# It4innovations/hyperqueue

Measured on AMD Instinct MI355X. Metric: tasks_assigned_per_sec, higher is better.
Workload: dtype u64

## Files before the change

hyperqueue_amd/_testhooks.py:

```python
from __future__ import annotations

import ctypes as C
import os

_LIB = None
LIB_PATH = os.environ.get("HQTICK_TEST_LIB") or os.path.join(os.path.dirname(os.path.abspath(__file__)), "libhqtick_test.so")


def load() -> C.CDLL:
    global _LIB
    if _LIB is None:
        if not os.path.exists(LIB_PATH):
            raise FileNotFoundError(f"{LIB_PATH} is missing: run `python -c 'import __graft_entry__ as g; g.build()'`")
        _LIB = C.CDLL(LIB_PATH)
    return _LIB
```

hyperqueue_amd/csrc/debug_capi.cpp:

```cpp
#include "../../include/hqtick_debug.h"

#include <algorithm>
#include <cstring>

#include "audit_core.h"
#include "clock_core.h"
#include "hb_order.h"
#include "milp.h"
#include "price_emul.h"

static thread_local int g_last_canonical = 0;
static thread_local long g_last_hull[2] = {0, 0};
extern "C" int hqtick_debug_milp_was_canonical(void) { return g_last_canonical; }
extern "C" void hqtick_debug_milp_last_hull(long *solves, long *nonpacking) {
    if (solves) *solves = g_last_hull[0];
    if (nonpacking) *nonpacking = g_last_hull[1];
}

extern "C" int hqtick_debug_milp_solve(int ncols, const double *obj, const uint8_t *col_kind, int nrows, const uint8_t *row_type,
                                       const double *rhs, const int *row_off, const int *row_col, const double *row_coef,
                                       double time_limit_s, int canonical, double *x_out, double *obj_out, int *is_optimal,
                                       long *nodes_out) {
    hqmilp::Model m;
    m.obj.assign(obj, obj + ncols);
    m.kind.assign(col_kind, col_kind + ncols);
    m.rtype.assign(row_type, row_type + nrows);
    m.rhs.assign(rhs, rhs + nrows);
    m.roff.assign(row_off, row_off + nrows + 1);
    int nnz = nrows ? row_off[nrows] : 0;
    m.rcol.assign(row_col, row_col + nnz);
    m.rcoef.assign(row_coef, row_coef + nnz);
    hqmilp::Result r = hqmilp::solve(m, time_limit_s, canonical != 0);
    g_last_canonical = r.canonical ? 1 : 0;
    g_last_hull[0] = r.hull_solves; g_last_hull[1] = r.hull_solves_nonpacking;
    if (nodes_out) *nodes_out = r.nodes;
    if (!r.feasible) return 0;
    for (int j = 0; j < ncols; j++) x_out[j] = r.x[j];
    *obj_out = r.objective;
    *is_optimal = r.optimal ? 1 : 0;
    return 1;
}

extern "C" void hqtick_debug_map_order_u32(const uint32_t *keys, uint32_t n, uint32_t *out_pos) {
    std::vector<uint32_t> order;
    hqhb::insertion_order_u32(keys, n, order);
    for (uint32_t i = 0; i < n; i++) out_pos[i] = order[i];
}

extern "C" int hqtick_debug_milp_solve_priced(int ncols, const double *obj, const uint8_t *col_kind, const int32_t *col_group, int nrows, const uint8_t *row_type,
                                              const uint8_t *row_implied, const double *rhs, const int *row_off, const int *row_col, const double *row_coef,
                                              double time_limit_s, int use_sweeps, uint32_t min_cols, double *x_out, double *obj_out, int *is_optimal, double *stats_out) {
    hqmilp::Model m;
    m.obj.assign(obj, obj + ncols);
    m.kind.assign(col_kind, col_kind + ncols);
    m.rtype.assign(row_type, row_type + nrows);
    m.rhs.assign(rhs, rhs + nrows);
    m.roff.assign(row_off, row_off + nrows + 1);
    int nnz = nrows ? row_off[nrows] : 0;
    m.rcol.assign(row_col, row_col + nnz);
    m.rcoef.assign(row_coef, row_coef + nnz);
    if (col_group) m.col_group.assign(col_group, col_group + ncols);
    if (row_implied) m.row_implied.assign(row_implied, row_implied + nrows);
    hqprice::EmulatedSweeper emu;
    if (min_cols) emu.min_cols = min_cols;
    hqmilp::Result r = hqmilp::solve(m, time_limit_s, true, hqmilp::REFERENCE_MIP_REL_GAP, use_sweeps ? &emu : nullptr);
    g_last_canonical = r.canonical ? 1 : 0;
    g_last_hull[0] = r.hull_solves; g_last_hull[1] = r.hull_solves_nonpacking;
    if (stats_out) { stats_out[0] = r.price_sweeps; stats_out[1] = r.price_rounds; stats_out[2] = r.price_total_us; stats_out[3] = r.canonical ? 1.0 : 0.0; }
    if (!r.feasible) return 0;
    for (int j = 0; j < ncols; j++) x_out[j] = r.x[j];
    *obj_out = r.objective;
    *is_optimal = r.optimal ? 1 : 0;
    return 1;
}

static thread_local hqmilp::Probe g_block_run_probe;
extern "C" void hqtick_debug_set_block_runs(int on) {
    hqmilp::g_probe = on < 0 ? nullptr : &g_block_run_probe; hqmilp::set_block_runs(on);
    if (on >= 0) { g_block_run_probe.model = g_block_run_probe.tables = g_block_run_probe.runs = g_block_run_probe.covered = 0; }
}
extern "C" void hqtick_debug_corrupt_block_runs(int on) { g_block_run_probe.corrupt_runs = on != 0; }
extern "C" void hqtick_debug_last_coupled_digest(uint64_t out[4]) {
    out[0] = g_block_run_probe.model; out[1] = g_block_run_probe.tables; out[2] = g_block_run_probe.runs; out[3] = g_block_run_probe.covered;
}
extern "C" void hqtick_debug_set_early_sweep(int on) { hqprice::set_early_sweep(on); }
extern "C" uint32_t hqtick_debug_early_sweeps(void) { return hqprice::early_sweeps(); }
extern "C" void hqtick_debug_capture_first_cut(int on) { hqprice::capture_first_cut(on != 0); }
extern "C" uint32_t hqtick_debug_first_cut(unsigned char *out, uint32_t cap) {
    const std::vector<unsigned char> &b = hqprice::first_cut_bytes();
    if (out && cap) memcpy(out, b.data(), std::min<size_t>(cap, b.size()));
    return (uint32_t)b.size();
}

extern "C" int hqtick_debug_clock_rows(uint32_t n, const int64_t *deadline_ns, int64_t now_ns, uint32_t nv, const uint64_t *min_time_ns, int sorted_form, int64_t *remaining_out) {
    if ((n && (!deadline_ns || !remaining_out)) || (nv && !min_time_ns)) return HQTICK_E_INVALID;
    if (!sorted_form) {
        for (uint32_t w = 0; w < n; w++) {
            if (deadline_ns[w] == hqclock::NO_LIMIT) { remaining_out[w] = hqclock::NO_LIMIT; continue; }
            const int64_t r = hqclock::sat_sub(deadline_ns[w], now_ns);
            uint64_t best = 0;
            for (uint32_t v0 = 0; r >= 0 && v0 < nv; v0 += hqclock::CHUNK) best = hqclock::fold_thresholds(best, r, min_time_ns + v0, std::min(hqclock::CHUNK, nv - v0));
            remaining_out[w] = r < 0 ? -1 : (int64_t)best;
        }
        return 0;
    }
    std::vector<uint64_t> thr(min_time_ns, min_time_ns + nv);
    std::sort(thr.begin(), thr.end()); thr.erase(std::unique(thr.begin(), thr.end()), thr.end());
    for (uint32_t w = 0; w < n; w++) remaining_out[w] = hqclock::canonical_sorted(deadline_ns[w], now_ns, thr.data(), (uint32_t)thr.size());
    return 0;
}
extern "C" int hqtick_debug_audit_host(const hqtick_debug_audit_tables *a, uint32_t parts, int order, hqtick_check_report *out) {
    if (!a || !out || (parts & ~(HQ_CHECK_ALL | HQ_CHECK_STRICT)) || order < 0 || order > 2 || (a->have & ~31u)) return HQTICK_E_INVALID;
    hqaudit::State S{};
    S.have = a->have; S.parts = parts;
    S.ready = hqaudit::Ready{a->ready_id, a->ready_rq, a->ready_n};
    S.graph = hqaudit::Graph{a->g_id, a->g_unfinished, a->g_gen, a->g_head, a->g_ht_key, a->g_ht_val, a->g_ht_mask, a->g_run_next, a->g_run_off, a->g_run_len, a->g_edge,
                             a->g_slots, a->g_runs, a->g_edges, a->g_tasks};
    S.ledger = hqaudit::Ledger{a->l_key, a->l_worker, a->l_rq, a->l_variant, a->l_mask, a->l_rq_off, a->l_ventry_off, a->l_ent_res, a->l_var_nodes, a->l_ent_kind, a->l_ent_amount,
                               a->l_Q, a->l_NV, a->l_wid, a->l_W, a->l_R, a->l_total, a->l_free, a->l_counts, a->l_stride, a->l_pf, a->l_pf_stride, a->l_mn_task, a->l_mn_root,
                               a->l_flags, a->l_n_live, a->l_mn_live, a->l_pf_live};
    S.retr = hqaudit::Retr{a->r_task, a->r_target, a->r_variant, a->r_flags, a->r_n};
    const hqaudit::Totals t{a->ready_live, a->g_tasks, a->g_free, a->g_slots};
    hqaudit::run_host(S, t, order, out);
    return (int)out->n_failed;
}
extern "C" int64_t hqtick_debug_clock_deadline(int64_t now_ns, int64_t remaining_ns) { return hqclock::deadline_of(now_ns, remaining_ns); }
extern "C" int64_t hqtick_debug_clock_remaining(int64_t deadline_ns, int64_t now_ns) { return hqclock::remaining_of(deadline_ns, now_ns); }
```

hyperqueue_amd/csrc/host_model.cpp:

```cpp
#include "host_model.h"

#include <algorithm>
#include <chrono>
#include <cmath>
#include <cstring>
#include <string>
#include <unordered_map>

#include "hb_order.h"

namespace hqhost {

namespace {

struct OrderEntry { uint64_t hash = 0; bool used = false; std::vector<uint32_t> ids, order; };
thread_local OrderEntry order_cache[32];
thread_local unsigned order_next = 0;
const std::vector<uint32_t> &cached_worker_order(const std::vector<uint32_t> &ids) {
    typedef OrderEntry Entry;
    Entry (&cache)[32] = order_cache;
    unsigned &next = order_next;
    uint64_t h = 0x9E3779B97F4A7C15ull ^ ids.size();
    for (uint32_t v : ids) { h ^= v; h *= 0xFF51AFD7ED558CCDull; h ^= h >> 29; }
    for (Entry &e : cache) if (e.used && e.hash == h && e.ids.size() == ids.size() && (ids.empty() || memcmp(e.ids.data(), ids.data(), ids.size() * 4) == 0)) return e.order;
// ... 1081 lines not shown
        if (blocker_ord[brq] < 0) {
            blocker_ord[brq] = (int32_t)n_blockers_seen++;
            left_state.resize((size_t)n_blockers_seen * n_sig_cap, 0); left_row.resize((size_t)n_blockers_seen * n_sig_cap * R); left_of.resize(left_state.size());
        }
        const size_t li = (size_t)blocker_ord[brq] * n_sig_cap + sg;
        if (left_state[li] == 0) {
            if (agg_off.empty()) build_agg();
            const uint32_t a0 = agg_off[w], na = agg_off[w + 1] - a0;
            const uint32_t *arq = na ? agg_rq.data() + a0 : nullptr, *acnt = na ? agg_cnt.data() + a0 : nullptr; const uint8_t *avar = na ? agg_variant.data() + a0 : nullptr;
            if (gaps.leftover_row(brq, ws.total + (size_t)w * R, R, arq, avar, na, acnt, &left_row[li * R])) left_state[li] = 3;
            else {
                Amounts tot; tot.a.assign(ws.total + (size_t)w * R, ws.total + (size_t)(w + 1) * R);
                left_state[li] = gaps.leftover(brq, tot, arq, avar, na, acnt, left_of[li]) ? 1 : 2;
            }
        }
        return left_state[li] == 3 ? gaps.fit_row(low_rq, &left_row[li * R], R) : (left_state[li] == 1 ? gaps.fit(low_rq, left_of[li]) : 0);
    };
    std::vector<uint32_t> gap_of_sig; uint32_t batch_no = UINT32_MAX;
    std::vector<std::vector<uint8_t>> cap_cache; std::vector<int8_t> all_cap_cache; size_t n_triples = 0, n_decided_once = 0;
    std::vector<uint32_t> bcols_off, bcols_end((size_t)ws.n, 0); std::vector<int> bcols; std::vector<uint64_t> bcols_ub; uint64_t bcols_ub_max = 0; uint32_t bcols_batch = UINT32_MAX;
    for (const TaskBatch &batch : batches) {
        batch_no++;
        auto cc = count_cols.find(batch.rq);
        if (cc == count_cols.end()) continue;
        const RequestView &brv = pb.rqs[batch.rq];
        if (!batch.limit_reached) {
            list_row(hqmilp::ROW_MAX, (double)batch.size, count_lhs_id(batch.rq), cc->second, -1, 0.0);
        }
        double bsize = (double)batch.size;
        std::vector<uint32_t> capped_by;
        struct PairMemo { bool done = false, whole = false, all_gap = false; uint32_t gap_all = 0; int lhs_id = -1; int64_t max_excess = INT64_MIN; std::vector<int> no_gap; std::vector<std::pair<uint32_t, uint32_t>> with_gap; };
        std::vector<PairMemo> pair_memo;
        for (const PriorityCut &cut : batch.cuts) {
            for (auto &bl : cut.blockers) {
                uint32_t brq = bl.first; bool bounded = bl.second != HQ_BLOCKER_UNBOUNDED;
                std::vector<int> no_gap_mn;
                const std::vector<int> *no_gap = &no_gap_mn;
                int no_gap_id = -1;
                std::vector<int> cols;
                int fl_cached = -2;
                if (pb.rq_multi_node(batch.rq)) {
                    for (uint32_t g = 0; g < pb.n_groups; g++) {
                        auto it = group_cols.find({batch.rq, g});
                        if (it != group_cols.end() && group_can_run_rq(g, brq)) no_gap_mn.push_back(it->second);
                    }
                } else {
                    if (pair_memo.size() < pb.rqs.size()) pair_memo.resize(pb.rqs.size());
                    PairMemo &pm = pair_memo[brq];
                    if (!pm.done) {
                        pm.done = true;
                        if (cap_cache.size() < pb.rqs.size()) cap_cache.resize(pb.rqs.size());
                        std::vector<uint8_t> &cap_brq = cap_cache[brq];
                        if (cap_brq.empty()) { cap_brq.assign(ws.n, 0); for (uint32_t w : solver_workers) cap_brq[w] = pb.capable_rqv(ws, w, brq) ? 1 : 0; }
                        if (bcols_batch != batch_no) {
                            bcols_batch = batch_no; bcols_off.assign((size_t)ws.n + 1, 0); bcols.clear(); bcols_ub.assign(ws.n, 0); bcols_ub_max = 0;
                            if (runs_on) bcols.reserve((size_t)m.ncols());
                            for (uint32_t w : solver_workers) {
                                bcols_off[w] = (uint32_t)bcols.size();
                                if (runs_on && stamp_first[w] != UINT32_MAX) {
                                    const uint32_t f = stamp_first[w]; const int d = blk_base[w] - blk_base[f];
                                    for (uint32_t i = bcols_off[f], e = bcols_end[f]; i < e; i++) { const int pc = bcols[i] + d; bcols.push_back(pc); }
                                    bcols_ub[w] = bcols_ub[f];
                                } else
                                for (uint8_t v = 0; v < brv.n_variants; v++) { const int pc = place_get(w, batch.rq, v); if (pc >= 0) { bcols.push_back(pc); bcols_ub[w] += col_ub[(size_t)pc]; } }
                                bcols_end[w] = (uint32_t)bcols.size(); bcols_ub_max = std::max(bcols_ub_max, bcols_ub[w]);
                            }
                        }
                        n_triples++;
                        if (!sigs_done) { for (uint32_t w : solver_workers) sig_of(w); sigs_done = true; }
                        gap_of_sig.assign(sig_rep.size(), UINT32_MAX);
                        bool all_capable = true;
                        if (runs_on) {
                            if (all_cap_cache.size() < pb.rqs.size()) all_cap_cache.resize(pb.rqs.size(), -1);
                            if (all_cap_cache[brq] < 0) { all_cap_cache[brq] = 1; for (uint32_t w : solver_workers) if (!cap_brq[w]) { all_cap_cache[brq] = 0; break; } }
                            all_capable = all_cap_cache[brq] != 0;
                        } else
                        if (sig_rep.size() == 1) for (uint32_t w : solver_workers) if (!cap_brq[w]) { all_capable = false; break; }
                        if (sig_rep.size() == 1 && all_capable && !solver_workers.empty()) {
                            const uint32_t w0 = solver_workers[0];
                            const uint32_t gap = gap_of(brq, batch.rq, gap_sig[w0], w0);
                            if (runs_on) {
                                if (gap > 0) { pm.all_gap = true; pm.gap_all = gap; pm.max_excess = (int64_t)bcols_ub_max - (int64_t)gap; } else pm.whole = true;
                            } else
                            if (gap > 0) { pm.with_gap.reserve(solver_workers.size()); for (uint32_t w : solver_workers) pm.with_gap.push_back({w, gap}); }
                            else pm.no_gap.assign(bcols.begin(), bcols.end());
                        } else {
                        pm.no_gap.reserve(bcols.size());
                        for (uint32_t w : solver_workers) {
                            if (!cap_brq[w]) continue;
                            uint32_t gap = gap_of_sig[gap_sig[w]];
                            if (gap == UINT32_MAX) gap = gap_of_sig[gap_sig[w]] = gap_of(brq, batch.rq, gap_sig[w], w);
                            if (gap > 0) pm.with_gap.push_back({w, gap});
                            else pm.no_gap.insert(pm.no_gap.end(), bcols.data() + bcols_off[w], bcols.data() + bcols_end[w]);
                        }
                        }
                        auto list_of = [&](const PairMemo &q) -> const std::vector<int> & { return q.whole ? bcols : q.no_gap; };
                        if (!list_of(pm).empty()) {
                            for (const PairMemo &o : pair_memo) if (&o != &pm && o.lhs_id >= 0 && ((o.whole && pm.whole) || list_of(o) == list_of(pm))) { pm.lhs_id = o.lhs_id; break; }
                            if (pm.lhs_id < 0) pm.lhs_id = next_lhs_id++;
                        }
                        if (runs_on) for (auto &wg : pm.with_gap) pm.max_excess = std::max(pm.max_excess, (int64_t)bcols_ub[wg.first] - (int64_t)wg.second);
                    }
                    no_gap = pm.whole ? &bcols : &pm.no_gap; no_gap_id = pm.lhs_id;
                    auto gap_rows = [&](const uint32_t w, const uint32_t gap) {
                        const int *wc = bcols.data() + bcols_off[w]; const size_t nwc = bcols_end[w] - bcols_off[w];
                        const uint64_t cols_ub = bcols_ub[w];
                        if (bounded && fl_cached == -2) fl_cached = short_flag(brq, bl.second);
                        const int fl = bounded ? fl_cached : -1;
                        if (cols_ub <= (uint64_t)cut.size + gap) return;
                        if (bounded && fl >= 0) { cols.assign(wc, wc + nwc); emit_plus(hqmilp::ROW_MAX, (double)cut.size + bsize + (double)gap, cols, fl, bsize); }
                        else if (!bounded) { m.begin_row(hqmilp::ROW_MAX, (double)cut.size + (double)gap); for (size_t k = 0; k < nwc; k++) m.term(wc[k], 1.0); m.end_row(); }
                    };
                    if (runs_on && (pm.all_gap || !pm.with_gap.empty()) && pm.max_excess <= (int64_t)cut.size) {
                        if (bounded) fl_cached = short_flag(brq, bl.second);
                        n_decided_once++;
                    } else if (pm.all_gap) for (uint32_t w : solver_workers) gap_rows(w, pm.gap_all);
                    else for (auto &wg : pm.with_gap) gap_rows(wg.first, wg.second);
                }
                if (no_gap->empty()) continue;
                int fl;
                if (bounded && (fl = short_flag(brq, bl.second)) >= 0) list_row(hqmilp::ROW_MAX, bsize + (double)cut.size, no_gap_id, *no_gap, fl, bsize);
                else if (!bounded && std::find(capped_by.begin(), capped_by.end(), brq) == capped_by.end()) {
                    capped_by.push_back(brq);
                    list_row(hqmilp::ROW_MAX, (double)cut.size, no_gap_id, *no_gap, -1, 0.0);
                }
            }
        }
    }

    if (!seq_start.empty()) {
        m.start.assign(m.ncols(), 0.0);
        for (const SeqStart &ss : seq_start) {
            const int pc = place_get(ss.w, batches[ss.batch].rq, ss.variant);
            if (pc < 0) { m.start.clear(); break; }
            m.start[pc] = ss.count;
        }
    }
    m.row_implied.resize(m.nrows(), 0);
    m.row_lhs.resize((size_t)m.nrows(), -1); m.row_lhs_len.resize((size_t)m.nrows(), 0); m.row_block.resize((size_t)m.nrows(), -1);
    m.col_ub = col_ub; m.col_ub.resize((size_t)m.ncols(), UINT32_MAX);
    if (hqmilp::g_probe) {
        using hqmilp::fnv1a_vec;
        uint64_t h = hqmilp::FNV_BASIS;
        h = fnv1a_vec(h, m.obj); h = fnv1a_vec(h, m.kind); h = fnv1a_vec(h, m.rtype); h = fnv1a_vec(h, m.rhs); h = fnv1a_vec(h, m.roff); h = fnv1a_vec(h, m.rcol); h = fnv1a_vec(h, m.rcoef);
        h = fnv1a_vec(h, m.start); h = fnv1a_vec(h, m.col_group); h = fnv1a_vec(h, m.row_implied); h = fnv1a_vec(h, m.row_lhs); h = fnv1a_vec(h, m.row_lhs_len);
        h = fnv1a_vec(h, m.list_off); h = fnv1a_vec(h, m.list_col); h = fnv1a_vec(h, m.row_block); h = fnv1a_vec(h, m.col_ub);
        hqmilp::g_probe->model = h; hqmilp::g_probe->runs = m.block_runs.size(); hqmilp::g_probe->tables = 0; hqmilp::g_probe->covered = 0;
    }
    const double t_model1 = clock_us();
    if (trace_model) {
        size_t run_blocks = 0; for (const auto &br : m.block_runs) run_blocks += (size_t)br.n_blocks;
        fprintf(stderr, "[model] cuts done at %.3f ms: %d columns, %d rows, %zu terms, %zu worker signatures, %zu (batch, cut, blocker) passes over the workers; %zu equal-block runs over %zu blocks, %zu (cut, blocker) passes decided once\n", (t_model1 - t_model0) / 1e3, m.ncols(), m.nrows(), m.rcol.size(), sig_rep.size(), n_triples, m.block_runs.size(), run_blocks, n_decided_once);
    }
    hqmilp::Result sol = hqmilp::solve(m, pb.time_limit_s, !pb.certificate_only, hqmilp::REFERENCE_MIP_REL_GAP, pb.pricer);
    if (trace_model) fprintf(stderr, "[model] solve done %.3f ms after the model\n", (clock_us() - t_model1) / 1e3);
    out.pre_us = t_model0 - t_enter; out.model_us = t_model1 - t_model0; out.milp_us = clock_us() - t_model1; out.price_sweeps = sol.price_sweeps; out.price_rounds = sol.price_rounds; out.price_us = sol.price_total_us;
    out.milp_nodes = sol.nodes; out.milp_cols = m.ncols(); out.milp_rows = m.nrows(); out.milp_components = sol.n_components;
    if (!sol.feasible) return out;
    out.is_optimal = sol.optimal;
    out.is_canonical = sol.canonical && sol.optimal;

    std::vector<uint64_t> key_hash; std::vector<std::pair<uint32_t, uint8_t>> key_list; std::vector<std::vector<std::pair<uint32_t, uint32_t>>> key_counts;
    std::vector<uint64_t> mn_hash; std::vector<uint32_t> mn_list; std::vector<std::vector<std::vector<uint32_t>>> mn_sets;
    std::vector<uint32_t> dec_ids, dec_widx, dec_cnt;
    for (const TaskBatch &batch : batches) {
        const RequestView &rv = pb.rqs[batch.rq];
        if (pb.rq_multi_node(batch.rq)) {
            size_t n_nodes = pb.variants[rv.first_variant].n_nodes;
            std::vector<std::vector<uint32_t>> sets;
            for (uint32_t w : solver_workers) {
                const int pc = place_get(w, batch.rq, 0);
                if (pc < 0 || (uint32_t)std::round(sol.x[pc]) == 0) continue;
                if (!sets.empty() && sets.back().size() < n_nodes) sets.back().push_back(w); else sets.push_back({w});
            }
            if (!sets.empty()) { mn_hash.push_back(hqhb::hash_rq_variant(batch.rq, 0)); mn_list.push_back(batch.rq); mn_sets.push_back(sets); }
        } else {
            for (uint8_t v = 0; v < rv.n_variants; v++) {
                const size_t nsw = solver_workers.size();
                dec_ids.resize(nsw + 1); dec_widx.resize(nsw + 1); dec_cnt.resize(nsw + 1);
                uint32_t *idp = dec_ids.data(), *wxp = dec_widx.data(), *cp = dec_cnt.data(); size_t nk = 0;
                const int *pcol = place_col.data() + rv.first_variant + v;
                const double *xs = sol.x.data();
                for (size_t i = 0; i < nsw; i++) {
                    const uint32_t w = solver_workers[i];
                    const int pc = pcol[(size_t)w * NVS];
                    const double xv = pc >= 0 ? xs[pc] : 0.0;
                    const uint32_t c = xv > 0.0 ? (uint32_t)(xv + 0.5) : 0u;
                    idp[nk] = ws.id[w]; wxp[nk] = w; cp[nk] = c; nk += c > 0 ? 1 : 0;
                }
                if (nk == 0) continue;
                dec_ids.resize(nk);
                const std::vector<uint32_t> &ids = dec_ids, &widx = dec_widx, &cnt = dec_cnt;
                const std::vector<uint32_t> &word = cached_worker_order(ids);
                std::vector<std::pair<uint32_t, uint32_t>> ordered; ordered.reserve(word.size());
                for (uint32_t k : word) ordered.push_back({widx[k], cnt[k]});
                key_hash.push_back(hqhb::hash_rq_variant(batch.rq, v)); key_list.push_back({batch.rq, v}); key_counts.push_back(std::move(ordered));
            }
        }
    }
    std::vector<uint32_t> ord;
    hqhb::insertion_order(key_hash.data(), (uint32_t)key_hash.size(), ord);
    for (uint32_t k : ord) { out.keys.push_back(key_list[k]); out.per_key.push_back(std::move(key_counts[k])); }
    hqhb::insertion_order(mn_hash.data(), (uint32_t)mn_hash.size(), ord);
    for (uint32_t k : ord) { out.mn_rq.push_back(mn_list[k]); out.mn_sets.push_back(std::move(mn_sets[k])); }
    if (trace_model) fprintf(stderr, "[model] decoded %.3f ms after the model, %.3f ms after the solver was entered\n", (clock_us() - t_model1) / 1e3, (clock_us() - t_enter) / 1e3);
    return out;
}

}
```

hyperqueue_amd/csrc/host_model.h:

```cpp
#pragma once
#include <cstdint>
#include <map>
#include <string>
#include <tuple>
#include <vector>

#include "../../include/hqtick.h"
#include "block_core.h"
#include "price.h"
#include "milp.h"

namespace hqhost {

struct VariantView {
    const uint32_t *res;
    const uint8_t *kind;
    const uint64_t *amount;
    uint32_t n_entries, n_nodes, weight;
    uint64_t min_time_ns;
    bool multi_node() const { return n_nodes > 0; }
};

struct RequestView {
    uint32_t first_variant, n_variants;
};

struct QueueLevels {
    std::vector<std::pair<uint64_t, uint32_t>> levels;
};

struct PriorityCut { uint32_t size; std::vector<std::pair<uint32_t, uint32_t>> blockers; };
struct TaskBatch {
    uint32_t rq = 0, size = 0, limit = 0;
    bool limit_reached = false, is_blocker = false;
    std::vector<PriorityCut> cuts;
};

struct WorkerGroups {
    std::vector<uint32_t> of, rep, count;
    std::vector<uint32_t> solver_workers;
    std::vector<double> pool;
    bool valid = false;
};

struct WorkerSet {
    WorkerGroups rows;
    uint32_t n = 0, R = 0;
    const uint32_t *id = nullptr;
    const uint64_t *total = nullptr, *free_ = nullptr;
    const int64_t *remaining_ns = nullptr;
    const float *min_util = nullptr;
    const uint8_t *flags = nullptr;
    const uint32_t *group = nullptr;
    const uint8_t *vflags = nullptr;
    const uint32_t *vtmc = nullptr;
    uint32_t n_variant_slots = 0;
    std::vector<std::vector<std::pair<uint32_t, uint8_t>>> blocked;
    uint32_t n_blocked_lists = 0;
    const uint32_t *assigned_off = nullptr, *assigned_rq = nullptr; const uint8_t *assigned_variant = nullptr;
    const uint32_t *agg_off = nullptr, *agg_rq = nullptr, *agg_cnt = nullptr; const uint8_t *agg_variant = nullptr;
    uint32_t n_assigned(uint32_t w) const { return assigned_off ? assigned_off[w + 1] - assigned_off[w] : agg_off ? agg_off[w + 1] - agg_off[w] : 0; }
    bool is_sn(uint32_t w) const { return flags ? (flags[w] & HQ_WORKER_SN) != 0 : true; }
    bool stopping(uint32_t w) const { return flags ? (flags[w] & HQ_WORKER_STOPPING) != 0 : false; }
    bool is_free(uint32_t w) const { return is_sn(w) && n_assigned(w) == 0 && !stopping(w); }
    uint8_t vf(uint32_t w, uint32_t slot) const { return vflags[(size_t)w * n_variant_slots + slot]; }
    uint32_t tmc(uint32_t w, uint32_t slot) const { return vtmc[(size_t)w * n_variant_slots + slot]; }
};

struct BlockSolver {
    virtual ~BlockSolver() {}
    virtual bool solve(const hqblock::ColTable &cols, const hqblock::ClassTable &classes, const hqblock::Output &out) = 0;
    virtual bool begin(const hqblock::ColTable &cols, const hqblock::ClassTable &classes, const hqblock::Output &out) { begun_ok = solve(cols, classes, out); return begun_ok; }
    virtual bool finish() { return begun_ok; }
    virtual bool overlaps() const { return false; }
    bool begun_ok = false;
};

void flush_tick_caches();

struct BlockMemo {
    struct Entry { uint64_t hash = 0; std::vector<unsigned char> key; std::vector<double> x; long nodes = 0; int n_components = 0; };
    static constexpr size_t CAP = 64;
    std::vector<Entry> entries;
    size_t next = 0;
    std::vector<unsigned char> scratch;
    uint64_t scratch_hash = 0;
    const Entry *find(const hqmilp::Model &m);
    void put(const hqmilp::Result &r);
};

struct Problem {
    BlockMemo *memo = nullptr;
    BlockSolver *blocks = nullptr;
    hqprice::Sweeper *pricer = nullptr;
    uint32_t block_min_classes = 1;
    uint32_t block_verify = 2;
    uint32_t tick_seq = 0;
    uint32_t R = 0, n_groups = 0;
    std::vector<RequestView> rqs;
    std::vector<VariantView> variants;
    WorkerSet real;
    const WorkerSet *custom = nullptr;
    double time_limit_s = 5.0;
    bool certificate_only = false;
    bool rq_multi_node(uint32_t rq) const { return variants[rqs[rq].first_variant].multi_node(); }
    bool capable_rqv(const WorkerSet &ws, uint32_t w, uint32_t rq) const {
        for (uint32_t v = 0; v < rqs[rq].n_variants; v++) {
            uint32_t slot = rqs[rq].first_variant + v;
            uint8_t f = ws.vf(w, slot);
            if ((f & 4) && (variants[slot].multi_node() || (f & 2))) return true;
        }
        return false;
    }
};

void group_equal_rows(WorkerSet &ws, bool all_solver);

std::vector<TaskBatch> create_task_batches(const Problem &pb, const std::vector<QueueLevels> &queues);

struct Counts {
    std::vector<std::pair<uint32_t, uint8_t>> keys;
    std::vector<std::vector<std::pair<uint32_t, uint32_t>>> per_key;
    std::vector<uint32_t> mn_rq;
    std::vector<std::vector<std::vector<uint32_t>>> mn_sets;
    struct WorkerList { std::vector<uint32_t> widx; };
    bool by_class = false;
    bool one_class = false;
    uint32_t n_cols = 0;
    std::vector<uint32_t> wclass, class_x, key_col, key_list;
    std::vector<WorkerList> lists;
    bool pairs_built = true;
    void pairs() {
        if (pairs_built) return;
        per_key.assign(keys.size(), {});
        for (size_t k = 0; k < keys.size(); k++) {
            const std::vector<uint32_t> &wi = lists[key_list[k]].widx;
            auto &out = per_key[k]; out.resize(wi.size());
            for (size_t i = 0; i < wi.size(); i++) out[i] = {wi[i], class_x[(size_t)wclass[wi[i]] * n_cols + key_col[k]]};
        }
        pairs_built = true;
    }
    size_t key_size(size_t k) const { return pairs_built ? per_key[k].size() : lists[key_list[k]].widx.size(); }
    bool is_optimal = true;
    bool is_canonical = true;
    bool empty() const {
        if (!pairs_built) { for (size_t k = 0; k < keys.size(); k++) if (key_size(k)) return false; }
        for (auto &k : per_key) if (!k.empty()) return false;
        for (auto &k : mn_sets) if (!k.empty()) return false;
        return true;
    }
    uint32_t checksum() const {
        uint32_t h = 2166136261u;
        auto mix = [&](uint32_t v) { for (int i = 0; i < 4; i++) { h ^= (v >> (8 * i)) & 0xFFu; h *= 16777619u; } };
        mix(is_optimal ? 1u : 0u);
        for (size_t k = 0; k < keys.size(); k++) {
            mix(keys[k].first); mix(keys[k].second);
            if (pairs_built) for (auto &wc : per_key[k]) { mix(wc.first); mix(wc.second); }
            else for (uint32_t w : lists[key_list[k]].widx) { mix(w); mix(class_x[(size_t)wclass[w] * n_cols + key_col[k]]); }
        }
        for (size_t k = 0; k < mn_rq.size(); k++) { mix(mn_rq[k]); for (auto &set : mn_sets[k]) { mix(0xFFFFFFFFu); for (uint32_t w : set) mix(w); } }
        return h;
    }
    int error = 0; std::string errmsg;
    long milp_nodes = 0; int milp_cols = 0, milp_rows = 0, milp_components = 0;
    int price_sweeps = 0, price_rounds = 0; double price_us = 0, milp_us = 0, model_us = 0, pre_us = 0;
    uint32_t blocks_device = 0, blocks_host = 0, block_steps_max = 0, n_classes = 0;
    uint32_t blocks_verified = 0, blocks_mismatch = 0, blocks_rejected = 0;
    uint32_t blocks_memo = 0;
    double t_classify_us = 0, t_blocks_us = 0, t_decode_us = 0;
};

Counts run_scheduling_solver(const Problem &pb, const std::vector<TaskBatch> &batches);

}
```

hyperqueue_amd/csrc/hqtick.cpp:

```cpp
#include "../../include/hqtick.h"
#ifdef HQTICK_TEST_HOOKS
#include "../../include/hqtick_debug.h"
#endif

#include <dlfcn.h>
#include <hip/hip_runtime.h>
#include <rccl/rccl.h>

#include <algorithm>
#include <chrono>
#include <cstdio>
#include <cstdlib>
#include <cstring>
#include <functional>
#include <map>
#include <string>
#include <vector>

#include "audit.h"
#include "block_solve.h"
#include "cluster.h"
#include "price_dev.h"
#include "ready.h"
#include "scan.h"
#ifdef HQTICK_TEST_HOOKS
#include "price_emul.h"
#endif
#include "devbuf.h"
#include "graph.h"
#include "ledger.h"
#include "map.h"
#include "hb_order.h"
#include "host_model.h"
#include "kernels.h"

using hqbuf::DevBuf;
using hqbuf::PinBuf;
using hqcluster::UpView;
using hqscan::Scan;
using hqscan::WorkerEval;

namespace {

double now_us() { return std::chrono::duration<double, std::micro>(std::chrono::steady_clock::now().time_since_epoch()).count(); }

}

namespace {
struct ViewHooks {
    hqscan::Scanner scan;
    bool valid = false; const void *ids = nullptr; uint64_t N = 0; uint32_t Q = 0, n_live = 0; bool rq_copy = false; std::vector<uint32_t> run_off, run_start, run_rank;
    DevBuf d_map, d_sel_task, d_sel_rank, d_rq, d_want;
    void release() { scan.release(); d_map.release(); d_sel_task.release(); d_sel_rank.release(); d_rq.release(); d_want.release(); }
};
}

struct hqtick_ctx {
    hqtick_config cfg;
    int device = 0;
    hipStream_t stream = nullptr;
    hipStream_t stream2 = nullptr;
    bool k2_on_hist = false;
    bool k2_own_stream = false;
    hipEvent_t ev[14] = {};
    std::string err = "";
    hqready::ReadySet ready;
    hqhost::BlockMemo block_memo;
    hqscan::Scanner scan;
    hqmap::Mapper map;
    bool timing = true, timing_k1 = false;
    PinBuf h_up, h_up2, h_q, h_blk;
    PinBuf h_blkprof; uint32_t n_blkprof = 0; bool block_profile = false;
    hqprice::DeviceSweeper *pricer = nullptr;
    uint32_t block_budget = 4096, block_min_classes = 12;
    DevBuf d_blk;
    hqcluster::WorkerSet ws;
    hqcluster::Retracting retr;
    uint32_t last_row_groups = 0;
    bool wait_on_kernel = true;
    hqhost::Problem pb;
    std::vector<uint32_t> b_rq, b_size, b_limit, b_cut_off, c_size, c_bl_off, bl_rq, bl_size; std::vector<uint8_t> b_lr, b_blk;
    std::vector<uint8_t> q_loaded;
    hqtick_kernel_stats stats{};
    uint32_t tpw_hint = 0;
    uint32_t shard_index = 0, shard_count = 1;
    void *sink = nullptr; size_t sink_bytes = 0;
    hqgraph::Graph graph;
    hqasg::Ledger asg;
    hqtick_ctx *qctx = nullptr;
    ViewHooks *view_hooks = nullptr;
    ncclComm_t comm = nullptr; uint32_t comm_rank = 0, comm_world = 0;
    hqtick_exchange_fn xfn = nullptr; void *xuser = nullptr;
    DevBuf d_xsend, d_xrecv; PinBuf h_xsend, h_xrecv;
    uint32_t shard_min_blocks = 1025, shard_min_classes = 1025; bool shard_solve = true;
    uint32_t block_verify = 2, tick_seq = 0;
    uint64_t x_calls = 0, x_bytes = 0; double x_us = 0;
    double tl[32] = {}; int ntl = 0;
    hqaudit::Auditor audit;
    bool check_resident = false; int audit_depth = 0;
};

namespace {

#define HQ_HIP(call)                                                                                          \
    do {                                                                                                      \
        hipError_t e_ = (call);                                                                               \
        if (e_ != hipSuccess) { ctx->err = std::string(#call) + ": " + hipGetErrorString(e_); return HQTICK_E_DEVICE; } \
    } while (0)

#define HQ_HIP_TIMED(call)                                                                                    \
    do {                                                                                                      \
        hipError_t e_ = (call);                                                                               \
        hqk::take_launch_timer();                                                                             \
        if (e_ != hipSuccess) { ctx->err = std::string(#call) + ": " + hipGetErrorString(e_); return HQTICK_E_DEVICE; } \
    } while (0)

#define HQ_HIP_LAST(call, launched)                                                                           \
    do {                                                                                                      \
        hipError_t e_ = (call);                                                                               \
        (launched) = hqk::take_launch_timer().stop == nullptr && ctx->wait_on_kernel;                        \
        if (e_ != hipSuccess) { ctx->err = std::string(#call) + ": " + hipGetErrorString(e_); return HQTICK_E_DEVICE; } \
    } while (0)

int fail(hqtick_ctx *ctx, int code, const std::string &msg) { ctx->err = msg; return code; }

double elapsed_us(hipEvent_t a, hipEvent_t b) {
    float ms = 0;
    if (hipEventElapsedTime(&ms, a, b) == hipSuccess) return (double)ms * 1000.0;
    (void)hipGetLastError();
    return -1.0;
}

int validate(hqtick_ctx *ctx, const hqtick_snapshot *s, bool need_tasks) {
    if (!s) return fail(ctx, HQTICK_E_INVALID, "null snapshot");
    if (s->n_workers && (!s->worker_id || !s->worker_total || !s->worker_free)) return fail(ctx, HQTICK_E_INVALID, "worker arrays missing");
    for (uint32_t w = 1; w < s->n_workers; w++) if (s->worker_id[w - 1] >= s->worker_id[w]) return fail(ctx, HQTICK_E_INVALID, "worker ids not ascending");
    if (s->n_requests && (!s->rq_variant_off || !s->variant_entry_off)) return fail(ctx, HQTICK_E_INVALID, "request arrays missing");
    for (uint32_t q = 0; q < s->n_requests; q++) {
        if (s->rq_variant_off[q + 1] <= s->rq_variant_off[q]) return fail(ctx, HQTICK_E_INVALID, "request without variants");
        if (s->rq_variant_off[q + 1] - s->rq_variant_off[q] > 32) return fail(ctx, HQTICK_E_INVALID, "more than 32 variants");
    }
    uint32_t nv = s->n_requests ? s->rq_variant_off[s->n_requests] : 0;
    for (uint32_t e = 0; e < (nv ? s->variant_entry_off[nv] : 0); e++) {
        if (s->entry_resource[e] >= s->n_resources) return fail(ctx, HQTICK_E_INVALID, "entry resource id out of range");
        if (s->entry_kind[e] == HQ_ENTRY_AMOUNT && s->entry_amount[e] == 0) return fail(ctx, HQTICK_E_INVALID, "zero amount request");
    }
    if (need_tasks && s->n_ready) {
        if (!s->task_id || !s->task_priority || !s->task_rq) return fail(ctx, HQTICK_E_INVALID, "ready-set columns missing");
        for (uint64_t i = 1; i < s->n_ready; i++) if (s->task_id[i - 1] >= s->task_id[i]) return fail(ctx, HQTICK_E_INVALID, "ready set not sorted by task id");
    }
    if (s->n_blocked && (!s->blocked_worker || !s->blocked_rq || !s->blocked_variant)) return fail(ctx, HQTICK_E_INVALID, "blocked arrays missing");
    for (uint32_t k = 0; k < s->n_blocked; k++) {
        if (s->blocked_worker[k] >= s->n_workers) return fail(ctx, HQTICK_E_INVALID, "blocked worker index");
        if (s->blocked_rq[k] >= s->n_requests) return fail(ctx, HQTICK_E_INVALID, "blocked request id out of range");
        if (s->blocked_variant[k] >= s->rq_variant_off[s->blocked_rq[k] + 1] - s->rq_variant_off[s->blocked_rq[k]]) return fail(ctx, HQTICK_E_INVALID, "blocked variant out of range");
    }
    if (s->worker_group) for (uint32_t w = 0; w < s->n_workers; w++) if (s->worker_group[w] >= (s->n_groups ? s->n_groups : 1)) return fail(ctx, HQTICK_E_INVALID, "worker_group >= n_groups");
    if (s->assigned_off) {
        for (uint32_t w = 0; w < s->n_workers; w++) if (s->assigned_off[w] > s->assigned_off[w + 1]) return fail(ctx, HQTICK_E_INVALID, "assigned_off not monotone");
        if (s->n_workers && s->assigned_off[s->n_workers] && (!s->assigned_rq || !s->assigned_variant)) return fail(ctx, HQTICK_E_INVALID, "assigned arrays missing");
    }
    if (s->prefilled_off) {
        for (uint32_t w = 0; w < s->n_workers; w++) if (s->prefilled_off[w] > s->prefilled_off[w + 1]) return fail(ctx, HQTICK_E_INVALID, "prefilled_off not monotone");
        if (s->n_workers && s->prefilled_off[s->n_workers] && !s->prefilled_rq) return fail(ctx, HQTICK_E_INVALID, "prefilled_rq missing");
    }
    if (s->prefill_off) {
        for (uint32_t q = 0; q < s->n_requests; q++) if (s->prefill_off[q] > s->prefill_off[q + 1]) return fail(ctx, HQTICK_E_INVALID, "prefill_off not monotone");
        const uint32_t np = s->n_requests ? s->prefill_off[s->n_requests] : 0;
        if (np && (!s->prefill_priority || !s->prefill_task || !s->prefill_worker)) return fail(ctx, HQTICK_E_INVALID, "prefill arrays missing");
        for (uint32_t i = 0; i < np; i++) if (s->prefill_worker[i] >= s->n_workers) return fail(ctx, HQTICK_E_INVALID, "prefill worker index");
    }
    if (s->n_retracting && (!s->retracting_task || !s->retracting_worker)) return fail(ctx, HQTICK_E_INVALID, "retracting arrays missing");
    for (uint32_t k = 0; k < s->n_retracting; k++) {
        if (s->retracting_worker[k] >= s->n_workers) return fail(ctx, HQTICK_E_INVALID, "retracting worker index");
        if (k && s->retracting_task[k - 1] >= s->retracting_task[k]) return fail(ctx, HQTICK_E_INVALID, "retracting tasks not ascending");
        if (s->retracting_redirect_worker && s->retracting_redirect_worker[k] != HQ_NO_WORKER && s->retracting_redirect_worker[k] >= s->n_workers) return fail(ctx, HQTICK_E_INVALID, "retracting redirect worker index");
    }
    return 0;
}

int upload_tables(hqtick_ctx *ctx, const hqtick_snapshot *s, uint32_t W, const uint64_t *total, const uint64_t *free_, const int64_t *rem, PinBuf &buf, UpView *uv) {
    const uint32_t R = s->n_resources;
    const hqcluster::TabLayout L = hqcluster::table_layout(s, W);
    if (hqk::worker_eval_lds(R, L.nv, L.ne) > 150 * 1024) return fail(ctx, HQTICK_E_CAPACITY, "request table + 32 worker rows exceed the 150 KiB the worker-evaluation kernel stages in LDS");
    if (!buf.ensure(L.bytes)) return fail(ctx, HQTICK_E_DEVICE, "allocating upload staging");
    unsigned char *h = buf.as<unsigned char>();
    hqcluster::pack_worker_rows(h, L, W, R, total, free_, rem);
    hqcluster::pack_request_tables(h, L, s);
    hqcluster::view_tables(buf.dev<unsigned char>(), L, uv);
    return 0;
}

int cluster_fail(hqtick_ctx *ctx, int rc) { if (rc < 0) ctx->err = ctx->ws.err; return rc; }

hqready::Env ready_env(hqtick_ctx *ctx) { return hqready::Env{ctx->device, ctx->stream, ctx->ev[11], ctx->wait_on_kernel}; }
int ready_fail(hqtick_ctx *ctx, int rc) { if (rc < 0) ctx->err = ctx->ready.err; return rc; }

int eval_workers_sync(hqtick_ctx *ctx, const hqtick_snapshot *s, uint32_t W, const uint64_t *total, const uint64_t *free_, const int64_t *rem, WorkerEval *out) {
    UpView uv; int rc;
    if ((rc = upload_tables(ctx, s, W, total, free_, rem, ctx->h_up2, &uv))) return rc;
    size_t n = (size_t)W * uv.rt.n_variants;
    if (!ctx->h_q.ensure(n * 5 + 64)) return fail(ctx, HQTICK_E_DEVICE, "hipHostMalloc query eval");
    out->tmc = ctx->h_q.as<uint32_t>(); out->flags = ctx->h_q.as<uint8_t>() + n * 4;
    if (n == 0) return 0;
    HQ_HIP(hqk::worker_eval(uv.total, uv.free_, uv.rem, W, s->n_resources, uv.rt, uv.n_entries, ctx->h_q.dev<uint8_t>() + n * 4, ctx->h_q.dev<uint32_t>(), ctx->stream));
    HQ_HIP(hipStreamSynchronize(ctx->stream));
    return 0;
}

void fill_problem(hqhost::Problem &pb, const hqtick_snapshot *s, const hqtick_config &cfg, const WorkerEval &ev) {
    pb.R = s->n_resources; pb.n_groups = s->n_groups ? s->n_groups : 1; pb.time_limit_s = cfg.mip_time_limit_s; pb.certificate_only = (cfg.flags & HQTICK_FLAG_CERTIFICATE_ONLY) != 0;
    uint32_t nv = s->n_requests ? s->rq_variant_off[s->n_requests] : 0;
    pb.rqs.resize(s->n_requests); pb.variants.resize(nv);
    for (uint32_t q = 0; q < s->n_requests; q++) pb.rqs[q] = {s->rq_variant_off[q], s->rq_variant_off[q + 1] - s->rq_variant_off[q]};
    for (uint32_t v = 0; v < nv; v++) {
        uint32_t e0 = s->variant_entry_off[v];
        pb.variants[v] = {s->entry_resource + e0, s->entry_kind + e0, s->entry_amount + e0, s->variant_entry_off[v + 1] - e0,
                          s->variant_n_nodes ? s->variant_n_nodes[v] : 0, s->variant_weight ? s->variant_weight[v] : 10000,
                          s->variant_min_time_ns ? s->variant_min_time_ns[v] : 0};
    }
    hqhost::WorkerSet &ws = pb.real;
    ws.n = s->n_workers; ws.R = s->n_resources; ws.id = s->worker_id; ws.total = s->worker_total; ws.free_ = s->worker_free;
    ws.remaining_ns = s->worker_remaining_ns; ws.min_util = s->worker_min_utilization; ws.flags = s->worker_flags; ws.group = s->worker_group;
    ws.vflags = ev.flags; ws.vtmc = ev.tmc; ws.n_variant_slots = nv;
    if (ws.blocked.size() != ws.n || ws.n_blocked_lists) { ws.blocked.assign(ws.n, {}); ws.n_blocked_lists = 0; }
    ws.assigned_off = s->assigned_off; ws.assigned_rq = s->assigned_rq; ws.assigned_variant = s->assigned_variant;
    ws.agg_off = nullptr; ws.agg_rq = nullptr; ws.agg_cnt = nullptr; ws.agg_variant = nullptr;
    for (uint32_t k = 0; k < s->n_blocked; k++) ws.blocked[s->blocked_worker[k]].push_back({s->blocked_rq[k], s->blocked_variant[k]});
    ws.n_blocked_lists = s->n_blocked;
    hqhost::group_equal_rows(ws, false);
}

// ... 57 lines not shown

struct DeviceBlocks : hqhost::BlockSolver {
    hqtick_ctx *ctx;
    explicit DeviceBlocks(hqtick_ctx *c) : ctx(c) {}
    bool solve(const hqblock::ColTable &ct, const hqblock::ClassTable &cl, const hqblock::Output &out) override { return begin(ct, cl, out) && finish(); }
    bool overlaps() const override { return true; }
    hqblock::Output p_out{}; size_t p_ox = 0, p_ost = 0, p_osteps = 0; uint32_t p_nd = 0, p_nc = 0; bool p_launched = false, p_pending = false;
    bool begin(const hqblock::ColTable &ct, const hqblock::ClassTable &cl, const hqblock::Output &out) override {
        p_pending = false;
        const uint32_t NC = ct.n_cols, R = ct.R, nd = cl.n_classes, ne = ct.ent_off[NC];
        auto al8 = [](size_t v) { return (v + 7) & ~(size_t)7; };
        const size_t o_off = 0, o_res = al8(o_off + (size_t)(NC + 1) * 4), o_w = al8(o_res + (size_t)ne * 4), o_kind = al8(o_w + (size_t)NC * 4), o_amt = al8(o_kind + ne),
                     o_pool = o_amt + (size_t)ne * 8, o_free = (o_pool + (size_t)R * 8 + 15) & ~(size_t)15, o_tot = o_free + (size_t)nd * R * 8, o_elig = o_tot + (size_t)nd * R * 8,
                     o_x = o_elig + (size_t)nd * 8, o_st = o_x + al8((size_t)nd * NC * 4), o_steps = o_st + al8((size_t)nd * 4), bytes = o_steps + al8((size_t)nd * 4) + 64;
        if (!ctx->h_blk.ensure(bytes)) return false;
        if (!ctx->d_blk.ensure(o_x + 64)) return false;
        unsigned char *h = ctx->h_blk.as<unsigned char>(), *d = ctx->d_blk.as<unsigned char>(), *dpin = ctx->h_blk.dev<unsigned char>();
        memcpy(h + o_off, ct.ent_off, (size_t)(NC + 1) * 4); memcpy(h + o_res, ct.ent_res, (size_t)ne * 4); memcpy(h + o_w, ct.weight, (size_t)NC * 4);
        memcpy(h + o_kind, ct.ent_kind, ne); memcpy(h + o_amt, ct.ent_amount, (size_t)ne * 8); memcpy(h + o_pool, ct.pool, (size_t)R * 8);
        memcpy(h + o_free, cl.free_, (size_t)nd * R * 8); memcpy(h + o_tot, cl.total, (size_t)nd * R * 8); memcpy(h + o_elig, cl.elig, (size_t)nd * 8);
        if (hqk::copy_pinned_to_hbm(dpin, d, o_x, ctx->stream) != hipSuccess) return false;
        hqblock::ColTable dct{NC, R, (const uint32_t *)(d + o_off), (const uint32_t *)(d + o_res), (const uint8_t *)(d + o_kind), (const uint64_t *)(d + o_amt), (const uint32_t *)(d + o_w), (const double *)(d + o_pool), d, (uint32_t)o_free};
        hqblock::ClassTable dcl{nd, (const uint64_t *)(d + o_free), (const uint64_t *)(d + o_tot), (const uint64_t *)(d + o_elig)};
        uint64_t *dprof = nullptr;
        if (ctx->block_profile) {
            if (!ctx->h_blkprof.ensure((size_t)nd * 64 + 64)) return false;
            memset(ctx->h_blkprof.p, 0, (size_t)nd * 64);
            dprof = ctx->h_blkprof.dev<uint64_t>(); ctx->n_blkprof = nd;
        }
        hqblock::Output dout{(uint32_t *)(dpin + o_x), (uint32_t *)(dpin + o_st), (uint32_t *)(dpin + o_steps), dprof};
        hqk::time_next_launch(ctx->timing ? ctx->ev[9] : nullptr, ctx->ev[10]);
        const hipError_t be = hqblock::block_solve(dct, dcl, dout, ctx->block_budget, ctx->stream);
        const bool launched = hqk::take_launch_timer().stop == nullptr && ctx->wait_on_kernel;
        if (be != hipSuccess) return false;
        p_out = out; p_ox = o_x; p_ost = o_st; p_osteps = o_steps; p_nd = nd; p_nc = NC; p_launched = launched; p_pending = true;
        return true;
    }
    bool finish() override {
        if (!p_pending) return false;
        p_pending = false;
        if ((p_launched ? hipEventSynchronize(ctx->ev[10]) : hipStreamSynchronize(ctx->stream)) != hipSuccess) return false;
        const unsigned char *h = ctx->h_blk.as<unsigned char>();
        memcpy(p_out.x, h + p_ox, (size_t)p_nd * p_nc * 4); memcpy(p_out.status, h + p_ost, (size_t)p_nd * 4); memcpy(p_out.steps, h + p_osteps, (size_t)p_nd * 4);
        if (ctx->timing) { const double us_ = elapsed_us(ctx->ev[9], ctx->ev[10]); if (us_ >= 0) ctx->stats.block_solve_us = us_; }
        ctx->stats.n_classes_device = p_nd;
        return true;
    }
};

bool rccl_allgather_host(hqtick_ctx *ctx, const void *send, void *recv, size_t bytes);
struct CtxExchange : hqprice::Exchange {
    hqtick_ctx *ctx;
    explicit CtxExchange(hqtick_ctx *c) : ctx(c) { rank = c->shard_index; world = c->shard_count; }
    static bool available(const hqtick_ctx *c) { return c->shard_solve && c->shard_count > 1 && (c->xfn || (c->comm && c->comm_world == c->shard_count)); }
    bool allgather(const void *send, void *recv, size_t bytes) override {
        if (ctx->xfn) return ctx->xfn(ctx->xuser, send, recv, bytes) == 0;
        return rccl_allgather_host(ctx, send, recv, bytes);
    }
    ~CtxExchange() override { ctx->x_calls += n_calls; ctx->x_bytes += n_bytes; ctx->x_us += us; }
};

struct ShardedBlocks : hqhost::BlockSolver {
    hqhost::BlockSolver &inner; hqprice::Exchange &ex; uint32_t min_classes;
    hqblock::Output p_out{}; uint32_t p_nd = 0, p_nc = 0, p_nm = 0; bool p_pass = false, p_inner_ok = false, p_pending = false;
    std::vector<uint64_t> cfree, ctot, celig; std::vector<uint32_t> dx, dst, dsteps; std::vector<unsigned char> send, recv;
    ShardedBlocks(hqhost::BlockSolver &in, hqprice::Exchange &e, uint32_t mc) : inner(in), ex(e), min_classes(mc) {}
    bool overlaps() const override { return inner.overlaps(); }
    bool solve(const hqblock::ColTable &ct, const hqblock::ClassTable &cl, const hqblock::Output &out) override { return begin(ct, cl, out) && finish(); }
    bool begin(const hqblock::ColTable &ct, const hqblock::ClassTable &cl, const hqblock::Output &out) override {
        p_pass = ex.world <= 1 || cl.n_classes < min_classes;
        if (p_pass) return inner.begin(ct, cl, out);
        const uint32_t nd = cl.n_classes, R = ct.R, NC = ct.n_cols, W = ex.world, me = ex.rank;
        const uint32_t nm = nd > me ? (nd - me + W - 1) / W : 0;
        cfree.resize((size_t)nm * R); ctot.resize((size_t)nm * R); celig.resize(nm);
        for (uint32_t j = 0; j < nm; j++) {
            const size_t i = (size_t)me + (size_t)j * W;
            memcpy(cfree.data() + (size_t)j * R, cl.free_ + i * R, (size_t)R * 8); memcpy(ctot.data() + (size_t)j * R, cl.total + i * R, (size_t)R * 8); celig[j] = cl.elig[i];
        }
        dx.assign((size_t)nm * NC, 0); dst.assign(nm, hqblock::ST_UNSUPPORTED); dsteps.assign(nm, 0);
        p_out = out; p_nd = nd; p_nc = NC; p_nm = nm; p_pending = true;
        p_inner_ok = nm == 0 || inner.begin(ct, hqblock::ClassTable{nm, cfree.data(), ctot.data(), celig.data()}, hqblock::Output{dx.data(), dst.data(), dsteps.data(), nullptr});
        return true;
    }
    bool finish() override {
        if (p_pass) return inner.finish();
        if (!p_pending) return false;
        p_pending = false;
        if (p_nm && !(p_inner_ok && inner.finish())) { std::fill(dst.begin(), dst.end(), (uint32_t)hqblock::ST_UNSUPPORTED); std::fill(dx.begin(), dx.end(), 0u); }
        const uint32_t W = ex.world, NC = p_nc, mx = (p_nd + W - 1) / W;
        const size_t o_st = (size_t)mx * NC * 4, o_steps = o_st + (size_t)mx * 4, bytes = (o_steps + (size_t)mx * 4 + 7) & ~(size_t)7;
        send.assign(bytes, 0); recv.resize(bytes * W);
        if (p_nm) { memcpy(send.data(), dx.data(), (size_t)p_nm * NC * 4); memcpy(send.data() + o_st, dst.data(), (size_t)p_nm * 4); memcpy(send.data() + o_steps, dsteps.data(), (size_t)p_nm * 4); }
        const double t0 = now_us();
        if (!ex.allgather(send.data(), recv.data(), bytes)) return false;
        ex.us += now_us() - t0; ex.n_calls++; ex.n_bytes += bytes * W;
        for (uint32_t r = 0; r < W; r++) {
            const unsigned char *b = recv.data() + (size_t)r * bytes;
            const uint32_t nr = p_nd > r ? (p_nd - r + W - 1) / W : 0;
            for (uint32_t j = 0; j < nr; j++) {
                const size_t i = (size_t)r + (size_t)j * W;
                memcpy(p_out.x + i * NC, b + (size_t)j * NC * 4, (size_t)NC * 4); memcpy(p_out.status + i, b + o_st + (size_t)j * 4, 4); memcpy(p_out.steps + i, b + o_steps + (size_t)j * 4, 4);
            }
        }
        return true;
    }
};

hqmap::Env map_env(hqtick_ctx *ctx, double t0 = 0) {
    return hqmap::Env{ctx->stream, ctx->ev[4], ctx->ev[5], ctx->ev[1], ctx->ev[6], ctx->ev[7], ctx->ev[11], ctx->timing, ctx->wait_on_kernel, ctx->cfg.flags,
                      ctx->sink, ctx->sink_bytes, ctx->shard_index, ctx->shard_count, hqmap::Timeline{t0, ctx->tl, &ctx->ntl}};
}
int map_fail(hqtick_ctx *ctx, int rc) { if (rc < 0) ctx->err = ctx->map.err; return rc; }
bool transpose_enabled() { const char *e = getenv("HQTICK_TRANSPOSE"); return !(e && atoi(e) == 0); }

struct TickRun {
    hqtick_ctx *ctx; const hqtick_snapshot *s; hqtick_result *out; const bool use_resident;
    hqmap::Plan &ps; hqhost::Problem &pb;
    const uint32_t W, R, Q;
    WorkerEval ev; Scan sc; hqhost::Counts cnt;
    uint64_t N = 0; int status = HQTICK_DONE;
    double t0 = 0;

    TickRun(hqtick_ctx *c, const hqtick_snapshot *snap, hqtick_result *o, bool resident)
        : ctx(c), s(snap), out(o), use_resident(resident), ps(c->map.plan), pb(c->pb), W(snap->n_workers), R(snap->n_resources), Q(snap->n_requests) {}

    void mark() { hqmap::Timeline{t0, ctx->tl, &ctx->ntl}.mark(); }
    int plan_fail(int rc, const char *why) { if (rc) ctx->err = why; return rc; }

    int load_ready_set() {
        if (!use_resident) {
            if (int rc = ready_fail(ctx, ctx->ready.load(ctx->stream, s, true))) return rc;
            ctx->scan.columns_changed();
        } else if (!ctx->ready.resident()) return fail(ctx, HQTICK_E_INVALID, "hqtick_run_resident without hqtick_upload_ready");
        N = ctx->ready.cols().n;
        return 0;
    }

    hqmap::PlanIn plan_in() {
        hqmap::PlanIn in{};
        in.sc = &sc; in.cnt = &cnt; in.s = s; in.rqs = pb.rqs.data(); in.variants = pb.variants.data();
        in.proactive_filling_reserve = ctx->cfg.proactive_filling_reserve; in.proactive_filling_max = ctx->cfg.proactive_filling_max; in.flags = ctx->cfg.flags;
        in.sink = ctx->sink != nullptr; in.shard_index = ctx->shard_index; in.shard_count = ctx->shard_count;
        in.N = N; in.retr_key = ctx->scan.retracting_keys(); in.retr_rank = ctx->scan.retracting_ranks();
        if (ctx->asg.on && ctx->asg.tracking()) {
            uint32_t pf_stride = 0;
            const std::vector<uint32_t> &h_pf = ctx->asg.prefilled_host(&pf_stride);
            if (h_pf.size() >= (size_t)W * pf_stride) { in.ledger_pf = h_pf.data(); in.ledger_pf_stride = pf_stride; }
        }
        in.transpose_on = transpose_enabled();
        in.storage = hqmap::Mapper::plan_storage; in.user = &ctx->map;
        return in;
    }

    int phase_c(const hqmap::Env &me, const hqmap::PlanIn &in) {
        hqmap::PhaseC pc{};
        pc.sc = &sc; pc.scan = &ctx->scan; pc.ready = &ctx->ready; pc.in = &in;
        pc.consume_in_tick = use_resident && (ctx->cfg.flags & HQTICK_FLAG_CONSUME_IN_TICK) != 0;
        pc.ledger_pfq_rq = ctx->asg.on;
        if (ps.n_sel && pc.consume_in_tick && ctx->asg.on && s->n_retracting) {
            pc.saved_rq = ctx->asg.saved_rq(N);
            if (!pc.saved_rq) return fail(ctx, HQTICK_E_DEVICE, "hipMalloc ledger request ids");
        }
        if (ps.n_sel && ctx->asg.on && ps.n_rec) {
            hqasg::StageCols c{};
            if (!ctx->asg.stage_for(ps.n_rec, sc.ordered, sc.L, &c)) return fail(ctx, HQTICK_E_DEVICE, "hipMalloc ledger staging");
            pc.stage = hqk::Stage{c.task, c.rq, c.row, c.level, c.meta};
        }
        const int rc = map_fail(ctx, ctx->map.phase_c(me, pc));
        const hqmap::Timings &tm = ctx->map.timings();
        if (tm.select_us >= 0) ctx->stats.select_us = tm.select_us;
        if (tm.sweep_us >= 0) ctx->stats.sweep_us = tm.sweep_us;
        if (tm.other_us >= 0) ctx->stats.other_us = tm.other_us;
        return rc;
    }

    void finish(const hqmap::Env &me, double t1, double t2, double t3) {
        out->status = status;
        ctx->map.export_result(me, cnt, out);
        mark();
        double t5 = now_us();
        out->t_total_us = t5 - t0; out->t_scan_us = t1 - t0; out->t_batches_us = t2 - t1; out->t_solve_us = t3 - t2; out->t_mapping_us = t5 - t3;
        uint64_t n_pref = 0; for (uint32_t q = 0; q < Q; q++) n_pref += ps.new_pf_total[q];
        uint64_t n_asg = 0; for (uint32_t w = 0; w < W; w++) n_asg += ps.n_assign[w];
        uint32_t nv = Q ? s->rq_variant_off[Q] : 0;
        ctx->stats.n_assigned = n_asg; ctx->stats.n_prefilled = n_pref;
        ctx->stats.algorithmic_bytes = N * 20 + (uint64_t)W * R * 16 + (uint64_t)nv * R * 9 + n_asg * 13 + n_pref * 12;
        ctx->stats.tick_gpu_us = ctx->stats.distinct_us + ctx->stats.level_hist_us + ctx->stats.scan_us + ctx->stats.block_solve_us + ctx->stats.select_us + ctx->stats.sweep_us + ctx->stats.other_us;
    }

    int run() {
        t0 = now_us();
        ctx->ntl = 0;
        if (ctx->cfg.flags & HQTICK_FLAG_NO_TICK_CACHES) { ctx->scan.columns_changed(); hqhost::flush_tick_caches(); }
        memset(out, 0, sizeof(*out));
        ctx->stats = hqtick_kernel_stats{};
        int rc = validate(ctx, s, !use_resident);
        if (rc) return rc;
        HQ_HIP(hipSetDevice(ctx->device));
        if ((rc = load_ready_set())) return rc;
        const std::function<void()> prep = [&]() {
            fill_problem(pb, s, ctx->cfg, ev);
            ctx->last_row_groups = (uint32_t)pb.real.rows.rep.size();
            if (ctx->asg.on && !s->assigned_off) {
                const hqasg::Agg g = ctx->asg.agg();
                pb.real.agg_off = g.off; pb.real.agg_rq = g.rq; pb.real.agg_cnt = g.cnt; pb.real.agg_variant = g.var;
            }
            if (pb.certificate_only && (ctx->shard_count > 1 || ctx->sink || ctx->xfn || ctx->comm)) pb.certificate_only = false;
        };
        if ((rc = phase_a(ctx, s, &ev, &sc, &prep))) return rc;
        mark();
        const double t1 = now_us();
        std::vector<hqhost::QueueLevels> qlv = queue_levels(sc, s);
        std::vector<hqhost::TaskBatch> batches = hqhost::create_task_batches(pb, qlv);
        export_batches(ctx, batches, out);
        mark();
        const double t2 = now_us();
        DeviceBlocks dev_blocks(ctx);
        pb.blocks = &dev_blocks; pb.block_min_classes = ctx->block_min_classes; pb.pricer = ctx->pricer;
        pb.block_verify = ctx->block_verify; pb.tick_seq = ctx->tick_seq++;
        pb.memo = (ctx->cfg.flags & (HQTICK_FLAG_NO_BLOCK_MEMO | HQTICK_FLAG_NO_TICK_CACHES)) ? nullptr : &ctx->block_memo;
        double shard_sweep_us = -1.0;
        ctx->x_calls = 0; ctx->x_bytes = 0; ctx->x_us = 0;
        if (CtxExchange::available(ctx)) {
            CtxExchange xch(ctx);
            ShardedBlocks sh_blocks(dev_blocks, xch, ctx->shard_min_classes);
            pb.blocks = &sh_blocks;
            if (ctx->pricer) {
                hqprice::ShardedSweeper sh_sweeps(*ctx->pricer, xch, ctx->shard_min_blocks);
                pb.pricer = &sh_sweeps;
                cnt = hqhost::run_scheduling_solver(pb, batches);
                shard_sweep_us = sh_sweeps.stat_sweep_us;
            } else cnt = hqhost::run_scheduling_solver(pb, batches);
        } else cnt = hqhost::run_scheduling_solver(pb, batches);
        pb.blocks = nullptr; pb.pricer = nullptr;
        ctx->stats.price_sweeps = (uint32_t)cnt.price_sweeps; ctx->stats.price_rounds = (uint32_t)cnt.price_rounds; ctx->stats.price_us = cnt.price_us; ctx->stats.milp_us = cnt.milp_us; ctx->stats.model_us = cnt.model_us; ctx->stats.solve_pre_us = cnt.pre_us;
        ctx->stats.price_sweep_us = shard_sweep_us >= 0.0 ? shard_sweep_us : (ctx->pricer ? ctx->pricer->stat_sweep_us : 0.0); ctx->stats.milp_cols = (uint32_t)cnt.milp_cols; ctx->stats.milp_rows = (uint32_t)cnt.milp_rows;
        ctx->stats.n_classes_verified = cnt.blocks_verified; ctx->stats.n_classes_mismatch = cnt.blocks_mismatch; ctx->stats.n_classes_rejected = cnt.blocks_rejected; ctx->stats.n_classes_memo = cnt.blocks_memo;
        ctx->stats.exchange_calls = (uint32_t)ctx->x_calls; ctx->stats.exchange_bytes = ctx->x_bytes; ctx->stats.exchange_us = ctx->x_us;
        if (cnt.error) return fail(ctx, cnt.error, cnt.errmsg);
        ctx->stats.n_classes_device = cnt.blocks_device; ctx->stats.n_classes_host = cnt.blocks_host; ctx->stats.block_steps_max = cnt.block_steps_max; ctx->stats.n_classes = cnt.n_classes;
        ctx->stats.solve_classify_us = cnt.t_classify_us; ctx->stats.solve_blocks_us = cnt.t_blocks_us; ctx->stats.solve_decode_us = cnt.t_decode_us;
        mark();
        const double t3 = now_us();
        out->is_optimal = cnt.is_optimal;
        out->is_canonical = cnt.is_canonical && cnt.is_optimal;
        status = HQTICK_DONE;
        if (!cnt.is_optimal) status = cnt.empty() ? HQTICK_NO_PROGRESS : HQTICK_NEED_MORE_COMPUTE;
        const hqmap::PlanIn in = plan_in();
        const hqmap::Env me = map_env(ctx, t0);
        hqmap::HostResult &hr = ctx->map.res;
        const char *why = nullptr;
        ctx->ready.selection_void();
        if ((rc = plan_fail(hqmap::plan_keys(ps, hr, in, &why), why))) return rc;
        if ((rc = map_fail(ctx, ctx->map.launch_sweep_early(me)))) return rc;
        if ((rc = plan_fail(hqmap::plan_redirects(ps, hr, in, &why), why))) return rc;
        mark();
        if ((rc = plan_fail(hqmap::plan_prefill(ps, hr, in, &why), why))) return rc;
        mark();
        if ((rc = plan_fail(hqmap::plan_outputs(ps, hr, in, &why), why))) return rc;
        if ((rc = map_fail(ctx, ctx->map.check_capacity(sc.ordered)))) return rc;
        mark();
        if ((rc = phase_c(me, in))) return rc;
        mark();
        finish(me, t1, t2, t3);
        return status;
    }
};

bool ledger_replica(const hqtick_ctx *ctx) { return ctx->shard_count > 1 || ctx->xfn || ctx->comm; }
hqasg::Env ledger_env(hqtick_ctx *ctx) {
    const hqready::Cols c = ctx->ready.cols();
    return hqasg::Env{ctx->device, ctx->stream, ctx->ws.rows(), ctx->ws.W(), ctx->ws.R(), c.id, c.prio, c.rq, c.n,
                      ctx->scan.levels_dev(), &ctx->ws.ids(), ctx->ws.flags(), ctx->ws.free_rows()};
}
int ledger_fail(hqtick_ctx *ctx, int rc) { if (rc < 0) ctx->err = ctx->asg.err; return rc; }
bool ledger_pending_live(hqtick_ctx *ctx) { return ctx->asg.pending_live(ctx->ready.selection_live()); }
int ledger_guard(hqtick_ctx *ctx) {
    if (ctx->asg.on && ledger_pending_live(ctx)) return fail(ctx, HQTICK_E_INVALID, "assignment ledger: the last tick's placement is pending (hqtick_ready_consume_last first)");
    return 0;
}

int run_tick(hqtick_ctx *ctx, const hqtick_snapshot *s, hqtick_result *out, bool use_resident) {
    hqtick_snapshot full;
    if (ctx->asg.on && s) {
        if (ledger_replica(ctx)) return fail(ctx, HQTICK_E_UNSUPPORTED, "assignment ledger on a sharded or replica context");
        if (s->worker_id || !ctx->ws.valid()) return fail(ctx, HQTICK_E_INVALID, "assignment ledger on: the tick runs on the resident worker set (HQ_WORKERS_RESIDENT, no worker arrays)");
        if (s->assigned_off) return fail(ctx, HQTICK_E_INVALID, "assignment ledger on: the snapshot must not carry an assigned CSR as well");
        if (ctx->asg.tracking() && s->prefilled_off) return fail(ctx, HQTICK_E_INVALID, "prefilled tracking on: the snapshot must not carry a prefilled CSR as well");
        HQ_HIP(hipSetDevice(ctx->device));
        ctx->asg.abandon_tick();
        ctx->asg.take_requests(s);
        if (ctx->asg.tracking() && ctx->asg.max_variants() >= hqasg::PF_VARIANT) return fail(ctx, HQTICK_E_UNSUPPORTED, "prefilled tracking: a request has 254 or more variants");
        if (int rc = ctx->asg.sync_mirror(ledger_env(ctx))) return ledger_fail(ctx, rc);
    }
    if (s) {
        if (int rc = cluster_fail(ctx, ctx->ws.complete(s, &full))) return rc;
        s = &full;
    }
    const bool retr_resident = s && s->n_retracting == HQ_RETRACTING_RESIDENT;
    if (retr_resident) { if (int rc = ctx->retr.to_snapshot(s->worker_id, s->n_workers, &full)) return fail(ctx, rc, ctx->retr.err); }
    int rc;
    {
        TickRun run(ctx, s, out, use_resident);
        rc = run.run();
    }
    if (ctx->ready.unconfirmed()) {
        ctx->ready.confirm();
        if (rc < 0) {
            const std::string why = ctx->err;
            bool restored = false;
            const bool synced = hipStreamSynchronize(ctx->stream) == hipSuccess;
            if (synced && ctx->ready.selection_valid())
                restored = ctx->map.replay_selection(ctx->stream, hqmap::REPLAY_RESTORE, ctx->ready.cols(), ctx->scan, ctx->ready.selected_count(), &ctx->h_q) == 0;
            if (restored) ctx->ready.put_back(); else ctx->ready.lost();
            ctx->err = why;
            if (restored) ctx->err += " (HQTICK_FLAG_CONSUME_IN_TICK: what the tick had taken is back in the resident ready set)";
            else { ctx->err += " (HQTICK_FLAG_CONSUME_IN_TICK: the tick had already taken its tasks and they could not be put back; the resident ready set is dropped, upload it again)"; }
        }
    }
    if (rc >= 0 && retr_resident) ctx->retr.apply_tick(s->worker_id, s->n_workers, ctx->map.res.retract_off, ctx->map.res.retract_task, ctx->map.res.red_task, ctx->map.res.red_worker, ctx->map.res.red_variant, ctx->map.res.red_kind);
    if (rc >= 0 && ctx->asg.on) {
        const bool in_tick = use_resident && (ctx->cfg.flags & HQTICK_FLAG_CONSUME_IN_TICK) != 0;
        ctx->asg.collect_tick(s, out, ctx->map.res.new_free, ctx->map.res.mn_rq, in_tick && s->n_retracting != 0);
        if (!use_resident || in_tick) {
            if (int r2 = ledger_fail(ctx, ctx->asg.apply_tick(ledger_env(ctx)))) {
                ctx->asg.on = false; ctx->asg.pending = false;
                ctx->err += " (the assignment ledger is switched off: upload the worker set and enable it again)";
                return r2;
            }
        }
    }
    return rc;
}

}

namespace {
struct AuditScope {
    hqtick_ctx *c;
    explicit AuditScope(hqtick_ctx *ctx) : c(ctx) { if (c) c->audit_depth++; }
    ~AuditScope() { if (c) c->audit_depth--; }
};
int audited(hqtick_ctx *ctx, int rc) {
    static const char *const names[HQ_INV_N] = {"HQ_INV_READY_ORDER", "HQ_INV_READY_COUNT", "HQ_INV_LEDGER_HASH", "HQ_INV_LEDGER_ENTRY", "HQ_INV_LEDGER_TOTALS", "HQ_INV_LEDGER_COUNTS",
                                                "HQ_INV_LEDGER_PREFILLED", "HQ_INV_LEDGER_FREE", "HQ_INV_LEDGER_MN", "HQ_INV_GRAPH_HASH", "HQ_INV_GRAPH_TOTALS", "HQ_INV_GRAPH_COUNTER",
                                                "HQ_INV_X_READY_ASSIGNED", "HQ_INV_X_READY_WAITING", "HQ_INV_X_RETRACTING", "HQ_INV_S_READY_UNKNOWN", "HQ_INV_S_ASSIGNED_WAITING",
                                                "HQ_INV_S_RELEASED_NOWHERE"};
    if (!ctx || !ctx->check_resident || ctx->audit_depth || rc < 0) return rc;
    hqtick_check_report rep;
    const int arc = hqtick_resident_check(ctx, HQ_CHECK_READY | HQ_CHECK_LEDGER | HQ_CHECK_GRAPH, &rep);
    if (arc <= 0) return arc < 0 ? arc : rc;
    std::string m = "HQTICK_CHECK_RESIDENT: the resident state is inconsistent after this call:";
    for (uint32_t k = 0; k < HQ_INV_N; k++)
        if (rep.count[k]) m += std::string(" ") + names[k] + " (" + std::to_string(rep.count[k]) + " violations, first key " + std::to_string(rep.first[k]) + ")";
    return fail(ctx, HQTICK_E_INVALID, m);
}
template <class F> int with_audit(hqtick_ctx *ctx, F &&body) {
    int rc;
    { AuditScope scope(ctx); rc = body(); }
    return audited(ctx, rc);
}
}

extern "C" {

uint32_t hqtick_abi_version(void) { return HQTICK_ABI_VERSION; }
const char *hqtick_build_arch(void) { return "gfx950"; }

int hqtick_create(const hqtick_config *config, hqtick_ctx **out_ctx) {
    if (!config || !out_ctx || (config->abi_version != HQTICK_ABI_VERSION && config->abi_version != 10u && config->abi_version != 11u)) return HQTICK_E_INVALID;
    int n = 0;
    if (hipGetDeviceCount(&n) != hipSuccess || n <= 0 || config->device_index < 0 || config->device_index >= n) return HQTICK_E_NO_DEVICE;
    hipDeviceProp_t prop;
    if (hipGetDeviceProperties(&prop, config->device_index) != hipSuccess) return HQTICK_E_NO_DEVICE;
    if (std::string(prop.gcnArchName).rfind("gfx950", 0) != 0) return HQTICK_E_NO_DEVICE;
    if (hipSetDevice(config->device_index) != hipSuccess) return HQTICK_E_NO_DEVICE;
    hqtick_ctx *ctx = new hqtick_ctx();
    ctx->cfg = *config; ctx->device = config->device_index;
    ctx->timing = (config->flags & HQTICK_FLAG_NO_KERNEL_TIMING) == 0;
    if (const char *e = getenv("HQTICK_TPW")) { long v = atol(e); if (v >= 256 && v <= (1 << 20) && v % 256 == 0) ctx->tpw_hint = (uint32_t)v; }
    if (const char *e = getenv("HQTICK_BLOCK_PROFILE")) ctx->block_profile = atoi(e) != 0;
    if (const char *e = getenv("HQTICK_CHECK_RESIDENT")) ctx->check_resident = atoi(e) != 0;
    if (const char *e = getenv("HQTICK_BLOCK_BUDGET")) { long v = atol(e); if (v >= 1 && v <= (1 << 24)) ctx->block_budget = (uint32_t)v; }
    if (const char *e = getenv("HQTICK_BLOCK_MIN_CLASSES")) { long v = atol(e); if (v >= 0) ctx->block_min_classes = (uint32_t)v; }
    if (hipStreamCreateWithFlags(&ctx->stream, hipStreamNonBlocking) != hipSuccess) { delete ctx; return HQTICK_E_DEVICE; }
    if (hipStreamCreateWithFlags(&ctx->stream2, hipStreamNonBlocking) != hipSuccess) { hipStreamDestroy(ctx->stream); delete ctx; return HQTICK_E_DEVICE; }
    if (const char *e = getenv("HQTICK_K2_RIDE_ALONG")) { ctx->k2_own_stream = atoi(e) == 0; ctx->k2_on_hist = atoi(e) == 1; }
    if (const char *e = getenv("HQTICK_WAIT_ON_KERNEL")) ctx->wait_on_kernel = atoi(e) != 0;
    {
        bool price = true; uint32_t min_cols = 0;
        if (const char *e = getenv("HQTICK_PRICE")) price = atoi(e) != 0;
        if (const char *e = getenv("HQTICK_PRICE_MIN_COLS")) { long v = atol(e); if (v > 0) min_cols = (uint32_t)v; }
        if (price) { ctx->pricer = new hqprice::DeviceSweeper(ctx->stream); ctx->pricer->budget = ctx->block_budget; if (min_cols) ctx->pricer->min_cols = min_cols; }
    }
    if (const char *e = getenv("HQTICK_BLOCK_VERIFY")) ctx->block_verify = strcmp(e, "all") == 0 ? 0xFFFFFFFFu : (uint32_t)std::max(0L, atol(e));
    if (const char *e = getenv("HQTICK_SHARD_SOLVE")) ctx->shard_solve = atoi(e) != 0;
    if (const char *e = getenv("HQTICK_SHARD_MIN_BLOCKS")) { long v = atol(e); if (v >= 0) ctx->shard_min_blocks = (uint32_t)v; }
    if (const char *e = getenv("HQTICK_SHARD_MIN_CLASSES")) { long v = atol(e); if (v >= 0) ctx->shard_min_classes = (uint32_t)v; }
    if (ctx->ws.init()) { delete ctx; return HQTICK_E_DEVICE; }
    for (auto &e : ctx->ev) if (hipEventCreate(&e) != hipSuccess) { delete ctx; return HQTICK_E_DEVICE; }
    if (ctx->scan.init()) { delete ctx; return HQTICK_E_DEVICE; }
    *out_ctx = ctx;
    return 0;
}

static void rccl_destroy_comm(hqtick_ctx *ctx);
void hqtick_destroy(hqtick_ctx *ctx) {
    if (!ctx) return;
    hipSetDevice(ctx->device);
    if (ctx->stream) hipStreamSynchronize(ctx->stream);
    if (ctx->stream2) hipStreamSynchronize(ctx->stream2);
    delete ctx->pricer; ctx->pricer = nullptr;
    ctx->d_blk.release();
    ctx->map.release();
    ctx->scan.release();
    ctx->ready.release();
    ctx->ws.release();
    if (ctx->qctx) { hqtick_destroy(ctx->qctx); ctx->qctx = nullptr; }
    if (ctx->view_hooks) { ctx->view_hooks->release(); delete ctx->view_hooks; ctx->view_hooks = nullptr; }
    hipSetDevice(ctx->device);
    if (ctx->comm) { rccl_destroy_comm(ctx); }
    ctx->graph.release();
    ctx->asg.release_all();
    ctx->audit.release();
    ctx->h_up.release(); ctx->h_up2.release(); ctx->h_q.release(); ctx->h_blk.release(); ctx->h_blkprof.release();
    for (auto &e : ctx->ev) if (e) hipEventDestroy(e);
    if (ctx->stream) hipStreamDestroy(ctx->stream);
    if (ctx->stream2) hipStreamDestroy(ctx->stream2);
    delete ctx;
}

const char *hqtick_last_error(const hqtick_ctx *ctx) { return ctx ? ctx->err.c_str() : "null ctx"; }

int hqtick_run(hqtick_ctx *ctx, const hqtick_snapshot *snapshot, hqtick_result *out) { return with_audit(ctx, [&]() -> int {
    if (!ctx || !out) return HQTICK_E_INVALID;
    return run_tick(ctx, snapshot, out, false);
}); }

int hqtick_upload_ready(hqtick_ctx *ctx, uint64_t n, const uint64_t *task_id, const uint64_t *task_priority, const uint32_t *task_rq, int sorted) { return with_audit(ctx, [&]() -> int {
    if (!ctx) return HQTICK_E_INVALID;
    if (n && (!task_id || !task_priority || !task_rq)) return fail(ctx, HQTICK_E_INVALID, "null ready-set column");
    if (sorted) for (uint64_t i = 1; i < n; i++) if (task_id[i - 1] >= task_id[i]) return fail(ctx, HQTICK_E_INVALID, "ready set not sorted by task id");
    for (uint64_t i = 0; i < n; i++) if (task_rq[i] == 0xFFFFFFFFu) return fail(ctx, HQTICK_E_INVALID, "request id 0xFFFFFFFF is reserved");
    HQ_HIP(hipSetDevice(ctx->device));
    if (int rc = ready_fail(ctx, ctx->ready.upload(ready_env(ctx), n, task_id, task_priority, task_rq, sorted != 0))) return rc;
    ctx->scan.columns_changed();
    return 0;
}); }

int hqtick_run_resident(hqtick_ctx *ctx, const hqtick_snapshot *snapshot, hqtick_result *out) { return with_audit(ctx, [&]() -> int {
    if (!ctx || !out) return HQTICK_E_INVALID;
    return run_tick(ctx, snapshot, out, true);
}); }

uint64_t hqtick_ready_count(const hqtick_ctx *ctx) { return ctx && ctx->ready.resident() ? ctx->ready.live() : 0; }

int hqtick_ready_consume_last(hqtick_ctx *ctx) { return with_audit(ctx, [&]() -> int {
    if (!ctx) return HQTICK_E_INVALID;
    if (!ctx->ready.resident()) return fail(ctx, HQTICK_E_INVALID, "no resident ready set");
    if (ledger_pending_live(ctx)) {
        HQ_HIP(hipSetDevice(ctx->device));
        if (int rc = ledger_fail(ctx, ctx->asg.apply_tick(ledger_env(ctx)))) {
            ctx->asg.on = false;
            ctx->err += " (the assignment ledger is switched off: upload the worker set and enable it again)";
            return rc;
        }
    }
    if (!ctx->ready.selection_pending()) {
        if (!ctx->ready.compact_due()) return 0;
        HQ_HIP(hipSetDevice(ctx->device));
        return ready_fail(ctx, ctx->ready.compact(ready_env(ctx)));
    }
    if (!ctx->ready.selection_valid()) return fail(ctx, HQTICK_E_INVALID, "hqtick_ready_consume_last needs a preceding hqtick_run_resident");
    HQ_HIP(hipSetDevice(ctx->device));
    if (int rc = map_fail(ctx, ctx->map.replay_selection(ctx->stream, hqmap::REPLAY_TOMBSTONE, ctx->ready.cols(), ctx->scan, ctx->ready.selected_count()))) return rc;
    return ready_fail(ctx, ctx->ready.consumed(ready_env(ctx)));
}); }

int hqtick_ready_remove(hqtick_ctx *ctx, uint64_t n, const uint64_t *task_id) { return with_audit(ctx, [&]() -> int {
    if (!ctx || (n && !task_id)) return HQTICK_E_INVALID;
    if (!ctx->ready.resident()) return fail(ctx, HQTICK_E_INVALID, "no resident ready set");
    if (n == 0 || ctx->ready.cols().n == 0) return 0;
    if (n > 0x7FFFFFFFull) return fail(ctx, HQTICK_E_CAPACITY, "more than 2^31 - 1 ids in one delta (the count of removed tasks is the int return value)");
    HQ_HIP(hipSetDevice(ctx->device));
    return ready_fail(ctx, ctx->ready.remove(ready_env(ctx), n, task_id));
}); }

int hqtick_ready_add_stage(hqtick_ctx *ctx, uint64_t n, uint64_t **task_id, uint64_t **task_priority, uint32_t **task_rq) {
    if (!ctx || !task_id || !task_priority || !task_rq) return HQTICK_E_INVALID;
    if (!ctx->ready.resident()) return fail(ctx, HQTICK_E_INVALID, "no resident ready set (hqtick_upload_ready with n = 0 creates an empty one)");
    if (n > 0xFFFFFFFFull) return fail(ctx, HQTICK_E_CAPACITY, "more than 2^32 ids in one delta");
    HQ_HIP(hipSetDevice(ctx->device));
    return ready_fail(ctx, ctx->ready.stage(n, task_id, task_priority, task_rq));
}

int hqtick_ready_add_staged(hqtick_ctx *ctx, uint64_t n) { return with_audit(ctx, [&]() -> int {
    if (!ctx) return HQTICK_E_INVALID;
    if (!ctx->ready.resident()) return fail(ctx, HQTICK_E_INVALID, "no resident ready set (hqtick_upload_ready with n = 0 creates an empty one)");
    return ready_fail(ctx, ctx->ready.add_staged(ready_env(ctx), n));
}); }

int hqtick_ready_add_packed(hqtick_ctx *ctx, uint64_t n, uint32_t n_id_runs, const uint64_t *id_run_start, const uint32_t *id_run_len, const uint32_t *id_off, uint32_t n_prio_runs, const uint64_t *prio_run_value, const uint32_t *prio_run_len, const uint16_t *task_rq) { return with_audit(ctx, [&]() -> int {
    if (!ctx) return HQTICK_E_INVALID;
    if (!ctx->ready.resident()) return fail(ctx, HQTICK_E_INVALID, "no resident ready set (hqtick_upload_ready with n = 0 creates an empty one)");
    if (n == 0) return 0;
    if (n > 0xFFFFFFFFull) return fail(ctx, HQTICK_E_CAPACITY, "more than 2^32 ids in one delta");
    if (!n_id_runs || !n_prio_runs || !id_run_start || !id_run_len || !prio_run_value || !prio_run_len || !task_rq) return fail(ctx, HQTICK_E_INVALID, "hqtick_ready_add_packed: null array");
    uint64_t tot = 0; for (uint32_t r = 0; r < n_id_runs; r++) { if (!id_run_len[r]) return fail(ctx, HQTICK_E_INVALID, "hqtick_ready_add_packed: empty id run"); tot += id_run_len[r]; }
    if (tot != n) return fail(ctx, HQTICK_E_INVALID, "hqtick_ready_add_packed: the id runs do not add up to n");
    tot = 0; for (uint32_t r = 0; r < n_prio_runs; r++) { if (!prio_run_len[r]) return fail(ctx, HQTICK_E_INVALID, "hqtick_ready_add_packed: empty priority run"); tot += prio_run_len[r]; }
    if (tot != n) return fail(ctx, HQTICK_E_INVALID, "hqtick_ready_add_packed: the priority runs do not add up to n");
    HQ_HIP(hipSetDevice(ctx->device));
    return ready_fail(ctx, ctx->ready.add_packed(ready_env(ctx), n, n_id_runs, id_run_start, id_run_len, id_off, n_prio_runs, prio_run_value, prio_run_len, task_rq));
}); }

int hqtick_ready_add(hqtick_ctx *ctx, uint64_t n, const uint64_t *task_id, const uint64_t *task_priority, const uint32_t *task_rq) { return with_audit(ctx, [&]() -> int {
    if (!ctx || (n && (!task_id || !task_priority || !task_rq))) return HQTICK_E_INVALID;
    if (!ctx->ready.resident()) return fail(ctx, HQTICK_E_INVALID, "no resident ready set (hqtick_upload_ready with n = 0 creates an empty one)");
    if (n == 0) return 0;
    uint64_t *hi = nullptr, *hp = nullptr; uint32_t *hq = nullptr;
    if (int rc = hqtick_ready_add_stage(ctx, n, &hi, &hp, &hq)) return rc;
    memcpy(hi, task_id, n * 8); memcpy(hp, task_priority, n * 8); memcpy(hq, task_rq, n * 4);
    return hqtick_ready_add_staged(ctx, n);
}); }

namespace {
int graph_fail(hqtick_ctx *ctx, int rc) { ctx->err = ctx->graph.err; return rc; }
int graph_pre(hqtick_ctx *ctx) {
    if (!ctx->ready.resident()) return fail(ctx, HQTICK_E_INVALID, "no resident ready set (hqtick_upload_ready with n = 0 creates an empty one)");
    if (hipSetDevice(ctx->device) != hipSuccess) return fail(ctx, HQTICK_E_DEVICE, "hipSetDevice");
    return 0;
}
}

int hqtick_graph_add_tasks(hqtick_ctx *ctx, uint64_t n, const uint64_t *task_id, const uint64_t *task_priority, const uint32_t *task_rq, const uint32_t *dep_off, const uint64_t *dep_task_id) { return with_audit(ctx, [&]() -> int {
    if (!ctx || (n && (!task_id || !task_priority || !task_rq))) return HQTICK_E_INVALID;
    if (n && dep_off && dep_off[n] && !dep_task_id) return HQTICK_E_INVALID;
    if (int rc = graph_pre(ctx)) return rc;
    int r = ctx->graph.add(n, task_id, task_priority, task_rq, dep_off, dep_task_id, ctx->stream);
    if (r < 0) return graph_fail(ctx, r);
    if (r > 0) { if (int rc = ready_fail(ctx, ctx->ready.add_device(ready_env(ctx), ctx->graph.out_id(), ctx->graph.out_prio(), ctx->graph.out_rq(), (uint32_t)r))) return rc; }
// ... 560 lines not shown
int hqtick_debug_order_view(hqtick_ctx *ctx, uint32_t n_requests, uint32_t counts[4], uint32_t *perm, uint32_t *inv, uint32_t *lrank, uint64_t cap_slots, uint32_t *run_rq,
                            uint32_t *run_start, uint32_t *run_rank, uint64_t *run_prio, uint32_t cap_runs) {
    if (!ctx || !counts) return HQTICK_E_INVALID;
    if (!ctx->ready.resident()) return fail(ctx, HQTICK_E_INVALID, "no resident ready set (hqtick_upload_ready)");
    HQ_HIP(hipSetDevice(ctx->device));
    if (!ctx->view_hooks) {
        ctx->view_hooks = new ViewHooks();
        if (int rc = ctx->view_hooks->scan.init()) { delete ctx->view_hooks; ctx->view_hooks = nullptr; return fail(ctx, rc, "creating the view sub-context failed"); }
    }
    ViewHooks *v = ctx->view_hooks;
    const hqready::Cols cols = ctx->ready.cols(); const uint64_t N = cols.n;
    v->valid = false; v->rq_copy = false;
    for (int i = 0; i < 4; i++) counts[i] = 0;
    Scan sc;
    hqscan::Env env{}; env.stream = ctx->stream;
    if (int rc = v->scan.view(env, cols, n_requests, &sc)) return fail(ctx, rc, v->scan.err);
    const uint32_t nr = (uint32_t)sc.run_cnt.size(), n = nr ? sc.run_start.back() + sc.run_cnt.back() : 0u;
    if ((nr != 0) != v->scan.last_view().valid) return fail(ctx, HQTICK_E_DEVICE, "ordered view: the run table and the debug record disagree");
    counts[0] = n; counts[1] = nr; counts[2] = sc.L; counts[3] = v->scan.last_view().passes;
    if (n > cap_slots || N > cap_slots || nr > cap_runs) return fail(ctx, HQTICK_E_CAPACITY, "hqtick_debug_order_view: output arrays too small");
    if (n) {
        if (perm) HQ_HIP(hipMemcpy(perm, v->scan.perm(), (size_t)n * 4, hipMemcpyDeviceToHost));
        if (inv) HQ_HIP(hipMemcpy(inv, v->scan.inv(), (size_t)N * 4, hipMemcpyDeviceToHost));
        if (lrank) HQ_HIP(hipMemcpy(lrank, v->scan.level_ranks(N), (size_t)N * 4, hipMemcpyDeviceToHost));
        const hqscan::OrderTabLayout tl = hqscan::order_tab_layout(n);
        const uint8_t *hh = v->scan.run_table();
        if (run_rq) memcpy(run_rq, hh + tl.o_rq, (size_t)nr * 4);
        if (run_start) memcpy(run_start, hh + tl.o_st, (size_t)nr * 4);
        if (run_rank) memcpy(run_rank, hh + tl.o_rk, (size_t)nr * 4);
        if (run_prio) memcpy(run_prio, hh + tl.o_pr, (size_t)nr * 8);
    }
    v->ids = cols.id; v->N = N; v->Q = n_requests; v->n_live = n;
    v->run_off = std::move(sc.run_off); v->run_start = std::move(sc.run_start); v->run_rank = std::move(sc.run_level);
    v->valid = true;
    return 0;
}

namespace {
ViewHooks *debug_view_of(hqtick_ctx *ctx) {
    ViewHooks *v = ctx->view_hooks;
    if (!v || !v->valid || !ctx->ready.resident() || v->ids != ctx->ready.cols().id || v->N != ctx->ready.cols().n) return nullptr;
    return v;
}
}

int hqtick_debug_order_select(hqtick_ctx *ctx, const uint32_t *rq_sel_base, const uint32_t *q_tnc, uint32_t n_sel, int mark_mode, uint64_t *sel_task, uint32_t *sel_rank,
                              uint32_t *rq_after, uint32_t *err) {
    if (!ctx || !rq_sel_base || !q_tnc || !sel_task || !sel_rank || !err || mark_mode < 0 || mark_mode > 3) return HQTICK_E_INVALID;
    ViewHooks *v = debug_view_of(ctx);
    if (!v) return fail(ctx, HQTICK_E_INVALID, "hqtick_debug_order_select: no view of the current ready set (hqtick_debug_order_view)");
    const uint32_t Q = v->Q, n = v->n_live, nr = (uint32_t)v->run_start.size();
    const uint64_t N = v->N;
    if (Q == 0 || n_sel == 0 || n == 0) return fail(ctx, HQTICK_E_INVALID, "hqtick_debug_order_select: nothing to select from");
    if (rq_sel_base[0] != 0 || rq_sel_base[Q] != n_sel) return fail(ctx, HQTICK_E_INVALID, "hqtick_debug_order_select: rq_sel_base does not span [0, n_sel]");
    for (uint32_t q = 0; q < Q; q++) {
        if (rq_sel_base[q] > rq_sel_base[q + 1]) return fail(ctx, HQTICK_E_INVALID, "hqtick_debug_order_select: rq_sel_base not monotone");
        const uint32_t take = rq_sel_base[q + 1] - rq_sel_base[q], nw = q_tnc[q] >> 16, c = q_tnc[q] & 0xFFFFu;
        if (!q_tnc[q]) continue;
        if (nw == 0) return fail(ctx, HQTICK_E_INVALID, "hqtick_debug_order_select: worker-major form without workers");
        for (uint32_t p = 0; p < take && p < nw * c; p++)
            if ((uint64_t)(p % nw) * c + p / nw >= take) return fail(ctx, HQTICK_E_INVALID, "hqtick_debug_order_select: a worker-major destination leaves its request's range");
    }
    if (mark_mode == 2 && !v->rq_copy) return fail(ctx, HQTICK_E_INVALID, "hqtick_debug_order_select: restore needs the copy a consume left");
    HQ_HIP(hipSetDevice(ctx->device));
    std::vector<uint32_t> tab;
    tab.insert(tab.end(), rq_sel_base, rq_sel_base + Q + 1);
    tab.insert(tab.end(), v->run_off.begin(), v->run_off.end());
    tab.insert(tab.end(), q_tnc, q_tnc + Q);
    tab.insert(tab.end(), v->run_start.begin(), v->run_start.end());
    tab.insert(tab.end(), v->run_rank.begin(), v->run_rank.end());
    if (!v->d_map.ensure(tab.size() * 4 + 16) || !v->d_sel_task.ensure((size_t)n_sel * 8 + 16) || !v->d_sel_rank.ensure((size_t)n_sel * 4 + 16) || !v->d_rq.ensure(N * 4 + 8))
        return fail(ctx, HQTICK_E_DEVICE, "hipMalloc view selection");
    HQ_HIP(hipMemcpy(v->d_map.p, tab.data(), tab.size() * 4, hipMemcpyHostToDevice));
    uint32_t *derr = v->scan.select_err_dev();
    HQ_HIP(hipMemsetAsync(derr, 0, 4, ctx->stream));
    HQ_HIP(hipMemsetAsync(v->d_sel_task.p, 0xFF, (size_t)n_sel * 8, ctx->stream));
    HQ_HIP(hipMemsetAsync(v->d_sel_rank.p, 0xFF, (size_t)n_sel * 4, ctx->stream));
    if (mark_mode != 2) { HQ_HIP(hipMemcpyAsync(v->d_rq.p, ctx->ready.cols().rq, N * 4, hipMemcpyDeviceToDevice, ctx->stream)); v->rq_copy = true; }
    const uint32_t *d = v->d_map.as<uint32_t>();
    hqk::OrderSelect os{};
    os.task_id = ctx->ready.cols().id; os.perm = v->scan.perm(); os.n_live = n; os.Q = Q; os.n_runs = nr;
    os.rq_sel_base = d; os.run_off = d + (Q + 1); os.q_tnc = d + 2 * (size_t)(Q + 1); os.run_start = os.q_tnc + Q; os.run_rank = os.run_start + nr;
    os.sel_task = v->d_sel_task.as<uint64_t>(); os.sel_rank = v->d_sel_rank.as<uint32_t>(); os.err = derr;
    if (mark_mode) { os.mark_rq = v->d_rq.as<uint32_t>(); os.mark_value = mark_mode == 2 ? 0u : hqk::RQ_TOMBSTONE; os.mark_and_select = mark_mode == 3 ? 1u : 0u; }
    HQ_HIP(hqk::order_select(os, n_sel, ctx->stream));
    HQ_HIP(hipStreamSynchronize(ctx->stream));
    HQ_HIP(hipMemcpy(sel_task, v->d_sel_task.p, (size_t)n_sel * 8, hipMemcpyDeviceToHost));
    HQ_HIP(hipMemcpy(sel_rank, v->d_sel_rank.p, (size_t)n_sel * 4, hipMemcpyDeviceToHost));
    if (rq_after) HQ_HIP(hipMemcpy(rq_after, v->d_rq.p, N * 4, hipMemcpyDeviceToHost));
    HQ_HIP(hipMemcpy(err, derr, 4, hipMemcpyDeviceToHost));
    return 0;
}

int hqtick_debug_order_rank_of(hqtick_ctx *ctx, const uint64_t *want, uint32_t n_want, uint32_t *out_rq, uint32_t *out_pos) {
    if (!ctx || (n_want && (!want || !out_rq || !out_pos))) return HQTICK_E_INVALID;
    ViewHooks *v = debug_view_of(ctx);
    if (!v) return fail(ctx, HQTICK_E_INVALID, "hqtick_debug_order_rank_of: no view of the current ready set (hqtick_debug_order_view)");
    if (n_want == 0) return 0;
    if (v->n_live == 0) { for (uint32_t i = 0; i < n_want; i++) out_rq[i] = out_pos[i] = 0xFFFFFFFFu; return 0; }
    HQ_HIP(hipSetDevice(ctx->device));
    if (!v->d_want.ensure((size_t)n_want * 16 + 16)) return fail(ctx, HQTICK_E_DEVICE, "hipMalloc wanted ids");
    uint8_t *dw = v->d_want.as<uint8_t>();
    HQ_HIP(hipMemcpy(dw, want, (size_t)n_want * 8, hipMemcpyHostToDevice));
    HQ_HIP(hqk::order_rank_of(ctx->ready.cols().id, ctx->ready.cols().rq, v->N, v->scan.inv(), reinterpret_cast<const uint64_t *>(dw), n_want,
                              reinterpret_cast<uint32_t *>(dw + (size_t)n_want * 8), reinterpret_cast<uint32_t *>(dw + (size_t)n_want * 12), ctx->stream));
    HQ_HIP(hipStreamSynchronize(ctx->stream));
    HQ_HIP(hipMemcpy(out_rq, dw + (size_t)n_want * 8, (size_t)n_want * 4, hipMemcpyDeviceToHost));
    HQ_HIP(hipMemcpy(out_pos, dw + (size_t)n_want * 12, (size_t)n_want * 4, hipMemcpyDeviceToHost));
    return 0;
}

void hqtick_debug_set_block_emulation(int on, uint32_t budget) { g_block_emulation = on; if (budget) g_block_budget = budget; }
void hqtick_debug_last_blocks(uint32_t *n_emulated, uint32_t *n_host) { if (n_emulated) *n_emulated = g_last_blocks_device; if (n_host) *n_host = g_last_blocks_host; }

int hqtick_debug_block_solve_host(uint32_t n_cols, uint32_t n_resources, const uint32_t *ent_off, const uint32_t *ent_res, const uint8_t *ent_kind, const uint64_t *ent_amount,
                                  const uint32_t *weight, const double *pool, uint32_t n_classes, const uint64_t *free_, const uint64_t *total, const uint64_t *elig,
                                  uint32_t budget, uint32_t *x, uint32_t *status, uint32_t *steps) {
    hqblock::ColTable ct{n_cols, n_resources, ent_off, ent_res, ent_kind, ent_amount, weight, pool, nullptr, 0};
    hqblock::ClassTable cl{n_classes, free_, total, elig};
    hqblock::Output out{x, status, steps, nullptr};
    EmulatedBlocks emu(budget ? budget : 4096);
    return emu.solve(ct, cl, out) ? 0 : HQTICK_E_DEVICE;
}

static uint32_t *heap_storage(void *vec, size_t words) { auto *v = static_cast<std::vector<uint32_t> *>(vec); v->assign(words, 0); return v->data(); }
static int host_stages(const hqtick_config *config, const hqtick_snapshot *s, const uint8_t *vflags, const uint32_t *vtmc, uint32_t n_levels, const uint64_t *levels,
                       const uint32_t *hist, bool with_plan, const uint32_t *retr_key, const uint32_t *retr_rank, hqtick_result *out, std::string *err) {
    if (!config || !s || !out) return HQTICK_E_INVALID;
    struct KeepError { hqtick_ctx *c; std::string *e; ~KeepError() { if (e) *e = c->err; } };
    static thread_local hqtick_ctx *holder = nullptr;
    if (!holder) holder = new hqtick_ctx();
    hqtick_ctx *ctx = holder;
    KeepError keep{ctx, err};
    ctx->cfg = *config; ctx->err.clear();
    if (int rc = validate(ctx, s, false)) return rc;
    WorkerEval ev; ev.flags = vflags; ev.tmc = vtmc;
    hqhost::Problem pb;
    fill_problem(pb, s, ctx->cfg, ev);
    Scan sc; sc.Q = s->n_requests; sc.L = n_levels; sc.G = n_levels * s->n_requests;
    sc.levels.assign(levels, levels + n_levels); sc.hist.assign(hist, hist + (size_t)n_levels * s->n_requests);
    runs_from_hist(sc);
    std::vector<hqhost::QueueLevels> qlv = queue_levels(sc, s);
    std::vector<hqhost::TaskBatch> batches = hqhost::create_task_batches(pb, qlv);
    memset(out, 0, sizeof(*out));
    g_last_mn_rq.clear(); g_last_mn_off.assign(1, 0); g_last_mn_worker.clear();
    export_batches(ctx, batches, out);
    EmulatedBlocks emu(g_block_budget);
    emu.corrupt_mode = g_corrupt_mode; emu.corrupt_class = g_corrupt_class; emu.corrupt_fill = g_corrupt_fill;
    if (g_block_emulation) { pb.blocks = &emu; pb.block_min_classes = 1; }
    pb.block_verify = g_block_verify; pb.tick_seq = g_tick_seq; pb.memo = g_memo;
    hqprice::EmulatedSweeper pemu;
    if (g_price_emulation) { pemu.fail_at = g_price_fault; pemu.budget = g_block_budget; if (g_price_min_cols) pemu.min_cols = g_price_min_cols; pb.pricer = &pemu; }
    hqhost::Counts cnt;
    if (g_xfn && g_xworld > 1) {
        struct FnExchange : hqprice::Exchange { bool allgather(const void *snd, void *rcv, size_t bytes) override { return g_xfn(g_xuser, snd, rcv, bytes) == 0; } } xch;
        xch.rank = g_xrank; xch.world = g_xworld;
        ShardedBlocks sh_blocks(emu, xch, g_xmin_classes);
        hqprice::ShardedSweeper sh_sweeps(pemu, xch, g_xmin_blocks);
        if (pb.blocks) pb.blocks = &sh_blocks;
        if (pb.pricer) pb.pricer = &sh_sweeps;
        cnt = hqhost::run_scheduling_solver(pb, batches);
        g_xcalls = (uint32_t)xch.n_calls;
    } else cnt = hqhost::run_scheduling_solver(pb, batches);
    if (cnt.error) return fail(ctx, cnt.error, cnt.errmsg);
    g_last_guard[0] = cnt.blocks_verified; g_last_guard[1] = cnt.blocks_mismatch; g_last_guard[2] = cnt.blocks_rejected;
    g_last_memo = cnt.blocks_memo;
    g_last_blocks_device = cnt.blocks_device; g_last_blocks_host = cnt.blocks_host; g_last_price_sweeps = (uint32_t)cnt.price_sweeps; g_last_price_rounds = (uint32_t)cnt.price_rounds;
    g_last_stage_us[0] = cnt.t_classify_us; g_last_stage_us[1] = cnt.t_blocks_us; g_last_stage_us[2] = cnt.t_decode_us;
    for (size_t i = 0; i < cnt.mn_rq.size(); i++)
        for (auto &set : cnt.mn_sets[i]) { g_last_mn_rq.push_back(cnt.mn_rq[i]); g_last_mn_worker.insert(g_last_mn_worker.end(), set.begin(), set.end()); g_last_mn_off.push_back((uint32_t)g_last_mn_worker.size()); }
    hqmap::HostResult &hr = ctx->map.res;
    hr.cnt_rq.clear(); hr.cnt_variant.clear(); hr.cnt_worker.clear(); hr.cnt_value.clear();
    cnt.pairs();
    for (size_t k = 0; k < cnt.keys.size(); k++)
        for (auto &wc : cnt.per_key[k]) { hr.cnt_rq.push_back(cnt.keys[k].first); hr.cnt_variant.push_back(cnt.keys[k].second); hr.cnt_worker.push_back(wc.first); hr.cnt_value.push_back(wc.second); }
    out->is_optimal = cnt.is_optimal; out->is_canonical = cnt.is_canonical && cnt.is_optimal;
    out->status = cnt.is_optimal ? HQTICK_DONE : (cnt.empty() ? HQTICK_NO_PROGRESS : HQTICK_NEED_MORE_COMPUTE);
    if (with_plan) {
        static thread_local std::vector<uint32_t> tables;
        hqmap::Plan &ps = ctx->map.plan;
        hqmap::PlanIn in{};
        in.sc = &sc; in.cnt = &cnt; in.s = s; in.rqs = pb.rqs.data(); in.variants = pb.variants.data();
        in.proactive_filling_reserve = config->proactive_filling_reserve; in.proactive_filling_max = config->proactive_filling_max; in.flags = config->flags;
        in.shard_count = 1; in.retr_key = retr_key; in.retr_rank = retr_rank; in.transpose_on = transpose_enabled();
        for (size_t g = 0; g < sc.hist.size(); g++) in.N += sc.hist[g];
        in.storage = heap_storage; in.user = &tables;
        const char *why = nullptr; int rc;
        if ((rc = hqmap::plan_keys(ps, hr, in, &why)) || (rc = hqmap::plan_redirects(ps, hr, in, &why)) || (rc = hqmap::plan_prefill(ps, hr, in, &why)) ||
            (rc = hqmap::plan_outputs(ps, hr, in, &why)))
            return fail(ctx, rc, why);
        hqmap::assemble_host_part(ps, hr, in);
        out->rec_off = hr.rec_off.data(); out->retract_off = hr.retract_off.data(); out->retract_task = hr.retract_task.data();
        out->n_redirects = (uint32_t)hr.red_task.size(); out->redirect_task = hr.red_task.data(); out->redirect_worker = hr.red_worker.data();
        out->redirect_variant = hr.red_variant.data(); out->redirect_kind = hr.red_kind.data(); out->new_free = hr.new_free.data();
    }
    out->n_counts = (uint32_t)hr.cnt_rq.size(); out->count_rq = hr.cnt_rq.data(); out->count_variant = hr.cnt_variant.data();
    out->count_worker = hr.cnt_worker.data(); out->count_value = hr.cnt_value.data();
    return out->status;
}
int hqtick_debug_host_stages(const hqtick_config *config, const hqtick_snapshot *s, const uint8_t *vflags, const uint32_t *vtmc, uint32_t n_levels,
                             const uint64_t *levels, const uint32_t *hist, hqtick_result *out) {
    return host_stages(config, s, vflags, vtmc, n_levels, levels, hist, false, nullptr, nullptr, out, nullptr);
}
int hqtick_debug_host_plan(const hqtick_config *config, const hqtick_snapshot *s, const uint8_t *vflags, const uint32_t *vtmc, uint32_t n_levels, const uint64_t *levels,
                           const uint32_t *hist, const uint32_t *retracting_key, const uint32_t *retracting_rank, hqtick_result *out, const char **error) {
    static thread_local std::string text;
    if (error) *error = "";
    if (s && s->n_retracting && (!retracting_key || !retracting_rank)) return HQTICK_E_INVALID;
    const int rc = host_stages(config, s, vflags, vtmc, n_levels, levels, hist, true, retracting_key, retracting_rank, out, &text);
    if (rc < 0 && error) *error = text.c_str();
    return rc;
}

int hqtick_debug_host_query(const hqtick_config *config, const hqtick_snapshot *s, const hqtick_query_workers *fake, const uint8_t *vflags, const uint32_t *vtmc,
                            const uint8_t *fake_vflags, const uint32_t *fake_vtmc, uint32_t n_levels, const uint64_t *levels, const uint32_t *hist,
                            hqtick_query_result *out) {
    if (!config || !s || !fake || !out) return HQTICK_E_INVALID;
    static thread_local hqtick_ctx *holder = nullptr;
    if (!holder) holder = new hqtick_ctx();
    hqtick_ctx *ctx = holder;
    ctx->cfg = *config;
    if (int rc = validate(ctx, s, false)) return rc;
    const uint32_t R = s->n_resources, Q = s->n_requests;
    WorkerEval ev; ev.flags = vflags; ev.tmc = vtmc;
    hqhost::Problem pb;
    fill_problem(pb, s, ctx->cfg, ev);
    hqhost::WorkerSet fw;
    fw.n = fake->n_workers; fw.R = R; fw.id = fake->worker_id; fw.total = fake->worker_total; fw.free_ = fake->worker_total;
    fw.remaining_ns = fake->worker_remaining_ns; fw.min_util = fake->worker_min_utilization; fw.flags = nullptr; fw.group = nullptr;
    fw.vflags = fake_vflags; fw.vtmc = fake_vtmc; fw.n_variant_slots = Q ? s->rq_variant_off[Q] : 0;
    fw.blocked.assign(fw.n, {});
    hqhost::group_equal_rows(fw, true);
    pb.custom = &fw;
    Scan sc; sc.Q = Q; sc.L = n_levels; sc.G = n_levels * Q;
    sc.levels.assign(levels, levels + n_levels); sc.hist.assign(hist, hist + (size_t)n_levels * Q);
    runs_from_hist(sc);
    std::vector<hqhost::QueueLevels> qlv = queue_levels(sc, s);
    std::vector<hqhost::TaskBatch> batches = hqhost::create_task_batches(pb, qlv);
    EmulatedBlocks emu(g_block_budget);
    if (g_block_emulation) { pb.blocks = &emu; pb.block_min_classes = 1; }
    hqhost::Counts cnt = hqhost::run_scheduling_solver(pb, batches);
    if (cnt.error) return fail(ctx, cnt.error, cnt.errmsg);
    ctx->q_loaded.assign(fake->n_workers, 0);
    for (auto &k : cnt.per_key) for (auto &wc : k) if (wc.second > 0) ctx->q_loaded[wc.first] = 1;
    out->n_workers = fake->n_workers; out->is_loaded = ctx->q_loaded.data(); out->is_optimal = cnt.is_optimal;
    return 0;
}

#endif

int hqtick_set_shard(hqtick_ctx *ctx, uint32_t shard_index, uint32_t shard_count) {
    if (!ctx) return HQTICK_E_INVALID;
    if (shard_count > 1 && shard_index >= shard_count) return fail(ctx, HQTICK_E_INVALID, "shard_index >= shard_count");
    if (shard_count > 1 && ctx->asg.on) return fail(ctx, HQTICK_E_UNSUPPORTED, "hqtick_set_shard: the assignment ledger is on (hqtick_assigned_disable first)");
    ctx->shard_index = shard_count > 1 ? shard_index : 0; ctx->shard_count = shard_count > 1 ? shard_count : 1;
    return 0;
}

int hqtick_set_exchange(hqtick_ctx *ctx, hqtick_exchange_fn fn, void *user) {
    if (!ctx) return HQTICK_E_INVALID;
    ctx->xfn = fn; ctx->xuser = fn ? user : nullptr;
    return 0;
}

size_t hqtick_sink_bytes(uint32_t n_workers, uint32_t capacity_records) {
    size_t o_task = (16 + (size_t)(n_workers + 1) * 4 + 7) & ~(size_t)7;
    return (o_task + (size_t)capacity_records * 10 + 15) & ~(size_t)15;
}

uint32_t hqtick_sink_capacity_records(uint32_t n_workers, size_t capacity_bytes) {
    size_t fixed = hqtick_sink_bytes(n_workers, 0);
    if (capacity_bytes < fixed) return 0;
    size_t cap = (capacity_bytes - fixed) / 10;
    while (cap && hqtick_sink_bytes(n_workers, (uint32_t)cap) > capacity_bytes) cap--;
    return cap > 0xFFFFFFFFull ? 0xFFFFFFFFu : (uint32_t)cap;
}

int hqtick_set_record_sink(hqtick_ctx *ctx, void *device_ptr, size_t capacity_bytes) {
    if (!ctx) return HQTICK_E_INVALID;
    if (device_ptr && (reinterpret_cast<uintptr_t>(device_ptr) & 15)) return fail(ctx, HQTICK_E_INVALID, "record sink must be 16-byte aligned");
    ctx->sink = device_ptr; ctx->sink_bytes = device_ptr ? capacity_bytes : 0;
    return 0;
}

#ifdef HQTICK_TEST_HOOKS
int hqtick_time_kernel(hqtick_ctx *ctx, int which, int iters, double *avg_us) {
    if (!ctx || !avg_us || iters <= 0) return HQTICK_E_INVALID;
    if (!ctx->ready.selection_valid() || !ctx->ready.resident()) return fail(ctx, HQTICK_E_INVALID, "hqtick_time_kernel needs a preceding hqtick_run_resident tick that placed tasks");
    const hqmap::Mapper::Last last = ctx->map.last_selection();
    if (last.ordered) return fail(ctx, HQTICK_E_INVALID, "hqtick_time_kernel times the dense scan: the last tick took the ordered view");
    HQ_HIP(hipSetDevice(ctx->device));
    const hqready::Cols cols = ctx->ready.cols(); const hqk::WaveGeom g = last.geom;
    if (which == 2) {
        double sum = 0.0; int cnt = 0;
        for (int i = 0; i < iters; i++) {
            hqk::time_next_launch(ctx->ev[2], ctx->ev[3]);
            HQ_HIP(hqk::empty_like_level_hist(g, ctx->stream));
            HQ_HIP(hipStreamSynchronize(ctx->stream));
            const double us_ = elapsed_us(ctx->ev[2], ctx->ev[3]);
            if (us_ >= 0) { sum += us_; cnt++; }
        }
        *avg_us = cnt ? sum / cnt : 0.0;
        return 0;
    }
    const bool as_graph = getenv("HQTICK_KTIME_GRAPH") != nullptr;
    if (as_graph) HQ_HIP(hipStreamBeginCapture(ctx->stream, hipStreamCaptureModeThreadLocal));
    else HQ_HIP(hipEventRecord(ctx->ev[10], ctx->stream));
    for (int i = 0; i < iters; i++) {
        if (which == 0) { if (int rc = scan_fail(ctx, ctx->scan.relaunch_level_hist(ctx->stream, cols, last.L, last.Q, g))) return rc; }
        else if (which == 1) { if (int rc = map_fail(ctx, ctx->map.replay_selection(ctx->stream, hqmap::REPLAY_TIMED, cols, ctx->scan, ctx->ready.selected_count()))) return rc; }
        else return fail(ctx, HQTICK_E_INVALID, "which: 0 = level_hist, 1 = select_scatter, 2 = empty kernel of level_hist's grid");
    }
    if (as_graph) {
        hipGraph_t gr = nullptr; hipGraphExec_t ge = nullptr;
        HQ_HIP(hipStreamEndCapture(ctx->stream, &gr));
        HQ_HIP(hipGraphInstantiate(&ge, gr, nullptr, nullptr, 0));
// ... 146 lines not shown
```

hyperqueue_amd/csrc/map.cpp:

```cpp
#include "map.h"

#include <chrono>

namespace hqmap {

#define HQ_HIP(call) do { hipError_t e_ = (call); if (e_ != hipSuccess) return fail(HQTICK_E_DEVICE, std::string(#call) + ": " + hipGetErrorString(e_)); } while (0)
#define HQ_HIP_TIMED(call) do { hipError_t e_ = (call); hqk::take_launch_timer(); if (e_ != hipSuccess) return fail(HQTICK_E_DEVICE, std::string(#call) + ": " + hipGetErrorString(e_)); } while (0)
#define HQ_HIP_LAST(call, launched) do { hipError_t e_ = (call); (launched) = hqk::take_launch_timer().stop == nullptr && e.wait_on_kernel; if (e_ != hipSuccess) return fail(HQTICK_E_DEVICE, std::string(#call) + ": " + hipGetErrorString(e_)); } while (0)

namespace {
double now_us() { return std::chrono::duration<double, std::micro>(std::chrono::steady_clock::now().time_since_epoch()).count(); }
double elapsed_us(hipEvent_t a, hipEvent_t b) {
    float ms = 0;
    if (hipEventElapsedTime(&ms, a, b) == hipSuccess) return (double)ms * 1000.0;
    (void)hipGetLastError();
    return -1.0;
}
}

void Timeline::mark() const { if (*n < 32) tl[(*n)++] = now_us() - t0; }

void Mapper::release() {
    hqbuf::DevBuf *bufs[] = {&d_sel_task, &d_sel_level, &d_map, &d_tsweep, &d_bits, &d_pre};
    for (hqbuf::DevBuf *b : bufs) b->release();
    h_plan.release(); h_rec.release(); h_sinkhdr.release(); h_k5a.release();
}

uint32_t *Mapper::plan_storage(void *mapper, size_t words) {
    Mapper *m = static_cast<Mapper *>(mapper);
    return m->h_plan.ensure(words * 4 + 64) ? m->h_plan.as<uint32_t>() : nullptr;
}

int Mapper::launch_sweep_early(const Env &e) {
    const Plan &ps = plan; const uint32_t nkeys = ps.nkeys;
    sweep_launched = false;
    if (nkeys == 0 || ps.n_bit_words == 0 || ps.max_nk > hqk::SWEEP_MAX_WORKERS) return 0;
    if (ps.n_tr == nkeys) { sweep_launched = true; return 0; }
    if (sweep_inflight) { HQ_HIP(hipStreamSynchronize(e.stream)); sweep_inflight = false; }
    if (!h_k5a.ensure(sweep_words(nkeys, ps.ord_cnt.size()) * 4 + 64) || !d_tsweep.ensure((size_t)ps.key_t_off[nkeys] * 4 + 16) || !d_bits.ensure((size_t)ps.n_bit_words * 8 + 16) ||
        !d_pre.ensure((size_t)ps.n_bit_words * 4 + 16))
        return fail(HQTICK_E_DEVICE, "hipMalloc mapping");
    const SweepTables t = pack_sweep_keys(h_k5a.as<uint32_t>(), ps);
    const uint32_t *d = h_k5a.dev<uint32_t>();
    hqk::MapKeys mk{};
    mk.n_keys = nkeys; mk.key_t_off = d + t.o_toff; mk.key_ord_off = d + t.o_ordoff; mk.key_bits_off = d + t.o_boff; mk.ord_cnt = d + t.o_ord; mk.key_tr = d + t.o_tr;
    mk.t_sweep = d_tsweep.as<uint32_t>(); mk.bits = d_bits.as<uint64_t>(); mk.pre = d_pre.as<uint32_t>();
    if (e.timing) hqk::time_next_launch(e.k5a_start, e.k5a_stop);
    HQ_HIP_TIMED(hqk::sweep_bits(mk, ps.max_count, ps.max_nk, e.stream));
    sweep_launched = true; sweep_inflight = true;
    return 0;
}

int Mapper::check_capacity(bool ordered) {
    const Plan &ps = plan;
    if (hqk::expand_mapping_lds(ps.max_items, ps.nkeys, ps.compact ? ps.max_out : 0, ps.may_reorder, ordered) > 150 * 1024) return fail(HQTICK_E_CAPACITY, "a worker receives more tasks in one tick than the mapping kernel stages in LDS");
    if (ps.max_nk > hqk::SWEEP_MAX_WORKERS) return fail(HQTICK_E_CAPACITY, "more than 24576 workers share one (request, variant) placement: beyond the round-robin kernel's LDS staging");
    return 0;
}

int Mapper::phase_c(const Env &e, const PhaseC &pc) {
    Plan &ps = plan; const hqscan::Scan &sc = *pc.sc; const hqhost::Counts &cnt = *pc.in->cnt; const hqtick_snapshot *s = pc.in->s;
    const uint32_t W = s->n_workers, Q = s->n_requests, nkeys = ps.nkeys, n_sel = ps.n_sel, n_rec = ps.n_rec;
    const bool compact = ps.compact;
    t_ = Timings{};
    size_t n_mn_ids = 0; for (auto &sets : cnt.mn_sets) n_mn_ids += sets.size();
    delta16 = compact && (e.flags & HQTICK_FLAG_COMPACT_DELTA16) != 0;
    if (compact) {
        o_rs = delta16 ? (size_t)n_rec * 8 : (((size_t)n_rec * 4 + 7) & ~(size_t)7); o_rf = o_rs + (size_t)W * 8;
        o_rv = o_rk = 0; o_mn = (o_rf + (size_t)n_rec * (delta16 ? 16 : 12) + 7) & ~(size_t)7;
    } else { o_rv = (size_t)n_rec * 8; o_rk = o_rv + n_rec; o_mn = (o_rk + n_rec + 7) & ~(size_t)7; }
    o_fl = o_mn + n_mn_ids * 8;
    const size_t rec_bytes = o_fl + 64;
    if (!h_rec.ensure(rec_bytes)) return fail(HQTICK_E_DEVICE, "hipHostMalloc records");
    uint64_t *mn_ids = reinterpret_cast<uint64_t *>(h_rec.as<uint8_t>() + o_mn);
    if (n_sel) {
        if (!d_sel_task.ensure((size_t)n_sel * 8) || !d_sel_level.ensure((size_t)n_sel * (sc.ordered ? 4 : 2) + 4))
            return fail(HQTICK_E_DEVICE, "hipMalloc selection");
        const size_t o_wpos = 0, o_wcnt = (size_t)nkeys * W, o_pflj = (size_t)2 * nkeys * W;
        const SmallTables t = pack_small(h_plan.as<uint32_t>(), ps, sc, pc.ledger_pfq_rq);
        const size_t plan_words = t.words;
        if (plan_words * 4 + 16 > h_plan.cap) return fail(HQTICK_E_DEVICE, "mapping plan larger than its buffer");
        if (!d_map.ensure(plan_words * 4 + 16) ||
            !d_tsweep.ensure((size_t)ps.key_t_off[nkeys] * 4 + 16) || !d_bits.ensure((size_t)ps.n_bit_words * 8 + 16) || !d_pre.ensure((size_t)ps.n_bit_words * 4 + 16))
            return fail(HQTICK_E_DEVICE, "hipMalloc mapping");
        e.tl.mark();
        const uint32_t *d = d_map.as<uint32_t>();
        hqk::MapKeys mk{};
        mk.n_keys = nkeys; mk.key_rq = d + t.o_rq; mk.key_variant = reinterpret_cast<const uint8_t *>(d + t.o_var); mk.key_seg_start = d + t.o_seg;
        mk.key_ord_off = d + t.o_ordoff; mk.ord_cnt = d + t.o_ord; mk.key_t_off = d + t.o_toff; mk.key_bits_off = d + t.o_boff; mk.key_tr = d + t.o_tr;
        mk.t_sweep = d_tsweep.as<uint32_t>(); mk.bits = d_bits.as<uint64_t>(); mk.pre = d_pre.as<uint32_t>();
        mk.wpos = d + o_wpos; mk.wcnt = d + o_wcnt; mk.rq_sel_base = d + t.o_base; mk.rq_pf_start = d + t.o_pfs; mk.rq_pf_n = d + t.o_pfn;
        mk.n_holes = (uint32_t)ps.holes.size(); mk.holes = reinterpret_cast<const uint64_t *>(d + t.o_holes);
        mk.n_pfq = ps.n_pfq; mk.pfq_src = d + t.o_pqs; mk.pfq_size = d + t.o_pqz; mk.pfl_j = d + o_pflj; mk.out_off = d + t.o_out;
        uint32_t *flags = reinterpret_cast<uint32_t *>(h_rec.as<uint8_t>() + o_fl);
        flags[0] = 0;
        pc.ready->selected(n_sel);
        const hqready::Cols cols = pc.ready->cols();
        const uint64_t N = cols.n;
        if (pc.saved_rq)
            HQ_HIP(hipMemcpyAsync(pc.saved_rq, cols.rq, N * 4, hipMemcpyDeviceToDevice, e.stream));
        last_geom = sc.geom; last_L = sc.L; last_Q = Q; last_G = sc.G; last_tb = t.o_tb; last_plan_bytes = plan_words * 4;
        last_ordered = sc.ordered;
        if (sc.ordered) {
            HQ_HIP(hqk::copy_pinned_to_hbm(h_plan.dev<void>(), d_map.p, plan_words * 4, e.stream));
            hqk::OrderSelect os{};
            os.task_id = cols.id; os.perm = pc.scan->perm(); os.n_live = sc.run_cnt.empty() ? 0u : sc.run_start.back() + sc.run_cnt.back(); os.Q = Q;
            os.n_runs = (uint32_t)sc.run_cnt.size(); os.rq_sel_base = d + t.o_base; os.run_off = d + t.o_roff; os.run_start = d + t.o_rst; os.run_rank = d + t.o_rrk; os.q_tnc = d + t.o_qtnc;
            os.sel_task = d_sel_task.as<uint64_t>(); os.sel_rank = d_sel_level.as<uint32_t>(); os.err = pc.scan->select_err_dev();
            last_os = os;
            if (pc.consume_in_tick) { os.mark_rq = cols.rq; os.mark_value = hqk::RQ_TOMBSTONE; os.mark_and_select = 1; }
            if (e.timing) hqk::time_next_launch(e.k4_start, e.k4_stop);
            HQ_HIP_TIMED(hqk::order_select(os, n_sel, e.stream));
        } else {
            if (e.timing) hqk::time_next_launch(e.k4_start, e.k4_stop);
            HQ_HIP_TIMED(hqk::select_scatter(cols.id, pc.scan->group_keys(), N, Q, sc.G, sc.geom, pc.scan->slice_table(), h_plan.as<uint32_t>() + t.o_tb,
                                d + t.o_tb, d_sel_task.as<uint64_t>(), d_sel_level.as<uint16_t>(), h_plan.dev<void>(), d_map.p, plan_words * 4,
                                pc.consume_in_tick ? cols.rq : nullptr, e.stream, pc.consume_in_tick ? 1u : 0u));
        }
        if (pc.consume_in_tick) pc.ready->consumed_in_tick();
        if (!sweep_launched && ps.n_tr < nkeys) {
            if (e.timing) hqk::time_next_launch(e.k5a_start, e.k5a_stop);
            HQ_HIP_TIMED(hqk::sweep_bits(mk, ps.max_count, ps.max_nk, e.stream));
        }
        uint8_t *drec = h_rec.dev<uint8_t>();
        uint64_t *k_task = reinterpret_cast<uint64_t *>(drec); uint8_t *k_var = drec + o_rv, *k_kind = drec + o_rk;
        if (e.sink) {
            const uint32_t cap = hqtick_sink_capacity_records(W, e.sink_bytes);
            if (n_rec > cap || hqtick_sink_bytes(W, cap) > e.sink_bytes) return fail(HQTICK_E_CAPACITY, "record sink too small for this tick");
            uint8_t *sk = reinterpret_cast<uint8_t *>(e.sink);
            const size_t so_off = 16, so_task = (so_off + (size_t)(W + 1) * 4 + 7) & ~(size_t)7, so_var = so_task + (size_t)cap * 8, so_kind = so_var + cap;
            std::vector<uint32_t> &hdr = ps.sink_hdr; hdr.assign(4 + W + 1, 0);
            hdr[0] = n_rec; hdr[1] = cnt.checksum(); hdr[2] = HQTICK_SINK_MAGIC; hdr[3] = cap;
            memcpy(hdr.data() + 4, ps.out_off.data(), (size_t)(W + 1) * 4);
            if (!h_sinkhdr.ensure(hdr.size() * 4)) return fail(HQTICK_E_DEVICE, "hipHostMalloc sink header");
            memcpy(h_sinkhdr.p, hdr.data(), hdr.size() * 4);
            HQ_HIP(hipMemcpyAsync(sk, h_sinkhdr.p, hdr.size() * 4, hipMemcpyHostToDevice, e.stream));
            k_task = reinterpret_cast<uint64_t *>(sk + so_task); k_var = sk + so_var; k_kind = sk + so_kind;
        }
        hqk::time_next_launch(e.timing ? e.k5b_start : nullptr, e.k5b_stop);
        hqk::CompactOut co{};
        if (compact) co = hqk::CompactOut{reinterpret_cast<uint32_t *>(drec), reinterpret_cast<uint2 *>(drec + o_rs), reinterpret_cast<uint32_t *>(drec + o_rf),
                                          delta16 ? reinterpret_cast<uint16_t *>(drec) : nullptr};
        hqk::Stage stg = pc.stage;
        if (stg.task) stg.pfq_rq = d_map.as<uint32_t>() + t.o_pqr;
        bool expand_is_last = false;
        if (sc.ordered) HQ_HIP_LAST(hqk::expand_mapping_wide(mk, W, d_sel_task.as<uint64_t>(), d_sel_level.as<uint32_t>(), ps.max_items, k_task, k_var, k_kind,
                                                       reinterpret_cast<uint32_t *>(drec + o_fl), co, ps.max_out, ps.may_reorder, e.stream, stg), expand_is_last);
        else HQ_HIP_LAST(hqk::expand_mapping(mk, W, d_sel_task.as<uint64_t>(), d_sel_level.as<uint16_t>(), Q, ps.max_items, k_task, k_var, k_kind,
                            reinterpret_cast<uint32_t *>(drec + o_fl), co, ps.max_out, ps.may_reorder, e.stream, stg), expand_is_last);
        if (!cnt.mn_rq.empty()) expand_is_last = false;
        if (sc.ordered) {
            HQ_HIP(hipMemcpyAsync(pc.scan->select_err_host(), pc.scan->select_err_dev(), 4, hipMemcpyDeviceToHost, e.stream));
            expand_is_last = false;
        }
        {
            size_t pos = 0;
            for (size_t i = 0; i < cnt.mn_rq.size(); i++) {
                size_t n = cnt.mn_sets[i].size();
                HQ_HIP(hipMemcpyAsync(mn_ids + pos, d_sel_task.as<uint64_t>() + ps.rq_sel_base[cnt.mn_rq[i]] + ps.mn_first[i], n * 8, hipMemcpyDeviceToHost, e.stream));
                pos += n;
            }
        }
        e.tl.mark();
        assemble_host_part(ps, res, *pc.in);
        if (expand_is_last) HQ_HIP(hipEventSynchronize(e.k5b_stop)); else HQ_HIP(hipStreamSynchronize(e.stream));
        sweep_inflight = false;
        if (flags[0]) return fail(HQTICK_E_CAPACITY, "mapping kernel capacity exceeded");
        if (sc.ordered && *pc.scan->select_err_host()) return fail(HQTICK_E_DEVICE, "ordered view: the selection left its request's segment");
        if (e.timing) { t_.select_us = elapsed_us(e.k4_start, e.k4_stop); t_.sweep_us = elapsed_us(e.k5a_start, e.k5a_stop); t_.other_us = elapsed_us(e.k5b_start, e.k5b_stop); }
    }
    if (!n_sel) {
        pc.ready->selected(0);
        assemble_host_part(ps, res, *pc.in);
    }
    if (!n_sel && e.sink) {
        if (hqtick_sink_bytes(W, 0) > e.sink_bytes) return fail(HQTICK_E_CAPACITY, "record sink too small for this tick");
        std::vector<uint32_t> &hdr = ps.sink_hdr; hdr.assign(4 + W + 1, 0);
        hdr[1] = cnt.checksum(); hdr[2] = HQTICK_SINK_MAGIC; hdr[3] = hqtick_sink_capacity_records(W, e.sink_bytes);
        HQ_HIP(hipMemcpy(e.sink, hdr.data(), hdr.size() * 4, hipMemcpyHostToDevice));
    }
    return 0;
}

void Mapper::export_result(const Env &e, const hqhost::Counts &cnt, hqtick_result *out) {
    const uint64_t *mn_ids = reinterpret_cast<const uint64_t *>(h_rec.as<uint8_t>() + o_mn);
    res.mn_task.clear(); res.mn_off.assign(1, 0); res.mn_worker.clear(); res.mn_rq.clear();
    {
        size_t pos = 0;
        for (size_t i = 0; i < cnt.mn_rq.size(); i++) for (auto &set : cnt.mn_sets[i]) {
            res.mn_task.push_back(mn_ids[pos++]); res.mn_rq.push_back(cnt.mn_rq[i]);
            for (uint32_t w : set) res.mn_worker.push_back(w);
            res.mn_off.push_back((uint32_t)res.mn_worker.size());
        }
    }
    out->n_counts = (uint32_t)res.cnt_rq.size(); out->count_rq = res.cnt_rq.data(); out->count_variant = res.cnt_variant.data();
    out->count_worker = res.cnt_worker.data(); out->count_value = res.cnt_value.data();
    out->rec_off = res.rec_off.data();
    const uint8_t *hb = h_rec.as<uint8_t>();
    if (plan.compact && plan.n_sel) {
        out->run_span = reinterpret_cast<const hqtick_run_span *>(hb + o_rs);
        if (delta16) { out->rec_delta16 = reinterpret_cast<const uint16_t *>(hb); out->runs16 = reinterpret_cast<const hqtick_rec_run16 *>(hb + o_rf); }
        else { out->rec_task_lo = reinterpret_cast<const uint32_t *>(hb); out->runs = reinterpret_cast<const hqtick_rec_run *>(hb + o_rf); }
    } else if (!e.sink) { out->rec_task = reinterpret_cast<const uint64_t *>(hb); out->rec_variant = hb + o_rv; out->rec_kind = hb + o_rk; }
    out->retract_off = res.retract_off.data(); out->retract_task = res.retract_task.data();
    out->n_redirects = (uint32_t)res.red_task.size(); out->redirect_task = res.red_task.data(); out->redirect_worker = res.red_worker.data(); out->redirect_variant = res.red_variant.data(); out->redirect_kind = res.red_kind.data();
    out->n_mn = (uint32_t)res.mn_task.size(); out->mn_task = res.mn_task.data(); out->mn_worker_off = res.mn_off.data(); out->mn_worker = res.mn_worker.data();
    out->new_free = res.new_free.data();
}

int Mapper::replay_selection(hipStream_t st, Replay mode, const hqready::Cols &cols, const hqscan::Scanner &scan, uint32_t n_sel, hqbuf::PinBuf *scratch) {
    const uint32_t *d = d_map.as<uint32_t>();
    if (last_ordered) {
        if (mode == REPLAY_TIMED) return fail(HQTICK_E_INVALID, "the timed replay is the dense selection's");
        hqk::OrderSelect os = last_os;
        os.mark_rq = cols.rq; os.mark_value = mode == REPLAY_TOMBSTONE ? hqk::RQ_TOMBSTONE : 0; os.mark_and_select = 0;
        HQ_HIP(hqk::order_select(os, n_sel, st));
        if (mode == REPLAY_RESTORE) HQ_HIP(hipStreamSynchronize(st));
        return 0;
    }
    switch (mode) {
    case REPLAY_TOMBSTONE:
        HQ_HIP(hqk::select_scatter(cols.id, scan.group_keys(), cols.n, last_Q, last_G, last_geom, scan.slice_table(), h_plan.as<uint32_t>() + last_tb, d + last_tb,
                                   d_sel_task.as<uint64_t>(), d_sel_level.as<uint16_t>(), nullptr, nullptr, 0, cols.rq, st));
        return 0;
    case REPLAY_RESTORE: {
        if (!last_Q || !scratch || !scratch->ensure(64)) return fail(HQTICK_E_DEVICE, "no restore of the selection");
        uint32_t *cntp = scratch->as<uint32_t>();
        cntp[0] = 0;
        HQ_HIP(hqk::ready_restore_consumed(scan.group_keys(), cols.rq, cols.n, last_Q, scratch->dev<uint32_t>(), st));
        HQ_HIP(hipStreamSynchronize(st));
        return cntp[0] <= n_sel ? 0 : fail(HQTICK_E_DEVICE, "the restore found more tombstones than the tick selected");
    }
    case REPLAY_TIMED:
        HQ_HIP(hqk::select_scatter(cols.id, scan.group_keys(), cols.n, last_Q, last_G, last_geom, scan.slice_table(), h_plan.as<uint32_t>() + last_tb, d + last_tb,
                                   d_sel_task.as<uint64_t>(), d_sel_level.as<uint16_t>(), h_plan.dev<void>(), d_map.p, last_plan_bytes, nullptr, st));
        return 0;
    }
    return HQTICK_E_INVALID;
}

}
```

hyperqueue_amd/csrc/map.h:

```cpp
#pragma once
#include <hip/hip_runtime.h>

#include <cstdint>
#include <string>

#include "../../include/hqtick.h"
#include "devbuf.h"
#include "kernels.h"
#include "map_core.h"
#include "ready.h"
#include "scan.h"

namespace hqmap {

struct Timeline {
    double t0; double *tl; int *n;
    void mark() const;
};

struct Env {
    hipStream_t stream;
    hipEvent_t k4_start, k4_stop, k5a_start, k5a_stop, k5b_start, k5b_stop;
    bool timing, wait_on_kernel;
    uint32_t flags;
    void *sink; size_t sink_bytes;
    uint32_t shard_index, shard_count;
    Timeline tl;
};
struct PhaseC {
    const hqscan::Scan *sc; hqscan::Scanner *scan; hqready::ReadySet *ready;
    const PlanIn *in;
    bool consume_in_tick;
    bool ledger_pfq_rq;
    uint32_t *saved_rq;
    hqk::Stage stage;
};
struct Timings { double select_us = -1, sweep_us = -1, other_us = -1; };
enum Replay { REPLAY_TOMBSTONE, REPLAY_RESTORE, REPLAY_TIMED };

class Mapper {
  public:
    std::string err;
    Plan plan;
    HostResult res;
    void release();
    static uint32_t *plan_storage(void *mapper, size_t words);
    int launch_sweep_early(const Env &e);
    int check_capacity(bool ordered);
    int phase_c(const Env &e, const PhaseC &pc);
    void export_result(const Env &e, const hqhost::Counts &cnt, hqtick_result *out);
    const Timings &timings() const { return t_; }
    int replay_selection(hipStream_t st, Replay mode, const hqready::Cols &cols, const hqscan::Scanner &scan, uint32_t n_sel, hqbuf::PinBuf *scratch = nullptr);
    struct Last { bool ordered; hqk::WaveGeom geom; uint32_t L, Q, G; };
    Last last_selection() const { return Last{last_ordered, last_geom, last_L, last_Q, last_G}; }

  private:
    int fail(int code, const std::string &m) { err = m; return code; }

    hqbuf::DevBuf d_sel_task, d_sel_level, d_map, d_tsweep, d_bits, d_pre;
    hqbuf::PinBuf h_plan, h_rec, h_sinkhdr, h_k5a;
    bool sweep_inflight = false;
    bool sweep_launched = false;
    size_t o_rv = 0, o_rk = 0, o_mn = 0, o_fl = 0, o_rs = 0, o_rf = 0; bool delta16 = false;
    bool last_ordered = false; hqk::OrderSelect last_os{};
    hqk::WaveGeom last_geom{}; uint32_t last_L = 0, last_Q = 0, last_G = 0; size_t last_tb = 0, last_plan_bytes = 0;
    Timings t_;
};

}
```

hyperqueue_amd/csrc/milp.cpp:

```cpp
#include "milp.h"
#include "lp_tab.h"
#include "price.h"

#include <algorithm>
#include <chrono>
#include <cstdio>
#include <cstdlib>
#include <cmath>
#include <climits>
#include <cstring>
#include <functional>
#include <numeric>
#include <string>
#include <unordered_map>

namespace hqmilp {
namespace {

using namespace lp;

struct DSUlite {
    std::vector<int> p;
    explicit DSUlite(int n) : p(n) { std::iota(p.begin(), p.end(), 0); }
    int find(int a) { while (p[a] != a) { p[a] = p[p[a]]; a = p[a]; } return a; }
// ... 1152 lines not shown
        std::vector<double> cur(bx);
        work_limit = work + std::max(2.0e8, work);
        Tab warm; warm.init(&R2, c, lb, ub); warm.deadline = deadline;
        if (solve_counted(warm) != LP_OPT) { xout = cur; return 1; }
        {
            double probes = 0.0; for (int j = 0; j < n; j++) if (cur[j] > lb[j]) probes += 1.0;
            if (work + probes * (double)(warm.ma + 1) * (double)warm.width() > work_limit) { canonical_done = false; xout = cur; return 1; }
        }
        for (int j = n - 1; j >= 0; j--) {
            double lo = lb[j], hi = cur[j];
            bool first = true;
            while (lo < hi) {
                double mid = first ? hi - 1 : std::floor((lo + hi) / 2);
                first = false;
                {
                    const double loss = warm.loss_if_ub(j, mid);
                    if (loss >= INF || warm.objective() - loss < best - 2.0 * tol - 1e-12) { lo = mid + 1; continue; }
                }
                Tab t = warm;
                work += (double)(warm.ma + 1) * (double)warm.width();
                t.set_ub(j, mid);
                std::vector<double> sol;
                bool ok = dfs_feas(t, sol);
                lp_iters += t.iters - warm.iters;
                if (timed_out) { xout = cur; canonical_done = false; return 1; }
                if (ok) { cur = sol; hi = sol[j]; } else lo = mid + 1;
            }
            if (tracing && !in_lns && cur[j] > lb[j]) fprintf(stderr, "[milp]   t=%.6fs column %d settled at %.0f (nodes %ld)\n", wall() - t_begin, j, hi, nodes);
            const bool unmoved = std::fabs(warm.x[j] - hi) <= FEAS_TOL;
            warm.set_lb(j, hi); warm.set_ub(j, hi);
            if (unmoved) continue;
            if (solve_counted(warm) != LP_OPT) {
                std::vector<double> flb(lb), fub(ub);
                for (int k = n - 1; k >= j; k--) flb[k] = fub[k] = cur[k];
                warm = Tab(); warm.init(&R2, c, flb, fub); warm.deadline = deadline;
                if (solve_counted(warm) != LP_OPT) { xout = cur; return 1; }
            }
        }
        xout = cur;
        trace("tie-break done");
        return 1;
    }
};

void order_by_cost_desc(const double *c, int n, std::vector<int> &out) {
    out.resize((size_t)n);
    if (n < 4096) {
        std::vector<std::pair<double, int>> key((size_t)n);
        for (int j = 0; j < n; j++) key[(size_t)j] = {-c[j], j};
        std::sort(key.begin(), key.end());
        for (int j = 0; j < n; j++) out[(size_t)j] = key[(size_t)j].second;
        return;
    }
    std::vector<uint64_t> ka((size_t)n), kb((size_t)n); std::vector<int> ib((size_t)n);
    for (int j = 0; j < n; j++) {
        double v = c[j] == 0.0 ? 0.0 : c[j];
        uint64_t u; memcpy(&u, &v, 8);
        u = (u >> 63) ? ~u : (u | 0x8000000000000000ull);
        ka[(size_t)j] = ~u;
        out[(size_t)j] = j;
    }
    const int BITS = 11, NB = 1 << BITS;
    uint32_t cnt[NB];
    uint64_t *src = ka.data(), *dst = kb.data(); int *isrc = out.data(), *idst = ib.data();
    for (int sh = 0; sh < 64; sh += BITS) {
        memset(cnt, 0, sizeof cnt);
        for (int j = 0; j < n; j++) cnt[(src[j] >> sh) & (NB - 1)]++;
        if (cnt[(src[0] >> sh) & (NB - 1)] == (uint32_t)n) continue;
        uint32_t run = 0; for (int d = 0; d < NB; d++) { const uint32_t t = cnt[d]; cnt[d] = run; run += t; }
        for (int j = 0; j < n; j++) { const uint32_t p = cnt[(src[j] >> sh) & (NB - 1)]++; dst[p] = src[j]; idst[p] = isrc[j]; }
        std::swap(src, dst); std::swap(isrc, idst);
    }
    if (isrc != out.data()) memcpy(out.data(), isrc, (size_t)n * sizeof(int));
}

struct DSU {
    std::vector<int> p;
    explicit DSU(int n) : p(n) { std::iota(p.begin(), p.end(), 0); }
    int find(int a) { while (p[a] != a) { p[a] = p[p[a]]; a = p[a]; } return a; }
    void unite(int a, int b) { a = find(a); b = find(b); if (a != b) p[std::max(a, b)] = std::min(a, b); }
};

bool sparse_greedy(const Model &mdl, const std::vector<double> &ub, std::vector<double> &x) {
    const int n = mdl.ncols(), m = mdl.nrows();
    std::vector<int> coff(n + 1, 0), crow; std::vector<double> ccoef;
    for (int k = 0; k < (int)mdl.rcol.size(); k++) coff[mdl.rcol[k] + 1]++;
    for (int j = 0; j < n; j++) coff[j + 1] += coff[j];
    crow.resize(mdl.rcol.size()); ccoef.resize(mdl.rcol.size());
    { std::vector<int> cur(coff.begin(), coff.end() - 1);
      for (int i = 0; i < m; i++) for (int k = mdl.roff[i]; k < mdl.roff[i + 1]; k++) { int j = mdl.rcol[k]; crow[cur[j]] = i; ccoef[cur[j]++] = mdl.rcoef[k]; } }
    x.assign(n, 0.0);
    for (int i = 0; i < m; i++) {
        if (mdl.rtype[i] == ROW_MAX || mdl.rhs[i] <= 1e-9) continue;
        for (int k = mdl.roff[i]; k < mdl.roff[i + 1]; k++) {
            int j = mdl.rcol[k];
            if (mdl.kind[j] == COL_BOOL && mdl.obj[j] == 0.0 && mdl.rcoef[k] >= mdl.rhs[i] - 1e-9) { x[j] = 1.0; break; }
        }
    }
    std::vector<double> act(m, 0.0);
    for (int i = 0; i < m; i++) { double a = 0.0; for (int k = mdl.roff[i]; k < mdl.roff[i + 1]; k++) a += mdl.rcoef[k] * x[mdl.rcol[k]]; act[i] = a; }
    auto row_ok = [&](int i, double a) {
        const double tol = 1e-7 * (1.0 + std::fabs(mdl.rhs[i]));
        return mdl.rtype[i] == ROW_MAX ? a <= mdl.rhs[i] + tol : (mdl.rtype[i] == ROW_MIN ? a >= mdl.rhs[i] - tol : std::fabs(a - mdl.rhs[i]) <= tol);
    };
    for (int i = 0; i < m; i++) if (!row_ok(i, act[i])) return false;
    std::vector<int> order;
    order_by_cost_desc(mdl.obj.data(), n, order);
    for (int pass = 0; pass < 64; pass++) {
        bool changed = false;
        for (int j : order) {
            if (mdl.obj[j] <= 0.0) break;
            double step = ub[j] - x[j];
            for (int k = coff[j]; k < coff[j + 1] && step >= 1.0; k++) {
                const int i = crow[k]; const double a = ccoef[k];
                if (mdl.rtype[i] == ROW_EQ) { step = 0.0; break; }
                if (a > 0.0 && mdl.rtype[i] == ROW_MAX) { const double room = mdl.rhs[i] - act[i]; if (room < 0.5 * a) { step = 0.0; break; } step = std::min(step, std::floor(room / a + 1e-9)); }
                else if (a < 0.0 && mdl.rtype[i] == ROW_MIN) { const double room = act[i] - mdl.rhs[i]; if (room < -0.5 * a) { step = 0.0; break; } step = std::min(step, std::floor(room / -a + 1e-9)); }
            }
            if (step < 1.0) continue;
            x[j] += step; changed = true;
            for (int k = coff[j]; k < coff[j + 1]; k++) act[crow[k]] += ccoef[k] * step;
        }
        bool dropped = false;
        for (int j = 0; j < n; j++) {
            if (mdl.kind[j] != COL_BOOL || mdl.obj[j] != 0.0 || x[j] != 1.0) continue;
            bool ok = true;
            for (int k = coff[j]; k < coff[j + 1] && ok; k++) ok = row_ok(crow[k], act[crow[k]] - ccoef[k]);
            if (!ok) continue;
            x[j] = 0.0; dropped = true;
            for (int k = coff[j]; k < coff[j + 1]; k++) act[crow[k]] -= ccoef[k];
        }
        if (!changed && !dropped) break;
        if (!dropped) break;
    }
    return true;
}

}

void columns_by_cost_desc(const double *c, int n, std::vector<int> &out) { order_by_cost_desc(c, n, out); }

thread_local int g_fast_path = -1;
void set_fast_path(int on) { g_fast_path = on; }
thread_local int g_block_runs = -1;
thread_local Probe *g_probe = nullptr;
void set_block_runs(int on) { g_block_runs = on; }
bool block_runs_on() {
    static const bool env_on = !(getenv("HQMILP_BLOCK_RUNS") && atoi(getenv("HQMILP_BLOCK_RUNS")) == 0);
    return g_block_runs < 0 ? env_on : g_block_runs != 0;
}

const double ROW_TOL = 1e-6;

namespace {
bool solve_fast(const Model &mdl_in, double time_limit_s, double rel_gap, hqprice::Sweeper *sweeper, const double ts0, Result &res_out) {
    static const bool tracing_solve = getenv("HQMILP_TRACE") != nullptr;
    auto tmark = [&](const char *what) { if (tracing_solve && mdl_in.ncols() > 1000) fprintf(stderr, "[milp] solve(): %s at %.3f ms\n", what, (wall() - ts0) * 1e3); };
    static const bool fast_env = !(getenv("HQMILP_FAST") && atoi(getenv("HQMILP_FAST")) == 0);
    const bool fast_on = g_fast_path < 0 ? fast_env : g_fast_path != 0;
    const int FAST_MIN_COLS = 2048;
    const bool hints_there = (int)mdl_in.col_group.size() == mdl_in.ncols() && (int)mdl_in.row_lhs.size() == mdl_in.nrows() && (int)mdl_in.row_lhs_len.size() == mdl_in.nrows();
    const bool takes_it = fast_on && sweeper && rel_gap > 0.0 && mdl_in.ncols() >= FAST_MIN_COLS && mdl_in.ncols() >= (int)sweeper->min_cols && hints_there && (int)mdl_in.start.size() != mdl_in.ncols();
    if (takes_it || (g_probe && hints_there)) {
        const int n = mdl_in.ncols(), m = mdl_in.nrows();
        hqprice::ModelView mv;
        mv.n = n; mv.m = m; mv.obj = mdl_in.obj.data(); mv.kind = mdl_in.kind.data(); mv.rtype = mdl_in.rtype.data(); mv.rhs = mdl_in.rhs.data();
        mv.roff = mdl_in.roff.data(); mv.rcol = mdl_in.rcol.data(); mv.rcoef = mdl_in.rcoef.data(); mv.col_group = mdl_in.col_group.data();
        mv.row_implied = (int)mdl_in.row_implied.size() == m ? mdl_in.row_implied.data() : nullptr; mv.row_lhs = mdl_in.row_lhs.data(); mv.row_lhs_len = mdl_in.row_lhs_len.data(); mv.list_off = mdl_in.list_off.data(); mv.list_col = mdl_in.list_col.data(); mv.n_lists = (int)mdl_in.list_off.size() - 1;
        if ((int)mdl_in.row_block.size() == m && (int)mdl_in.col_ub.size() == n) { mv.row_block = mdl_in.row_block.data(); mv.col_ub = mdl_in.col_ub.data(); }
        static_assert(sizeof(Model::BlockRun) == 7 * sizeof(int32_t), "ModelView::block_runs reads seven int32 per run");
        if (!mdl_in.block_runs.empty()) { mv.block_runs = &mdl_in.block_runs[0].col0; mv.n_block_runs = (int)mdl_in.block_runs.size(); }
        mv.run_stats = g_probe ? &g_probe->covered : nullptr; mv.tables_digest = g_probe ? &g_probe->tables : nullptr;
        if (!takes_it) { hqprice::flatten_for_probe(mv, tracing_solve); return false; }
        double cost_scale = 1.0;
        const double tf0 = wall();
        hqprice::Answer pa = hqprice::solve_model(mv, rel_gap, time_limit_s, ts0 + (time_limit_s > 0 ? time_limit_s : 1e18), tracing_solve, *sweeper, &cost_scale);
        if (tracing_solve) fprintf(stderr, "[milp] fast path: ran %d (%s) sweeps %u rounds %u bound %.9f point %.9f, %.3f ms of which %.3f ms inside the sweeps\n", (int)pa.ran, pa.why, pa.sweeps, pa.rounds, pa.ran ? pa.bound : -1.0, pa.x.empty() ? -1.0 : pa.x_value, (wall() - tf0) * 1e3, sweeper->stat_sweep_us / 1e3);
        if (pa.ran && (int)pa.x.size() == n && pa.bound * (1.0 + 1e-9) + 1e-12 <= pa.x_value + rel_gap * std::fabs(pa.x_value)) {
            bool ok = true;
            for (int j = 0; j < n && ok; j++) { const double v = pa.x[(size_t)j]; if (v < -1e-9 || std::fabs(v - std::floor(v + 0.5)) > 1e-9 || (mdl_in.kind[j] == COL_BOOL && v > 1.0 + 1e-9)) ok = false; }
            std::vector<double> lhs_act; std::vector<uint8_t> lhs_seen;
            for (int i = 0; i < m && ok; i++) {
                double a = 0.0;
                int k0 = mdl_in.roff[i];
                const int L = mdl_in.row_lhs[i];
                if (L >= 0) {
                    if ((size_t)L >= lhs_seen.size()) { lhs_seen.resize((size_t)L + 1, 0); lhs_act.resize((size_t)L + 1, 0.0); }
                    if (!lhs_seen[(size_t)L]) { double s = 0.0; for (int k = mdl_in.list_off[L]; k < mdl_in.list_off[L + 1]; k++) s += pa.x[(size_t)mdl_in.list_col[k]]; lhs_act[(size_t)L] = s; lhs_seen[(size_t)L] = 1; }
                    a = lhs_act[(size_t)L];
                }
                for (int k = k0; k < mdl_in.roff[i + 1]; k++) a += mdl_in.rcoef[k] * pa.x[(size_t)mdl_in.rcol[k]];
                const double tol = std::max(ROW_TOL, 1e-9 * std::max(1.0, std::fabs(mdl_in.rhs[i])));
                if (mdl_in.rtype[i] != ROW_MIN && a > mdl_in.rhs[i] + tol) ok = false;
                if (mdl_in.rtype[i] != ROW_MAX && a < mdl_in.rhs[i] - tol) ok = false;
            }
            double z_pt = 0.0;
            if (ok) {
                for (int j = 0; j < n; j++) z_pt += mdl_in.obj[j] * std::floor(pa.x[(size_t)j] + 0.5);
                const double zs = cost_scale > 0.0 ? z_pt / cost_scale : z_pt;
                if (!(pa.bound * (1.0 + 1e-9) + 1e-12 <= zs + rel_gap * std::fabs(zs))) ok = false;
            }
            if (ok) {
                Result res;
                res.x = std::move(pa.x);
                for (double &v : res.x) v = std::floor(v + 0.5);
                res.feasible = true; res.optimal = true; res.canonical = false;
                res.n_components = 1; res.nodes = pa.sweeps; res.price_sweeps = (int)pa.sweeps; res.price_rounds = (int)pa.rounds; res.price_total_us = (wall() - tf0) * 1e6;
                res.objective = z_pt;
                tmark("fast path certified");
                res_out = std::move(res);
                return true;
            }
            if (tracing_solve) fprintf(stderr, "[milp] fast path: the certified point fails a row of the model (or its own objective misses the certificate): classic path\n");
        }
    }
    return false;
}
}

static Result solve_classic(const Model &mdl_in, double time_limit_s, bool canonical, double rel_gap, hqprice::Sweeper *sweeper, const double ts0);

Result solve(const Model &mdl_arg, double time_limit_s, bool canonical, double rel_gap, hqprice::Sweeper *sweeper) {
    const double ts_entry = wall();
    { Result r; if (solve_fast(mdl_arg, time_limit_s, rel_gap, sweeper, ts_entry, r)) return r; }
    if (mdl_arg.has_lists()) {
        Model plain = mdl_arg;
        plain.expand_lists();
        return solve_classic(plain, time_limit_s, canonical, rel_gap, sweeper, ts_entry);
    }
    return solve_classic(mdl_arg, time_limit_s, canonical, rel_gap, sweeper, ts_entry);
}

static Result solve_classic(const Model &mdl_in, double time_limit_s, bool canonical, double rel_gap, hqprice::Sweeper *sweeper, const double ts0) {
    static const bool tracing_solve = getenv("HQMILP_TRACE") != nullptr;
    auto tmark = [&](const char *what) { if (tracing_solve && mdl_in.ncols() > 1000) fprintf(stderr, "[milp] solve(): %s at %.3f ms\n", what, (wall() - ts0) * 1e3); };
    Model snapped;
    bool need_snap = false;
    for (size_t k = 0; k < mdl_in.rcoef.size() && !need_snap; k++) {
        if (mdl_in.kind[mdl_in.rcol[k]] != COL_BOOL) continue;
        const double c = mdl_in.rcoef[k], g = std::round(c * 10000.0) / 10000.0;
        if (g != c && std::fabs(g - c) <= ROW_TOL) need_snap = true;
    }
    if (need_snap) {
        snapped = mdl_in;
        for (size_t k = 0; k < snapped.rcoef.size(); k++) {
            if (snapped.kind[snapped.rcol[k]] != COL_BOOL) continue;
            const double c = snapped.rcoef[k], g = std::round(c * 10000.0) / 10000.0;
            if (g != c && std::fabs(g - c) <= ROW_TOL) snapped.rcoef[k] = g;
        }
    }
    {
        const Model &src = need_snap ? snapped : mdl_in;
        const double GRID = 10000.0;
        std::vector<long long> ci;
        std::vector<uint8_t> reach;
        struct Seen { std::vector<long long> ci; double rhs, new_rhs; };
        std::vector<Seen> seen_rows; size_t seen_next = 0; const size_t SEEN_CAP = 8;
        struct Cut { int row; long long d, rhs; };
        std::vector<Cut> cuts; std::vector<long long> cut_d;
        for (int i = 0; i < src.nrows(); i++) {
            if (src.rtype[i] != ROW_MAX) continue;
            const int a = src.roff[i], b = src.roff[i + 1];
            if (b - a < 1 || !(src.rhs[i] > 0.0) || src.rhs[i] > 1e11) continue;
            ci.clear();
            bool ok = true;
            for (int k = a; k < b && ok; k++) {
                const double c = src.rcoef[k] * GRID, r = std::round(c);
                if (!(src.rcoef[k] > 0.0) || r < 1.0 || std::fabs(c - r) > 1e-6 * std::max(1.0, r) || r > 9e15) ok = false; else ci.push_back((long long)r);
            }
            if (!ok) continue;
            double new_rhs;
            const Seen *hit = nullptr;
            for (const Seen &sr : seen_rows) if (sr.rhs == src.rhs[i] && sr.ci == ci) { hit = &sr; break; }
            if (hit) new_rhs = hit->new_rhs;
            else {
                long long g = 0;
                for (long long c : ci) { long long x = c, y = g; while (y) { const long long t = x % y; x = y; y = t; } g = x; }
                const long long cap = (long long)std::floor(src.rhs[i] * GRID + 1e-6);
                long long units = cap / g;
                long long cmin = ci[0]; for (long long c : ci) cmin = std::min(cmin, c);
                if (cmin != g && units <= 65536) {
                    reach.assign((size_t)units + 1, 0); reach[0] = 1;
                    for (long long sidx = 1; sidx <= units; sidx++) for (long long c : ci) { const long long st = c / g; if (st <= sidx && reach[(size_t)(sidx - st)]) { reach[(size_t)sidx] = 1; break; } }
                    while (units > 0 && !reach[(size_t)units]) units--;
                }
                new_rhs = (double)(units * g) / GRID;
                if (seen_rows.size() < SEEN_CAP) seen_rows.push_back({ci, src.rhs[i], new_rhs});
                else { seen_rows[seen_next % SEEN_CAP] = {ci, src.rhs[i], new_rhs}; seen_next++; }
            }
            if (new_rhs < src.rhs[i] - 1e-9) {
                if (!need_snap) { snapped = mdl_in; need_snap = true; }
                snapped.rhs[i] = new_rhs;
            }
            {
                const long long cap_new = (long long)std::llround(new_rhs * GRID);
                long long cmin = ci[0]; for (long long c : ci) cmin = std::min(cmin, c);
                const int CUT_ITEMS = 32;
                if (cap_new / cmin <= CUT_ITEMS && b - a >= 2 && src.ncols() <= 512) {
                    cut_d.assign(ci.begin(), ci.end());
                    std::sort(cut_d.begin(), cut_d.end()); cut_d.erase(std::unique(cut_d.begin(), cut_d.end()), cut_d.end());
                    for (long long d : cut_d) {
                        if (d == cmin && cmin * (cap_new / cmin) == cap_new) { bool all_mult = true; for (long long c : ci) if (c % d) all_mult = false; if (all_mult) continue; }
                        const long long rhs_c = cap_new / d;
                        long long lhs_max = 0; int nz = 0;
                        for (long long c : ci) { if (c / d) nz++; lhs_max += (c / d) * (cap_new / c); }
                        if (nz < 2 || lhs_max <= rhs_c) continue;
                        cuts.push_back({i, d, rhs_c});
                    }
                }
            }
        }
        if (!cuts.empty()) {
            if (!need_snap) { snapped = mdl_in; need_snap = true; }
            snapped.row_implied.resize((size_t)snapped.nrows(), 0);
            for (const auto &cu : cuts) {
                const int a = mdl_in.roff[cu.row], b = mdl_in.roff[cu.row + 1];
                snapped.row_implied.push_back(1);
                snapped.begin_row(ROW_MAX, (double)cu.rhs);
                for (int k = a; k < b; k++) { const long long c = (long long)std::llround(mdl_in.rcoef[k] * GRID) / cu.d; if (c) snapped.term(mdl_in.rcol[k], (double)c); }
                snapped.end_row();
            }
        }
    }
    tmark("presolve done");
    const Model &mdl = need_snap ? snapped : mdl_in;
    Result res;
    int n = mdl.ncols(), m = mdl.nrows();
    res.x.assign(n, 0.0);
    res.feasible = true; res.optimal = true; res.canonical = canonical;
    if (n == 0) return res;
    double deadline = wall() + (time_limit_s > 0 ? time_limit_s : 1e18);

    std::vector<double> ub(n, INF);
    for (int j = 0; j < n; j++) if (mdl.kind[j] == COL_BOOL) ub[j] = 1.0;
    bool chained = false;
    for (int pass = 0; pass < 2 && (pass == 0 || chained); pass++) {
        for (int i = 0; i < m; i++) {
            if (mdl.rtype[i] == ROW_MIN) continue;
            int a = mdl.roff[i], b = mdl.roff[i + 1];
            bool nonneg = true; int neg = -1; double negc = 0;
            for (int k = a; k < b; k++) if (mdl.rcoef[k] < 0) { if (neg >= 0) nonneg = false; neg = mdl.rcol[k]; negc = mdl.rcoef[k]; }
            if (neg < 0) {
                if (mdl.rhs[i] < -1e-9) { res.feasible = false; res.optimal = false; return res; }
                for (int k = a; k < b; k++) if (mdl.rcoef[k] > 0) ub[mdl.rcol[k]] = std::min(ub[mdl.rcol[k]], std::floor(mdl.rhs[i] / mdl.rcoef[k] + 1e-9));
            } else if (nonneg && mdl.rtype[i] == ROW_EQ && mdl.rhs[i] == 0.0) {
                double s = 0; bool fin = true;
                for (int k = a; k < b; k++) if (mdl.rcoef[k] > 0) { if (ub[mdl.rcol[k]] >= INF) fin = false; else s += mdl.rcoef[k] * ub[mdl.rcol[k]]; }
                chained = true;
                if (fin) ub[neg] = std::min(ub[neg], std::floor(s / -negc + 1e-9));
            }
        }
    }
    std::vector<char> capped(n, 0);
    for (int j = 0; j < n; j++) if (ub[j] >= INF) { ub[j] = UB_CAP; capped[j] = 1; }

    tmark("bounds done");
    std::vector<double> hx;
    bool have_hx = false, hx_joined = false;
    auto join_hx = [&]() {
        if (hx_joined) return;
        hx_joined = true;
        have_hx = sparse_greedy(mdl, ub, hx);
        tmark("sparse greedy done");
        if ((int)mdl.start.size() == n) {
            bool ok = true; double zs = 0.0, zh = 0.0;
            for (int j = 0; j < n && ok; j++) { double v = mdl.start[j]; if (v < -1e-9 || v > ub[j] + 1e-9 || std::fabs(v - std::round(v)) > 1e-9) ok = false; zs += mdl.obj[j] * v; }
            for (int i = 0; i < m && ok; i++) {
                double a = 0.0, sc = 0.0;
                for (int k = mdl.roff[i]; k < mdl.roff[i + 1]; k++) { a += mdl.rcoef[k] * mdl.start[mdl.rcol[k]]; sc = std::max(sc, std::fabs(mdl.rcoef[k])); }
                const double tol = 1e-9 * std::max(1.0, sc);
                if (mdl.rtype[i] != ROW_MIN && a > mdl.rhs[i] + tol) ok = false;
                if (mdl.rtype[i] != ROW_MAX && a < mdl.rhs[i] - tol) ok = false;
            }
            if (ok) {
                if (have_hx) for (int j = 0; j < n; j++) zh += mdl.obj[j] * hx[j];
                if (!have_hx || zs > zh) { hx = mdl.start; have_hx = true; }
            }
// ... 128 lines not shown
```

hyperqueue_amd/csrc/milp.h:

```cpp
#pragma once
#include <cstddef>
#include <cstdint>
#include <algorithm>
#include <vector>

namespace hqprice { struct Sweeper; }

namespace hqmilp {

enum { COL_NAT = 0, COL_BOOL = 1 };
enum { ROW_MIN = 0, ROW_MAX = 1, ROW_EQ = 2 };

struct Model {
    std::vector<double> obj;
    std::vector<uint8_t> kind;
    std::vector<uint8_t> rtype;
    std::vector<double> rhs;
    std::vector<int> roff{0};
    std::vector<int> rcol;
    std::vector<double> rcoef;
    std::vector<double> start;
    std::vector<int32_t> col_group;
    std::vector<uint8_t> row_implied;
    std::vector<int32_t> row_lhs, row_lhs_len;
    std::vector<int> list_off{0}, list_col;
    int add_list(const int *cols, size_t n) { list_col.insert(list_col.end(), cols, cols + n); list_off.push_back((int)list_col.size()); return (int)list_off.size() - 2; }
    bool has_lists() const { return list_off.size() > 1; }
    void expand_lists() {
        if (!has_lists()) return;
        const int m = nrows();
        std::vector<int> noff; noff.reserve((size_t)m + 1); noff.push_back(0);
        size_t total = rcol.size();
        for (int i = 0; i < m; i++) if (i < (int)row_lhs.size() && row_lhs[i] >= 0) total += (size_t)(list_off[row_lhs[i] + 1] - list_off[row_lhs[i]]);
        std::vector<int> ncol; std::vector<double> ncoef; ncol.reserve(total); ncoef.reserve(total);
        for (int i = 0; i < m; i++) {
            if (i < (int)row_lhs.size() && row_lhs[i] >= 0) {
                const int l = row_lhs[i];
                ncol.insert(ncol.end(), list_col.begin() + list_off[l], list_col.begin() + list_off[l + 1]);
                ncoef.resize(ncol.size(), 1.0);
            }
            ncol.insert(ncol.end(), rcol.begin() + roff[i], rcol.begin() + roff[i + 1]);
            ncoef.insert(ncoef.end(), rcoef.begin() + roff[i], rcoef.begin() + roff[i + 1]);
            noff.push_back((int)ncol.size());
        }
        roff.swap(noff); rcol.swap(ncol); rcoef.swap(ncoef);
        list_off.assign(1, 0); list_col.clear();
        std::fill(row_lhs.begin(), row_lhs.end(), -1); std::fill(row_lhs_len.begin(), row_lhs_len.end(), 0);
    }
    std::vector<int32_t> row_block;
    std::vector<uint32_t> col_ub;
    struct BlockRun { int32_t col0, row0, term0, n_blocks, n_cols, n_rows, n_terms; };
    std::vector<BlockRun> block_runs;
    int ncols() const { return (int)obj.size(); }
    int nrows() const { return (int)rhs.size(); }
    int add_col(double w, uint8_t k) {
        obj.push_back(w);
        kind.push_back(k);
        return (int)obj.size() - 1;
    }
    void begin_row(uint8_t t, double b) {
        rtype.push_back(t);
        rhs.push_back(b);
    }
    void term(int c, double v) {
        rcol.push_back(c);
        rcoef.push_back(v);
    }
    void end_row() { roff.push_back((int)rcol.size()); }
};

struct Result {
    std::vector<double> x;
    double objective = 0.0;
    bool feasible = false;
    bool optimal = false;
    bool canonical = true;
    long nodes = 0, lp_iters = 0;
    int n_components = 0;
    int price_sweeps = 0, price_rounds = 0;
    double price_bound_us = 0, price_total_us = 0;
    long hull_solves = 0, hull_solves_nonpacking = 0;
};

const double REFERENCE_MIP_REL_GAP = 1e-4;

Result solve(const Model &m, double time_limit_s, bool canonical = true, double rel_gap = REFERENCE_MIP_REL_GAP, hqprice::Sweeper *sweeper = nullptr);

void columns_by_cost_desc(const double *c, int n, std::vector<int> &out);
void set_fast_path(int on);
void set_block_runs(int on);
bool block_runs_on();
struct Probe { uint64_t model = 0, tables = 0, runs = 0, covered = 0; bool corrupt_runs = false; };
extern thread_local Probe *g_probe;
inline uint64_t fnv1a(uint64_t h, const void *p, size_t bytes) { const unsigned char *b = (const unsigned char *)p; for (size_t i = 0; i < bytes; i++) h = (h ^ b[i]) * 1099511628211ull; return h; }
template <class T> inline uint64_t fnv1a_vec(uint64_t h, const std::vector<T> &v) { const uint64_t n = v.size(); h = fnv1a(h, &n, 8); return v.empty() ? h : fnv1a(h, v.data(), v.size() * sizeof(T)); }
const uint64_t FNV_BASIS = 1469598103934665603ull;

}
```

include/hqtick_debug.h:

```cpp
#ifndef HQTICK_DEBUG_H
#define HQTICK_DEBUG_H
#include <stdint.h>
#include "hqtick.h"
#ifdef __cplusplus
extern "C" {
#endif
#if defined(__GNUC__)
#pragma GCC visibility push(default)
#endif

int hqtick_debug_milp_solve(int ncols, const double *obj, const uint8_t *col_kind, int nrows, const uint8_t *row_type,
                            const double *rhs, const int *row_off, const int *row_col, const double *row_coef,
                            double time_limit_s, int canonical, double *x_out, double *obj_out, int *is_optimal,
                            long *nodes_out);

int hqtick_debug_last_order(const hqtick_ctx *ctx, uint32_t *n_runs, uint32_t *n_levels, double *order_us);

int hqtick_debug_last_scan(const hqtick_ctx *ctx, int which, uint32_t *n_levels, uint32_t *n_groups, uint32_t shape[4],
                           uint64_t *levels, uint32_t cap_levels, uint32_t *hist, uint32_t cap_groups);

int hqtick_debug_order_view(hqtick_ctx *ctx, uint32_t n_requests, uint32_t counts[4], uint32_t *perm, uint32_t *inv, uint32_t *lrank, uint64_t cap_slots, uint32_t *run_rq,
                            uint32_t *run_start, uint32_t *run_rank, uint64_t *run_prio, uint32_t cap_runs);
int hqtick_debug_order_select(hqtick_ctx *ctx, const uint32_t *rq_sel_base, const uint32_t *q_tnc, uint32_t n_sel, int mark_mode, uint64_t *sel_task, uint32_t *sel_rank,
                              uint32_t *rq_after, uint32_t *err);
int hqtick_debug_order_rank_of(hqtick_ctx *ctx, const uint64_t *want, uint32_t n_want, uint32_t *out_rq, uint32_t *out_pos);

int hqtick_debug_host_stages(const hqtick_config *config, const hqtick_snapshot *snapshot, const uint8_t *vflags, const uint32_t *vtmc,
                             uint32_t n_levels, const uint64_t *levels, const uint32_t *hist, hqtick_result *out);

int hqtick_debug_host_plan(const hqtick_config *config, const hqtick_snapshot *snapshot, const uint8_t *vflags, const uint32_t *vtmc,
                           uint32_t n_levels, const uint64_t *levels, const uint32_t *hist, const uint32_t *retracting_key,
                           const uint32_t *retracting_rank, hqtick_result *out, const char **error);

int hqtick_debug_host_query(const hqtick_config *config, const hqtick_snapshot *snapshot, const hqtick_query_workers *fake,
                            const uint8_t *vflags, const uint32_t *vtmc, const uint8_t *fake_vflags, const uint32_t *fake_vtmc,
                            uint32_t n_levels, const uint64_t *levels, const uint32_t *hist, hqtick_query_result *out);

int hqtick_debug_milp_was_canonical(void);
void hqtick_debug_milp_last_hull(long *solves, long *nonpacking);

void hqtick_debug_map_order_u32(const uint32_t *keys, uint32_t n, uint32_t *out_pos);

int hqtick_debug_block_solve_host(uint32_t n_cols, uint32_t n_resources, const uint32_t *ent_off, const uint32_t *ent_res, const uint8_t *ent_kind,
                                  const uint64_t *ent_amount, const uint32_t *weight, const double *pool, uint32_t n_classes, const uint64_t *free_,
                                  const uint64_t *total, const uint64_t *elig, uint32_t budget, uint32_t *x, uint32_t *status, uint32_t *steps);
void hqtick_debug_set_block_emulation(int on, uint32_t budget);
void hqtick_debug_last_stage_us(double *out3);
void hqtick_debug_last_blocks(uint32_t *n_emulated, uint32_t *n_host);

int hqtick_time_kernel(hqtick_ctx *ctx, int which, int iters, double *avg_us);
int hqtick_timeline(const hqtick_ctx *ctx, double *out, int cap);
const uint64_t *hqtick_block_profile_last(const hqtick_ctx *ctx, uint32_t *n_classes);


void hqtick_debug_set_price_emulation(int on, uint32_t min_cols);
void hqtick_debug_set_price_fault(int fail_at);
void hqtick_debug_set_fast_path(int on);
void hqtick_debug_check_model_hints(int on);
int hqtick_debug_model_hint_mismatches(void);
void hqtick_debug_set_block_runs(int on);
void hqtick_debug_last_coupled_digest(uint64_t out[4]);
void hqtick_debug_set_early_sweep(int on);
uint32_t hqtick_debug_early_sweeps(void);
void hqtick_debug_capture_first_cut(int on);
uint32_t hqtick_debug_first_cut(unsigned char *out, uint32_t cap);
void hqtick_debug_corrupt_block_runs(int on);
void hqtick_debug_last_price(uint32_t *sweeps, uint32_t *rounds);
uint32_t hqtick_debug_last_mn(const uint32_t **rq, const uint32_t **off, const uint32_t **worker);
int hqtick_debug_milp_solve_priced(int ncols, const double *obj, const uint8_t *col_kind, const int32_t *col_group, int nrows, const uint8_t *row_type,
                                   const uint8_t *row_implied, const double *rhs, const int *row_off, const int *row_col, const double *row_coef,
                                   double time_limit_s, int use_sweeps, uint32_t min_cols, double *x_out, double *obj_out, int *is_optimal, double *stats_out);

struct hqwire_tables;
struct hqwire_records;
struct hqwire_output;
int hqwire_debug_encode_host(const struct hqwire_tables *tables, const struct hqwire_records *records, const struct hqwire_output *out);
int hqwire_debug_encode_host_order(const struct hqwire_tables *tables, const struct hqwire_records *records, const struct hqwire_output *out, int order);
struct hqwire_table;
struct hqwire_table_config;
int hqwire_debug_table_create_host(struct hqwire_table **out, const struct hqwire_table_config *cfg, int order);

void hqtick_debug_set_block_guard(uint32_t verify, uint32_t tick_seq, int corrupt_mode, uint32_t corrupt_class, uint32_t corrupt_fill);
void hqtick_debug_last_block_guard(uint32_t *verified, uint32_t *mismatch, uint32_t *rejected);
void hqtick_debug_set_block_memo(int on);
uint32_t hqtick_debug_last_block_memo(void);
void hqtick_debug_set_exchange(hqtick_exchange_fn fn, void *user, uint32_t rank, uint32_t world, uint32_t min_blocks, uint32_t min_classes);
uint32_t hqtick_debug_last_exchange_calls(void);
int hqtick_debug_exchange(hqtick_ctx *ctx, const void *send, void *recv, size_t bytes_per_rank);

int hqtick_debug_clock_rows(uint32_t n, const int64_t *deadline_ns, int64_t now_ns, uint32_t nv, const uint64_t *min_time_ns, int sorted_form, int64_t *remaining_out);
int64_t hqtick_debug_clock_deadline(int64_t now_ns, int64_t remaining_ns);
int64_t hqtick_debug_clock_remaining(int64_t deadline_ns, int64_t now_ns);
uint32_t hqtick_debug_clock_launches(const hqtick_ctx *ctx);

typedef struct hqtick_debug_audit_tables {
    uint32_t have;
    uint64_t ready_n, ready_live; const uint64_t *ready_id; const uint32_t *ready_rq;
    uint32_t g_slots, g_runs, g_edges, g_free, g_ht_mask; uint64_t g_tasks;
    const uint64_t *g_id; const uint32_t *g_unfinished, *g_gen, *g_head; const uint64_t *g_ht_key; const uint32_t *g_ht_val, *g_run_next, *g_run_off, *g_run_len, *g_edge;
    uint32_t l_mask, l_Q, l_NV, l_W, l_R, l_stride, l_pf_stride; uint64_t l_n_live, l_mn_live, l_pf_live;
    const uint64_t *l_key; const uint32_t *l_worker, *l_rq; const uint8_t *l_variant;
    const uint32_t *l_rq_off, *l_ventry_off, *l_ent_res, *l_var_nodes; const uint8_t *l_ent_kind; const uint64_t *l_ent_amount;
    const uint32_t *l_wid; const uint64_t *l_total, *l_free; const uint32_t *l_counts, *l_pf; const uint64_t *l_mn_task; const uint8_t *l_mn_root, *l_flags;
    uint32_t r_n; const uint64_t *r_task; const uint32_t *r_target; const uint8_t *r_variant, *r_flags;
} hqtick_debug_audit_tables;
int hqtick_debug_audit_host(const hqtick_debug_audit_tables *tables, uint32_t parts, int order, hqtick_check_report *out);
#if defined(__GNUC__)
#pragma GCC visibility pop
#endif
#ifdef __cplusplus
}
#endif
#endif
```

Baseline: 71.54 million.

## Defer MILP fast-path row feasibility check to overlap with GPU mapping

When the pricing fast path certifies a solution, the host-side row feasibility and objective check is no longer run inside the solver. The check is carried out by a callback that runs while the GPU phase-C kernels execute. If the deferred check fails, the tick synchronizes the stream, discards the selection, and re-solves on the classic path. This takes the row check off the critical path, at the cost of a rollback path and of carrying the model along in the result.

```diff
diff --git a/hyperqueue_amd/_testhooks.py b/hyperqueue_amd/_testhooks.py
--- a/hyperqueue_amd/_testhooks.py
+++ b/hyperqueue_amd/_testhooks.py
@@ -13,4 +13,10 @@
         if not os.path.exists(LIB_PATH):
             raise FileNotFoundError(f"{LIB_PATH} is missing: run `python -c 'import __graft_entry__ as g; g.build()'`")
         _LIB = C.CDLL(LIB_PATH)
+        _LIB.hqtick_debug_set_defer_row_check.argtypes = [C.c_int]
+        _LIB.hqtick_debug_set_defer_row_check.restype = None
+        _LIB.hqtick_debug_deferred_row_checks.argtypes = [C.c_int]
+        _LIB.hqtick_debug_deferred_row_checks.restype = C.c_uint32
+        _LIB.hqtick_debug_fail_row_checks.argtypes = [C.c_uint32]
+        _LIB.hqtick_debug_fail_row_checks.restype = C.c_uint32
     return _LIB
diff --git a/hyperqueue_amd/csrc/debug_capi.cpp b/hyperqueue_amd/csrc/debug_capi.cpp
--- a/hyperqueue_amd/csrc/debug_capi.cpp
+++ b/hyperqueue_amd/csrc/debug_capi.cpp
@@ -92,6 +92,12 @@
     return (uint32_t)b.size();
 }
 
+static thread_local hqmilp::CheckHook g_row_check_hook;
+static hqmilp::CheckHook &row_check_hook() { hqmilp::g_check_hook = &g_row_check_hook; return g_row_check_hook; }
+extern "C" void hqtick_debug_set_defer_row_check(int on) { row_check_hook().allow = on; }
+extern "C" uint32_t hqtick_debug_deferred_row_checks(int clear) { hqmilp::CheckHook &h = row_check_hook(); const uint32_t n = h.deferred; if (clear) h.deferred = 0; return n; }
+extern "C" uint32_t hqtick_debug_fail_row_checks(uint32_t n) { hqmilp::CheckHook &h = row_check_hook(); const uint32_t left = h.fail_next; h.fail_next = n; return left; }
+
 extern "C" int hqtick_debug_clock_rows(uint32_t n, const int64_t *deadline_ns, int64_t now_ns, uint32_t nv, const uint64_t *min_time_ns, int sorted_form, int64_t *remaining_out) {
     if ((n && (!deadline_ns || !remaining_out)) || (nv && !min_time_ns)) return HQTICK_E_INVALID;
     if (!sorted_form) {
diff --git a/hyperqueue_amd/csrc/host_model.cpp b/hyperqueue_amd/csrc/host_model.cpp
--- a/hyperqueue_amd/csrc/host_model.cpp
+++ b/hyperqueue_amd/csrc/host_model.cpp
@@ -1257,7 +1257,8 @@
         size_t run_blocks = 0; for (const auto &br : m.block_runs) run_blocks += (size_t)br.n_blocks;
         fprintf(stderr, "[model] cuts done at %.3f ms: %d columns, %d rows, %zu terms, %zu worker signatures, %zu (batch, cut, blocker) passes over the workers; %zu equal-block runs over %zu blocks, %zu (cut, blocker) passes decided once\n", (t_model1 - t_model0) / 1e3, m.ncols(), m.nrows(), m.rcol.size(), sig_rep.size(), n_triples, m.block_runs.size(), run_blocks, n_decided_once);
     }
-    hqmilp::Result sol = hqmilp::solve(m, pb.time_limit_s, !pb.certificate_only, hqmilp::REFERENCE_MIP_REL_GAP, pb.pricer);
+    hqmilp::SolveOpts opts; opts.no_fast_path = pb.no_fast_path; opts.defer_row_check = pb.defer_row_check;
+    hqmilp::Result sol = hqmilp::solve(m, pb.time_limit_s, !pb.certificate_only, hqmilp::REFERENCE_MIP_REL_GAP, pb.pricer, &opts);
     if (trace_model) fprintf(stderr, "[model] solve done %.3f ms after the model\n", (clock_us() - t_model1) / 1e3);
     out.pre_us = t_model0 - t_enter; out.model_us = t_model1 - t_model0; out.milp_us = clock_us() - t_model1; out.price_sweeps = sol.price_sweeps; out.price_rounds = sol.price_rounds; out.price_us = sol.price_total_us;
     out.milp_nodes = sol.nodes; out.milp_cols = m.ncols(); out.milp_rows = m.nrows(); out.milp_components = sol.n_components;
@@ -1309,6 +1310,7 @@
     hqhb::insertion_order(mn_hash.data(), (uint32_t)mn_hash.size(), ord);
     for (uint32_t k : ord) { out.mn_rq.push_back(mn_list[k]); out.mn_sets.push_back(std::move(mn_sets[k])); }
     if (trace_model) fprintf(stderr, "[model] decoded %.3f ms after the model, %.3f ms after the solver was entered\n", (clock_us() - t_model1) / 1e3, (clock_us() - t_enter) / 1e3);
+    if (sol.row_check.pending) { out.row_check.check = std::move(sol.row_check); out.row_check.model = std::move(m); }
     return out;
 }
 
diff --git a/hyperqueue_amd/csrc/host_model.h b/hyperqueue_amd/csrc/host_model.h
--- a/hyperqueue_amd/csrc/host_model.h
+++ b/hyperqueue_amd/csrc/host_model.h
@@ -103,6 +103,8 @@
     const WorkerSet *custom = nullptr;
     double time_limit_s = 5.0;
     bool certificate_only = false;
+    bool defer_row_check = false;
+    bool no_fast_path = false;
     bool rq_multi_node(uint32_t rq) const { return variants[rqs[rq].first_variant].multi_node(); }
     bool capable_rqv(const WorkerSet &ws, uint32_t w, uint32_t rq) const {
         for (uint32_t v = 0; v < rqs[rq].n_variants; v++) {
@@ -141,6 +143,9 @@
         pairs_built = true;
     }
     size_t key_size(size_t k) const { return pairs_built ? per_key[k].size() : lists[key_list[k]].widx.size(); }
+    struct PendingRowCheck { hqmilp::Model model; hqmilp::RowCheck check; } row_check;
+    bool row_check_pending() const { return row_check.check.pending; }
+    bool settle_row_check() { return hqmilp::run_row_check(row_check.model, row_check.check); }
     bool is_optimal = true;
     bool is_canonical = true;
     bool empty() const {
diff --git a/hyperqueue_amd/csrc/hqtick.cpp b/hyperqueue_amd/csrc/hqtick.cpp
--- a/hyperqueue_amd/csrc/hqtick.cpp
+++ b/hyperqueue_amd/csrc/hqtick.cpp
@@ -78,6 +78,7 @@
     hqcluster::Retracting retr;
     uint32_t last_row_groups = 0;
     bool wait_on_kernel = true;
+    bool defer_row_check = true;
     hqhost::Problem pb;
     std::vector<uint32_t> b_rq, b_size, b_limit, b_cut_off, c_size, c_bl_off, bl_rq, bl_size; std::vector<uint8_t> b_lr, b_blk;
     std::vector<uint8_t> q_loaded;
@@ -441,9 +442,9 @@
         return in;
     }
 
-    int phase_c(const hqmap::Env &me, const hqmap::PlanIn &in) {
+    int phase_c(const hqmap::Env &me, const hqmap::PlanIn &in, const std::function<void()> *while_gpu_runs) {
         hqmap::PhaseC pc{};
-        pc.sc = &sc; pc.scan = &ctx->scan; pc.ready = &ctx->ready; pc.in = &in;
+        pc.sc = &sc; pc.scan = &ctx->scan; pc.ready = &ctx->ready; pc.in = &in; pc.while_gpu_runs = while_gpu_runs;
         pc.consume_in_tick = use_resident && (ctx->cfg.flags & HQTICK_FLAG_CONSUME_IN_TICK) != 0;
         pc.ledger_pfq_rq = ctx->asg.on;
         if (ps.n_sel && pc.consume_in_tick && ctx->asg.on && s->n_retracting) {
@@ -461,6 +462,14 @@
         if (tm.sweep_us >= 0) ctx->stats.sweep_us = tm.sweep_us;
         if (tm.other_us >= 0) ctx->stats.other_us = tm.other_us;
         return rc;
+    }
+
+    bool may_defer_row_check() const {
+        const int sw = hqmilp::g_check_hook ? hqmilp::g_check_hook->allow : -1;
+        if (!(sw < 0 ? ctx->defer_row_check : sw != 0)) return false;
+        if (use_resident && (ctx->cfg.flags & HQTICK_FLAG_CONSUME_IN_TICK)) return false;
+        if (ctx->asg.on || ctx->sink || ctx->shard_count > 1 || ctx->xfn || ctx->comm) return false;
+        return s->n_retracting == 0;
     }
 
     void finish(const hqmap::Env &me, double t1, double t2, double t3) {
@@ -504,52 +513,70 @@
         export_batches(ctx, batches, out);
         mark();
         const double t2 = now_us();
-        DeviceBlocks dev_blocks(ctx);
-        pb.blocks = &dev_blocks; pb.block_min_classes = ctx->block_min_classes; pb.pricer = ctx->pricer;
-        pb.block_verify = ctx->block_verify; pb.tick_seq = ctx->tick_seq++;
-        pb.memo = (ctx->cfg.flags & (HQTICK_FLAG_NO_BLOCK_MEMO | HQTICK_FLAG_NO_TICK_CACHES)) ? nullptr : &ctx->block_memo;
-        double shard_sweep_us = -1.0;
-        ctx->x_calls = 0; ctx->x_bytes = 0; ctx->x_us = 0;
-        if (CtxExchange::available(ctx)) {
-            CtxExchange xch(ctx);
-            ShardedBlocks sh_blocks(dev_blocks, xch, ctx->shard_min_classes);
-            pb.blocks = &sh_blocks;
-            if (ctx->pricer) {
-                hqprice::ShardedSweeper sh_sweeps(*ctx->pricer, xch, ctx->shard_min_blocks);
-                pb.pricer = &sh_sweeps;
-                cnt = hqhost::run_scheduling_solver(pb, batches);
-                shard_sweep_us = sh_sweeps.stat_sweep_us;
+        const hqmap::Env me = map_env(ctx, t0);
+        const uint32_t tick_seq = ctx->tick_seq++;
+        const int ntl_solve = ctx->ntl;
+        double t3 = t2;
+        bool check_ok = true;
+        const std::function<void()> check = [&]() { if (cnt.row_check_pending()) check_ok = cnt.settle_row_check(); };
+        auto solve_plan_map = [&](bool defer, bool classic) -> int {
+            int rc;
+            DeviceBlocks dev_blocks(ctx);
+            pb.blocks = &dev_blocks; pb.block_min_classes = ctx->block_min_classes; pb.pricer = ctx->pricer;
+            pb.defer_row_check = defer; pb.no_fast_path = classic;
+            pb.block_verify = ctx->block_verify; pb.tick_seq = tick_seq;
+            pb.memo = (ctx->cfg.flags & (HQTICK_FLAG_NO_BLOCK_MEMO | HQTICK_FLAG_NO_TICK_CACHES)) ? nullptr : &ctx->block_memo;
+            double shard_sweep_us = -1.0;
+            ctx->x_calls = 0; ctx->x_bytes = 0; ctx->x_us = 0;
+            if (CtxExchange::available(ctx)) {
+                CtxExchange xch(ctx);
+                ShardedBlocks sh_blocks(dev_blocks, xch, ctx->shard_min_classes);
+                pb.blocks = &sh_blocks;
+                if (ctx->pricer) {
+                    hqprice::ShardedSweeper sh_sweeps(*ctx->pricer, xch, ctx->shard_min_blocks);
+                    pb.pricer = &sh_sweeps;
+                    cnt = hqhost::run_scheduling_solver(pb, batches);
+                    shard_sweep_us = sh_sweeps.stat_sweep_us;
+                } else cnt = hqhost::run_scheduling_solver(pb, batches);
             } else cnt = hqhost::run_scheduling_solver(pb, batches);
-        } else cnt = hqhost::run_scheduling_solver(pb, batches);
-        pb.blocks = nullptr; pb.pricer = nullptr;
-        ctx->stats.price_sweeps = (uint32_t)cnt.price_sweeps; ctx->stats.price_rounds = (uint32_t)cnt.price_rounds; ctx->stats.price_us = cnt.price_us; ctx->stats.milp_us = cnt.milp_us; ctx->stats.model_us = cnt.model_us; ctx->stats.solve_pre_us = cnt.pre_us;
-        ctx->stats.price_sweep_us = shard_sweep_us >= 0.0 ? shard_sweep_us : (ctx->pricer ? ctx->pricer->stat_sweep_us : 0.0); ctx->stats.milp_cols = (uint32_t)cnt.milp_cols; ctx->stats.milp_rows = (uint32_t)cnt.milp_rows;
-        ctx->stats.n_classes_verified = cnt.blocks_verified; ctx->stats.n_classes_mismatch = cnt.blocks_mismatch; ctx->stats.n_classes_rejected = cnt.blocks_rejected; ctx->stats.n_classes_memo = cnt.blocks_memo;
-        ctx->stats.exchange_calls = (uint32_t)ctx->x_calls; ctx->stats.exchange_bytes = ctx->x_bytes; ctx->stats.exchange_us = ctx->x_us;
-        if (cnt.error) return fail(ctx, cnt.error, cnt.errmsg);
-        ctx->stats.n_classes_device = cnt.blocks_device; ctx->stats.n_classes_host = cnt.blocks_host; ctx->stats.block_steps_max = cnt.block_steps_max; ctx->stats.n_classes = cnt.n_classes;
-        ctx->stats.solve_classify_us = cnt.t_classify_us; ctx->stats.solve_blocks_us = cnt.t_blocks_us; ctx->stats.solve_decode_us = cnt.t_decode_us;
-        mark();
-        const double t3 = now_us();
-        out->is_optimal = cnt.is_optimal;
-        out->is_canonical = cnt.is_canonical && cnt.is_optimal;
-        status = HQTICK_DONE;
-        if (!cnt.is_optimal) status = cnt.empty() ? HQTICK_NO_PROGRESS : HQTICK_NEED_MORE_COMPUTE;
-        const hqmap::PlanIn in = plan_in();
-        const hqmap::Env me = map_env(ctx, t0);
-        hqmap::HostResult &hr = ctx->map.res;
-        const char *why = nullptr;
-        ctx->ready.selection_void();
-        if ((rc = plan_fail(hqmap::plan_keys(ps, hr, in, &why), why))) return rc;
-        if ((rc = map_fail(ctx, ctx->map.launch_sweep_early(me)))) return rc;
-        if ((rc = plan_fail(hqmap::plan_redirects(ps, hr, in, &why), why))) return rc;
-        mark();
-        if ((rc = plan_fail(hqmap::plan_prefill(ps, hr, in, &why), why))) return rc;
-        mark();
-        if ((rc = plan_fail(hqmap::plan_outputs(ps, hr, in, &why), why))) return rc;
-        if ((rc = map_fail(ctx, ctx->map.check_capacity(sc.ordered)))) return rc;
-        mark();
-        if ((rc = phase_c(me, in))) return rc;
+            pb.blocks = nullptr; pb.pricer = nullptr; pb.defer_row_check = false; pb.no_fast_path = false;
+            ctx->stats.price_sweeps = (uint32_t)cnt.price_sweeps; ctx->stats.price_rounds = (uint32_t)cnt.price_rounds; ctx->stats.price_us = cnt.price_us; ctx->stats.milp_us = cnt.milp_us; ctx->stats.model_us = cnt.model_us; ctx->stats.solve_pre_us = cnt.pre_us;
+            ctx->stats.price_sweep_us = shard_sweep_us >= 0.0 ? shard_sweep_us : (ctx->pricer ? ctx->pricer->stat_sweep_us : 0.0); ctx->stats.milp_cols = (uint32_t)cnt.milp_cols; ctx->stats.milp_rows = (uint32_t)cnt.milp_rows;
+            ctx->stats.n_classes_verified = cnt.blocks_verified; ctx->stats.n_classes_mismatch = cnt.blocks_mismatch; ctx->stats.n_classes_rejected = cnt.blocks_rejected; ctx->stats.n_classes_memo = cnt.blocks_memo;
+            ctx->stats.exchange_calls = (uint32_t)ctx->x_calls; ctx->stats.exchange_bytes = ctx->x_bytes; ctx->stats.exchange_us = ctx->x_us;
+            if (cnt.error) return fail(ctx, cnt.error, cnt.errmsg);
+            ctx->stats.n_classes_device = cnt.blocks_device; ctx->stats.n_classes_host = cnt.blocks_host; ctx->stats.block_steps_max = cnt.block_steps_max; ctx->stats.n_classes = cnt.n_classes;
+            ctx->stats.solve_classify_us = cnt.t_classify_us; ctx->stats.solve_blocks_us = cnt.t_blocks_us; ctx->stats.solve_decode_us = cnt.t_decode_us;
+            mark();
+            t3 = now_us();
+            out->is_optimal = cnt.is_optimal;
+            out->is_canonical = cnt.is_canonical && cnt.is_optimal;
+            status = HQTICK_DONE;
+            if (!cnt.is_optimal) status = cnt.empty() ? HQTICK_NO_PROGRESS : HQTICK_NEED_MORE_COMPUTE;
+            const hqmap::PlanIn in = plan_in();
+            hqmap::HostResult &hr = ctx->map.res;
+            const char *why = nullptr;
+            ctx->ready.selection_void();
+            if ((rc = plan_fail(hqmap::plan_keys(ps, hr, in, &why), why))) return rc;
+            if ((rc = map_fail(ctx, ctx->map.launch_sweep_early(me)))) return rc;
+            if ((rc = plan_fail(hqmap::plan_redirects(ps, hr, in, &why), why))) return rc;
+            mark();
+            if ((rc = plan_fail(hqmap::plan_prefill(ps, hr, in, &why), why))) return rc;
+            mark();
+            if ((rc = plan_fail(hqmap::plan_outputs(ps, hr, in, &why), why))) return rc;
+            if ((rc = map_fail(ctx, ctx->map.check_capacity(sc.ordered)))) return rc;
+            mark();
+            return phase_c(me, in, defer && cnt.row_check_pending() ? &check : nullptr);
+        };
+        rc = solve_plan_map(may_defer_row_check(), false);
+        check();
+        if (!check_ok) {
+            HQ_HIP(hipStreamSynchronize(ctx->stream));
+            ctx->ready.selection_void(); ctx->map.forget_selection();
+            ctx->ntl = ntl_solve; cnt = hqhost::Counts();
+            rc = solve_plan_map(false, true);
+        }
+        if (rc) return rc;
         mark();
         finish(me, t1, t2, t3);
         return status;
@@ -676,6 +703,7 @@
     if (hipStreamCreateWithFlags(&ctx->stream2, hipStreamNonBlocking) != hipSuccess) { hipStreamDestroy(ctx->stream); delete ctx; return HQTICK_E_DEVICE; }
     if (const char *e = getenv("HQTICK_K2_RIDE_ALONG")) { ctx->k2_own_stream = atoi(e) == 0; ctx->k2_on_hist = atoi(e) == 1; }
     if (const char *e = getenv("HQTICK_WAIT_ON_KERNEL")) ctx->wait_on_kernel = atoi(e) != 0;
+    if (const char *e = getenv("HQTICK_DEFER_ROW_CHECK")) ctx->defer_row_check = atoi(e) != 0;
     {
         bool price = true; uint32_t min_cols = 0;
         if (const char *e = getenv("HQTICK_PRICE")) price = atoi(e) != 0;
@@ -1542,16 +1570,21 @@
     hqprice::EmulatedSweeper pemu;
     if (g_price_emulation) { pemu.fail_at = g_price_fault; pemu.budget = g_block_budget; if (g_price_min_cols) pemu.min_cols = g_price_min_cols; pb.pricer = &pemu; }
     hqhost::Counts cnt;
-    if (g_xfn && g_xworld > 1) {
-        struct FnExchange : hqprice::Exchange { bool allgather(const void *snd, void *rcv, size_t bytes) override { return g_xfn(g_xuser, snd, rcv, bytes) == 0; } } xch;
-        xch.rank = g_xrank; xch.world = g_xworld;
-        ShardedBlocks sh_blocks(emu, xch, g_xmin_classes);
-        hqprice::ShardedSweeper sh_sweeps(pemu, xch, g_xmin_blocks);
-        if (pb.blocks) pb.blocks = &sh_blocks;
-        if (pb.pricer) pb.pricer = &sh_sweeps;
-        cnt = hqhost::run_scheduling_solver(pb, batches);
-        g_xcalls = (uint32_t)xch.n_calls;
-    } else cnt = hqhost::run_scheduling_solver(pb, batches);
+    auto solve = [&]() {
+        if (g_xfn && g_xworld > 1) {
+            struct FnExchange : hqprice::Exchange { bool allgather(const void *snd, void *rcv, size_t bytes) override { return g_xfn(g_xuser, snd, rcv, bytes) == 0; } } xch;
+            xch.rank = g_xrank; xch.world = g_xworld;
+            ShardedBlocks sh_blocks(emu, xch, g_xmin_classes);
+            hqprice::ShardedSweeper sh_sweeps(pemu, xch, g_xmin_blocks);
+            if (pb.blocks) pb.blocks = &sh_blocks;
+            if (pb.pricer) pb.pricer = &sh_sweeps;
+            cnt = hqhost::run_scheduling_solver(pb, batches);
+            g_xcalls = (uint32_t)xch.n_calls;
+        } else cnt = hqhost::run_scheduling_solver(pb, batches);
+    };
+    pb.defer_row_check = hqmilp::g_check_hook && hqmilp::g_check_hook->allow == 1 && !(g_xfn && g_xworld > 1);
+    solve();
+    if (cnt.row_check_pending() && !cnt.settle_row_check()) { pb.defer_row_check = false; pb.no_fast_path = true; solve(); }
     if (cnt.error) return fail(ctx, cnt.error, cnt.errmsg);
     g_last_guard[0] = cnt.blocks_verified; g_last_guard[1] = cnt.blocks_mismatch; g_last_guard[2] = cnt.blocks_rejected;
     g_last_memo = cnt.blocks_memo;
diff --git a/hyperqueue_amd/csrc/map.cpp b/hyperqueue_amd/csrc/map.cpp
--- a/hyperqueue_amd/csrc/map.cpp
+++ b/hyperqueue_amd/csrc/map.cpp
@@ -1,6 +1,8 @@
 #include "map.h"
 
 #include <chrono>
+#include <cstdio>
+#include <cstdlib>
 
 namespace hqmap {
 
@@ -163,7 +165,12 @@
         }
         e.tl.mark();
         assemble_host_part(ps, res, *pc.in);
+        static const bool tracing = getenv("HQMILP_TRACE") != nullptr;
+        const double tw0 = tracing ? now_us() : 0.0;
+        if (pc.while_gpu_runs) (*pc.while_gpu_runs)();
+        const double tw1 = tracing ? now_us() : 0.0;
         if (expand_is_last) HQ_HIP(hipEventSynchronize(e.k5b_stop)); else HQ_HIP(hipStreamSynchronize(e.stream));
+        if (tracing && n_sel > 1000) fprintf(stderr, "[map] phase C: %.1f us of the caller's work while the kernels ran, then %.1f us waiting for them\n", tw1 - tw0, now_us() - tw1);
         sweep_inflight = false;
         if (flags[0]) return fail(HQTICK_E_CAPACITY, "mapping kernel capacity exceeded");
         if (sc.ordered && *pc.scan->select_err_host()) return fail(HQTICK_E_DEVICE, "ordered view: the selection left its request's segment");
@@ -172,6 +179,7 @@
     if (!n_sel) {
         pc.ready->selected(0);
         assemble_host_part(ps, res, *pc.in);
+        if (pc.while_gpu_runs) (*pc.while_gpu_runs)();
     }
     if (!n_sel && e.sink) {
         if (hqtick_sink_bytes(W, 0) > e.sink_bytes) return fail(HQTICK_E_CAPACITY, "record sink too small for this tick");
diff --git a/hyperqueue_amd/csrc/map.h b/hyperqueue_amd/csrc/map.h
--- a/hyperqueue_amd/csrc/map.h
+++ b/hyperqueue_amd/csrc/map.h
@@ -2,6 +2,7 @@
 #include <hip/hip_runtime.h>
 
 #include <cstdint>
+#include <functional>
 #include <string>
 
 #include "../../include/hqtick.h"
@@ -34,6 +35,7 @@
     bool ledger_pfq_rq;
     uint32_t *saved_rq;
     hqk::Stage stage;
+    const std::function<void()> *while_gpu_runs;
 };
 struct Timings { double select_us = -1, sweep_us = -1, other_us = -1; };
 enum Replay { REPLAY_TOMBSTONE, REPLAY_RESTORE, REPLAY_TIMED };
@@ -50,6 +52,7 @@
     int phase_c(const Env &e, const PhaseC &pc);
     void export_result(const Env &e, const hqhost::Counts &cnt, hqtick_result *out);
     const Timings &timings() const { return t_; }
+    void forget_selection() { sweep_launched = false; last_ordered = false; last_os = hqk::OrderSelect{}; last_geom = hqk::WaveGeom{}; last_L = last_Q = last_G = 0; last_tb = last_plan_bytes = 0; t_ = Timings{}; }
     int replay_selection(hipStream_t st, Replay mode, const hqready::Cols &cols, const hqscan::Scanner &scan, uint32_t n_sel, hqbuf::PinBuf *scratch = nullptr);
     struct Last { bool ordered; hqk::WaveGeom geom; uint32_t L, Q, G; };
     Last last_selection() const { return Last{last_ordered, last_geom, last_L, last_Q, last_G}; }
diff --git a/hyperqueue_amd/csrc/milp.cpp b/hyperqueue_amd/csrc/milp.cpp
--- a/hyperqueue_amd/csrc/milp.cpp
+++ b/hyperqueue_amd/csrc/milp.cpp
@@ -1328,12 +1328,48 @@
 
 const double ROW_TOL = 1e-6;
 
+bool check_point(const Model &mdl_in, const std::vector<double> &x, double cost_scale, double bound, double rel_gap, double *objective) {
+    const int n = mdl_in.ncols(), m = mdl_in.nrows();
+    if ((int)x.size() != n) return false;
+    bool ok = true;
+    for (int j = 0; j < n && ok; j++) { const double v = x[(size_t)j]; if (v < -1e-9 || std::fabs(v - std::floor(v + 0.5)) > 1e-9 || (mdl_in.kind[j] == COL_BOOL && v > 1.0 + 1e-9)) ok = false; }
+    std::vector<double> lhs_act; std::vector<uint8_t> lhs_seen;
+    for (int i = 0; i < m && ok; i++) {
+        double a = 0.0;
+        int k0 = mdl_in.roff[i];
+        const int L = mdl_in.row_lhs[i];
+        if (L >= 0) {
+            if ((size_t)L >= lhs_seen.size()) { lhs_seen.resize((size_t)L + 1, 0); lhs_act.resize((size_t)L + 1, 0.0); }
+            if (!lhs_seen[(size_t)L]) { double s = 0.0; for (int k = mdl_in.list_off[L]; k < mdl_in.list_off[L + 1]; k++) s += x[(size_t)mdl_in.list_col[k]]; lhs_act[(size_t)L] = s; lhs_seen[(size_t)L] = 1; }
+            a = lhs_act[(size_t)L];
+        }
+        for (int k = k0; k < mdl_in.roff[i + 1]; k++) a += mdl_in.rcoef[k] * x[(size_t)mdl_in.rcol[k]];
+        const double tol = std::max(ROW_TOL, 1e-9 * std::max(1.0, std::fabs(mdl_in.rhs[i])));
+        if (mdl_in.rtype[i] != ROW_MIN && a > mdl_in.rhs[i] + tol) ok = false;
+        if (mdl_in.rtype[i] != ROW_MAX && a < mdl_in.rhs[i] - tol) ok = false;
+    }
+    if (!ok) return false;
+    double z_pt = 0.0;
+    for (int j = 0; j < n; j++) z_pt += mdl_in.obj[j] * std::floor(x[(size_t)j] + 0.5);
+    const double zs = cost_scale > 0.0 ? z_pt / cost_scale : z_pt;
+    if (!(bound * (1.0 + 1e-9) + 1e-12 <= zs + rel_gap * std::fabs(zs))) return false;
+    *objective = z_pt;
+    return true;
+}
+
+thread_local CheckHook *g_check_hook = nullptr;
+bool run_row_check(const Model &m, RowCheck &rc) {
+    rc.pending = false;
+    if (g_check_hook && g_check_hook->fail_next > 0) { g_check_hook->fail_next--; return false; }
+    return check_point(m, rc.x, rc.cost_scale, rc.bound, rc.rel_gap, &rc.objective);
+}
+
 namespace {
-bool solve_fast(const Model &mdl_in, double time_limit_s, double rel_gap, hqprice::Sweeper *sweeper, const double ts0, Result &res_out) {
+bool solve_fast(const Model &mdl_in, double time_limit_s, double rel_gap, hqprice::Sweeper *sweeper, const double ts0, const SolveOpts *opts, Result &res_out) {
     static const bool tracing_solve = getenv("HQMILP_TRACE") != nullptr;
     auto tmark = [&](const char *what) { if (tracing_solve && mdl_in.ncols() > 1000) fprintf(stderr, "[milp] solve(): %s at %.3f ms\n", what, (wall() - ts0) * 1e3); };
     static const bool fast_env = !(getenv("HQMILP_FAST") && atoi(getenv("HQMILP_FAST")) == 0);
-    const bool fast_on = g_fast_path < 0 ? fast_env : g_fast_path != 0;
+    const bool fast_on = !(opts && opts->no_fast_path) && (g_fast_path < 0 ? fast_env : g_fast_path != 0);
     const int FAST_MIN_COLS = 2048;
     const bool hints_there = (int)mdl_in.col_group.size() == mdl_in.ncols() && (int)mdl_in.row_lhs.size() == mdl_in.nrows() && (int)mdl_in.row_lhs_len.size() == mdl_in.nrows();
     const bool takes_it = fast_on && sweeper && rel_gap > 0.0 && mdl_in.ncols() >= FAST_MIN_COLS && mdl_in.ncols() >= (int)sweeper->min_cols && hints_there && (int)mdl_in.start.size() != mdl_in.ncols();
@@ -1353,29 +1389,20 @@
         hqprice::Answer pa = hqprice::solve_model(mv, rel_gap, time_limit_s, ts0 + (time_limit_s > 0 ? time_limit_s : 1e18), tracing_solve, *sweeper, &cost_scale);
         if (tracing_solve) fprintf(stderr, "[milp] fast path: ran %d (%s) sweeps %u rounds %u bound %.9f point %.9f, %.3f ms of which %.3f ms inside the sweeps\n", (int)pa.ran, pa.why, pa.sweeps, pa.rounds, pa.ran ? pa.bound : -1.0, pa.x.empty() ? -1.0 : pa.x_value, (wall() - tf0) * 1e3, sweeper->stat_sweep_us / 1e3);
         if (pa.ran && (int)pa.x.size() == n && pa.bound * (1.0 + 1e-9) + 1e-12 <= pa.x_value + rel_gap * std::fabs(pa.x_value)) {
-            bool ok = true;
-            for (int j = 0; j < n && ok; j++) { const double v = pa.x[(size_t)j]; if (v < -1e-9 || std::fabs(v - std::floor(v + 0.5)) > 1e-9 || (mdl_in.kind[j] == COL_BOOL && v > 1.0 + 1e-9)) ok = false; }
-            std::vector<double> lhs_act; std::vector<uint8_t> lhs_seen;
-            for (int i = 0; i < m && ok; i++) {
-                double a = 0.0;
-                int k0 = mdl_in.roff[i];
-                const int L = mdl_in.row_lhs[i];
-                if (L >= 0) {
-                    if ((size_t)L >= lhs_seen.size()) { lhs_seen.resize((size_t)L + 1, 0); lhs_act.resize((size_t)L + 1, 0.0); }
-                    if (!lhs_seen[(size_t)L]) { double s = 0.0; for (int k = mdl_in.list_off[L]; k < mdl_in.list_off[L + 1]; k++) s += pa.x[(size_t)mdl_in.list_col[k]]; lhs_act[(size_t)L] = s; lhs_seen[(size_t)L] = 1; }
-                    a = lhs_act[(size_t)L];
-                }
-                for (int k = k0; k < mdl_in.roff[i + 1]; k++) a += mdl_in.rcoef[k] * pa.x[(size_t)mdl_in.rcol[k]];
-                const double tol = std::max(ROW_TOL, 1e-9 * std::max(1.0, std::fabs(mdl_in.rhs[i])));
-                if (mdl_in.rtype[i] != ROW_MIN && a > mdl_in.rhs[i] + tol) ok = false;
-                if (mdl_in.rtype[i] != ROW_MAX && a < mdl_in.rhs[i] - tol) ok = false;
+            if (opts && opts->defer_row_check) {
+                Result res;
+                res.x.resize((size_t)n);
+                for (int j = 0; j < n; j++) res.x[(size_t)j] = std::floor(pa.x[(size_t)j] + 0.5);
+                res.feasible = true; res.optimal = true; res.canonical = false;
+                res.n_components = 1; res.nodes = pa.sweeps; res.price_sweeps = (int)pa.sweeps; res.price_rounds = (int)pa.rounds; res.price_total_us = (wall() - tf0) * 1e6;
+                res.row_check.pending = true; res.row_check.x = std::move(pa.x); res.row_check.cost_scale = cost_scale; res.row_check.bound = pa.bound; res.row_check.rel_gap = rel_gap;
+                if (g_check_hook) g_check_hook->deferred++;
+                tmark("fast path certified by the sweeps, row check pending");
+                res_out = std::move(res);
+                return true;
             }
             double z_pt = 0.0;
-            if (ok) {
-                for (int j = 0; j < n; j++) z_pt += mdl_in.obj[j] * std::floor(pa.x[(size_t)j] + 0.5);
-                const double zs = cost_scale > 0.0 ? z_pt / cost_scale : z_pt;
-                if (!(pa.bound * (1.0 + 1e-9) + 1e-12 <= zs + rel_gap * std::fabs(zs))) ok = false;
-            }
+            const bool ok = check_point(mdl_in, pa.x, cost_scale, pa.bound, rel_gap, &z_pt);
             if (ok) {
                 Result res;
                 res.x = std::move(pa.x);
@@ -1396,9 +1423,9 @@
 
 static Result solve_classic(const Model &mdl_in, double time_limit_s, bool canonical, double rel_gap, hqprice::Sweeper *sweeper, const double ts0);
 
-Result solve(const Model &mdl_arg, double time_limit_s, bool canonical, double rel_gap, hqprice::Sweeper *sweeper) {
+Result solve(const Model &mdl_arg, double time_limit_s, bool canonical, double rel_gap, hqprice::Sweeper *sweeper, const SolveOpts *opts) {
     const double ts_entry = wall();
-    { Result r; if (solve_fast(mdl_arg, time_limit_s, rel_gap, sweeper, ts_entry, r)) return r; }
+    { Result r; if (solve_fast(mdl_arg, time_limit_s, rel_gap, sweeper, ts_entry, opts, r)) return r; }
     if (mdl_arg.has_lists()) {
         Model plain = mdl_arg;
         plain.expand_lists();
diff --git a/hyperqueue_amd/csrc/milp.h b/hyperqueue_amd/csrc/milp.h
--- a/hyperqueue_amd/csrc/milp.h
+++ b/hyperqueue_amd/csrc/milp.h
@@ -69,6 +69,13 @@
     void end_row() { roff.push_back((int)rcol.size()); }
 };
 
+struct RowCheck {
+    bool pending = false;
+    std::vector<double> x;
+    double cost_scale = 1.0, bound = 0.0, rel_gap = 0.0;
+    double objective = 0.0;
+};
+
 struct Result {
     std::vector<double> x;
     double objective = 0.0;
@@ -80,11 +87,20 @@
     int price_sweeps = 0, price_rounds = 0;
     double price_bound_us = 0, price_total_us = 0;
     long hull_solves = 0, hull_solves_nonpacking = 0;
+    RowCheck row_check;
+};
+
+struct SolveOpts {
+    bool no_fast_path = false;
+    bool defer_row_check = false;
 };
 
 const double REFERENCE_MIP_REL_GAP = 1e-4;
 
-Result solve(const Model &m, double time_limit_s, bool canonical = true, double rel_gap = REFERENCE_MIP_REL_GAP, hqprice::Sweeper *sweeper = nullptr);
+Result solve(const Model &m, double time_limit_s, bool canonical = true, double rel_gap = REFERENCE_MIP_REL_GAP, hqprice::Sweeper *sweeper = nullptr, const SolveOpts *opts = nullptr);
+
+bool check_point(const Model &m, const std::vector<double> &x, double cost_scale, double bound, double rel_gap, double *objective);
+bool run_row_check(const Model &m, RowCheck &rc);
 
 void columns_by_cost_desc(const double *c, int n, std::vector<int> &out);
 void set_fast_path(int on);
@@ -92,6 +108,8 @@
 bool block_runs_on();
 struct Probe { uint64_t model = 0, tables = 0, runs = 0, covered = 0; bool corrupt_runs = false; };
 extern thread_local Probe *g_probe;
+struct CheckHook { int allow = -1; uint32_t deferred = 0, fail_next = 0; };
+extern thread_local CheckHook *g_check_hook;
 inline uint64_t fnv1a(uint64_t h, const void *p, size_t bytes) { const unsigned char *b = (const unsigned char *)p; for (size_t i = 0; i < bytes; i++) h = (h ^ b[i]) * 1099511628211ull; return h; }
 template <class T> inline uint64_t fnv1a_vec(uint64_t h, const std::vector<T> &v) { const uint64_t n = v.size(); h = fnv1a(h, &n, 8); return v.empty() ? h : fnv1a(h, v.data(), v.size() * sizeof(T)); }
 const uint64_t FNV_BASIS = 1469598103934665603ull;
diff --git a/include/hqtick_debug.h b/include/hqtick_debug.h
--- a/include/hqtick_debug.h
+++ b/include/hqtick_debug.h
@@ -62,6 +62,9 @@
 void hqtick_debug_last_coupled_digest(uint64_t out[4]);
 void hqtick_debug_set_early_sweep(int on);
 uint32_t hqtick_debug_early_sweeps(void);
+void hqtick_debug_set_defer_row_check(int on);
+uint32_t hqtick_debug_deferred_row_checks(int clear);
+uint32_t hqtick_debug_fail_row_checks(uint32_t n);
 void hqtick_debug_capture_first_cut(int on);
 uint32_t hqtick_debug_first_cut(unsigned char *out, uint32_t cap);
 void hqtick_debug_corrupt_block_runs(int on);
```

Result: faster. 76.93 million (median of 6 runs) (+7.5%).
